# LiangZhaoPKUImperial/LinearSFM

Hardware: AMD Instinct MI355X
Metric: hierarchical linear map-joining solve wall-clock, NC3500-like stereo (all transforms + joins) (lower is better)
Workload: dtype f64

## Files before the change

include/lsfm.h:

```cpp
#ifndef LSFM_H
#define LSFM_H

#include <stddef.h>

#ifdef __cplusplus
extern "C" {
#endif

#define LSFM_OK 0
#define LSFM_ERR_ARG (-1)
#define LSFM_ERR_NO_DEVICE (-2)
#define LSFM_ERR_HIP (-3)
#define LSFM_ERR_OOM (-4)
#define LSFM_ERR_INTERNAL (-5)
#define LSFM_ERR_IO (-6)
#define LSFM_ERR_NOT_SPD (-7)
#define LSFM_NOT_CONVERGED 1

typedef struct lsfm_context lsfm_context;

typedef struct lsfm_map {
	int Ref, FRef, m, n, nU, nW;
	int ScaP, Fix, Sign, FScaP, FFix;
	int* stno;
	double* stVal;
	double* U;
	int *Ui, *Uj;
	double* W;
	int *photo, *feature;
	double* V;
	int* FBlock;
	int* pose_origin;
} lsfm_map;

typedef struct lsfm_stats {
	double t_total_ms;
	double t_transform_ms, t_join_ms, t_schur_ms, t_pcg_ms, t_backsub_ms;
	long pcg_iterations;
	long spmv_launches;
	double spmv_ms;
	double spmv_bytes;
	long spmv_nnzb_upper_last, spmv_rows_last;
	double max_rel_residual;
	int levels, joins, transforms;
	int not_converged;
	long schur_launches, trf_launches;
	double schur_ms, schur_bytes, trf_ms, trf_bytes;
	double schur_flops;
	double upload_ms;
	int attempts;
	unsigned long long s_digest, factor_digest;
	int dist_solves;
	double dist_work_total, dist_work_shared;
	int refactor_mismatch;
	int s_rebuild_mismatch;
	int small_levels;
	double t_small_ms;
} lsfm_stats;

int lsfm_context_create(int device, size_t arena_bytes, lsfm_context** out);
void lsfm_context_destroy(lsfm_context* ctx);
int lsfm_set_pcg(lsfm_context* ctx, double rel_tol, int max_steps);
int lsfm_set_precision(lsfm_context* ctx, int mode);
int lsfm_set_small_solve(lsfm_context* ctx, int max_poses);
int lsfm_set_spmv_variant(lsfm_context* ctx, int variant);
int lsfm_set_covcols_panel(lsfm_context* ctx, int variant);
const char* lsfm_last_error(lsfm_context* ctx);
void* lsfm_stream(lsfm_context* ctx);

void lsfm_map_release(lsfm_map* g);

int lsfm_transform_stereo(lsfm_context* ctx, const lsfm_map* in, int Ref, lsfm_map* out);
int lsfm_transform_mono(lsfm_context* ctx, const lsfm_map* in, int Ref, int ScaP, int Fix, lsfm_map* out);

int lsfm_join_stereo(lsfm_context* ctx, const lsfm_map* End, const lsfm_map* Cur, lsfm_map* joint,
                     double* eP_out, double* eF_out);
int lsfm_join_mono(lsfm_context* ctx, const lsfm_map* End, const lsfm_map* Cur, lsfm_map* joint,
                   double* eP_out, double* eF_out);

int lsfm_solve_stereo(lsfm_context* ctx, double* stVal, const double* eb, const double* ea, const double* U,
                      const double* W, const double* V, const int* Ui, const int* Uj, const int* photo,
                      const int* feature, int m, int n, int nU, int nW, const double* x0);
int lsfm_solve_mono(lsfm_context* ctx, double* stVal, const double* eb, const double* ea, const double* U,
                    const double* W, const double* V, const int* Ui, const int* Uj, const int* photo,
                    const int* feature, int m, int n, int nU, int nW, int Ref, int ScaP, int Fix, int Sign,
                    int FixBlk, const double* x0);

int lsfm_gn_polish(lsfm_context* ctx, const lsfm_map* maps, int N, int type, lsfm_map* x, int iters, double* obj, double* gnorm, int* halvings);

int lsfm_map_chi2(lsfm_context* ctx, const lsfm_map* maps, int N, int type, const lsfm_map* x, double* chi2, int* dof);
int lsfm_gn_polish_robust(lsfm_context* ctx, const lsfm_map* maps, int N, int type, lsfm_map* x, int iters, int kind, double c,
                          double* obj, double* gnorm, int* halvings, double* chi2, double* weight);

int lsfm_map_feature_chi2(lsfm_context* ctx, const lsfm_map* maps, int N, int type, const lsfm_map* x, double* fchi2, double* pose_chi2);
int lsfm_gn_polish_robust_features(lsfm_context* ctx, const lsfm_map* maps, int N, int type, lsfm_map* x, int iters, int kind, double c,
                                   double* obj, double* gnorm, int* halvings, double* fchi2, double* fweight);

int lsfm_gn_linearise(lsfm_context* ctx, const lsfm_map* maps, int N, int type, const lsfm_map* x, const double* weight,
                      lsfm_map* out, double* obj, double* b);
int lsfm_gn_linearise_timed(lsfm_context* ctx, const lsfm_map* maps, int N, int type, const lsfm_map* x, const double* weight,
                            lsfm_map* out, double* obj, double* b, double* times, int* counts);

int lsfm_map_covariance(lsfm_context* ctx, const lsfm_map* map, int mono, double* pose_cov, double* feat_cov, double* pair_cov, int cap_blocks, int* nnzb);
int lsfm_map_covariance_timed(lsfm_context* ctx, const lsfm_map* map, int mono, double* pose_cov, double* feat_cov, double* pair_cov, int cap_blocks, int* nnzb,
                              double* times);

int lsfm_map_covariance_columns(lsfm_context* ctx, const lsfm_map* map, int mono, const int* poses, int k, double* pose_cols, double* feat_cols,
                                double* joint, int* steps, double* last_corr);
int lsfm_map_covariance_columns_timed(lsfm_context* ctx, const lsfm_map* map, int mono, const int* poses, int k, double* pose_cols, double* feat_cols,
                                      double* joint, int* steps, double* last_corr, double* times);

int lsfm_map_covariance_feature_columns(lsfm_context* ctx, const lsfm_map* map, int mono, const int* feats, int k, double* pose_cols, double* feat_cols,
                                        double* joint, int* steps, double* last_corr);
int lsfm_map_feature_pair_gate(lsfm_context* ctx, const lsfm_map* map, int mono, const int* pairs, int K, double* d2, double* cov_diff, int* steps,
                               double* last_corr);
int lsfm_map_covariance_feature_columns_timed(lsfm_context* ctx, const lsfm_map* map, int mono, const int* feats, int k, double* pose_cols,
                                              double* feat_cols, double* joint, int* steps, double* last_corr, double* times);
int lsfm_map_feature_pair_gate_timed(lsfm_context* ctx, const lsfm_map* map, int mono, const int* pairs, int K, double* d2, double* cov_diff, int* steps,
                                     double* last_corr, double* times);

int lsfm_map_merge_features(lsfm_context* ctx, const lsfm_map* map, int mono, const int* pairs, int K, lsfm_map* out, double* d2, int* dof, int* rep,
                            int* steps, double* last_corr);
int lsfm_map_merge_features_timed(lsfm_context* ctx, const lsfm_map* map, int mono, const int* pairs, int K, lsfm_map* out, double* d2, int* dof,
                                  int* rep, int* steps, double* last_corr, double* times);
int lsfm_merge_structure(const lsfm_map* map, const int* pairs, int K, int* rep, int* photo, int* feature, int* FBlock, int* sptr, int* sidx, int cap_w,
                         int* info, char* why, int why_cap);

int lsfm_map_feature_pair_candidates(lsfm_context* ctx, const lsfm_map* map, const double* feat_cov, double radius, double tau, int* pairs, double* dist2,
                                     double* q, long long cap, long long* count);
int lsfm_map_feature_pair_candidates_timed(lsfm_context* ctx, const lsfm_map* map, const double* feat_cov, double radius, double tau, int* pairs,
                                           double* dist2, double* q, long long cap, long long* count, double* times, long long* info);

#define LSFM_JOINT_GATE_MAX 2048
int lsfm_map_feature_pair_joint_gate(lsfm_context* ctx, const lsfm_map* map, int mono, const int* pairs, int K, const int* order, double tau, int* status,
                                     double* delta, double* d2, double* joint_C, int* accepted, int* implied, double* D2, int* steps, double* last_corr);
int lsfm_map_feature_pair_joint_gate_timed(lsfm_context* ctx, const lsfm_map* map, int mono, const int* pairs, int K, const int* order, double tau,
                                           int* status, double* delta, double* d2, double* joint_C, int* accepted, int* implied, double* D2, int* steps,
                                           double* last_corr, double* times);
int lsfm_selftest_pair_select(lsfm_context* ctx, int K, const double* C, const double* d, const int* ends, const int* order, double tau, int* status,
                              double* delta, double* D2, int* accepted, int* implied);

int lsfm_map_marginalise(lsfm_context* ctx, const lsfm_map* map, const unsigned char* drop, lsfm_map* out);
int lsfm_map_marginalise_timed(lsfm_context* ctx, const lsfm_map* map, const unsigned char* drop, lsfm_map* out, double* times);

int lsfm_map_marginalise_poses(lsfm_context* ctx, const lsfm_map* map, int mono, const unsigned char* keep_pose, const unsigned char* drop_feat,
                               lsfm_map* out);
int lsfm_map_marginalise_poses_timed(lsfm_context* ctx, const lsfm_map* map, int mono, const unsigned char* keep_pose, const unsigned char* drop_feat,
                                     lsfm_map* out, double* times, int* info);
int lsfm_marg_pose_structure(const lsfm_map* map, int mono, const unsigned char* keep_pose, const unsigned char* drop_feat, unsigned char* drop,
                             int* comp, int* nptr, int* nidx, int cap_n, int* bd, int* Ui, int* Uj, int cap_u, int* info, char* why, int why_cap);

int lsfm_gn_structure(const lsfm_map* maps, int N, int type, const lsfm_map* x, int want_slots, int want_coalesce, int* info, int* map_hubs,
                      int* wdst, int* fptrJ, int* photoJ, int cap_wj, int* UiJ, int* UjJ, int cap_uj, int* photo, int* feature, int* FBlock,
                      int cap_w, int* Ui, int* Uj, int cap_u, int* slot_map, int* slot_a, int* slot_b, int* slot_count, int cap_s, char* why,
                      int why_cap);

int lsfm_inverse_v(lsfm_context* ctx, double* V, int m, int n);
int lsfm_solve_features(lsfm_context* ctx, const double* W, const double* IV, const double* ea, const double* eb, const double* dpa, double* dpb,
                        int m, int n, const int* mapCor, const int* photo);

int lsfm_schur_pattern(lsfm_context* ctx, const int* Ui, const int* Uj, const int* photo, const int* feature, int m, int n, int nU, int nW,
                       int* rowptr, int* colidx, int cap, int* nnzb);

int lsfm_symbolic_analyse(int m, const int* rowptr, const int* colidx, const int* origin, int reps, int* perm, int* colptr, int* rowidx,
                          int cap, int* info, double* avg_ms);

typedef struct lsfm_tree lsfm_tree;
int lsfm_tree_upload(lsfm_context* ctx, const lsfm_map* maps, int N, int mono, lsfm_tree** out);
int lsfm_tree_run(lsfm_context* ctx, lsfm_tree* tree, lsfm_stats* stats);
int lsfm_tree_set_final_reanchor(lsfm_tree* tree, int on);
int lsfm_tree_set_plans(lsfm_tree* tree, int on);
int lsfm_tree_download(lsfm_context* ctx, lsfm_tree* tree, lsfm_map* out);
int lsfm_tree_set_stop_level(lsfm_tree* tree, int levels);
int lsfm_tree_node_count(lsfm_context* ctx, lsfm_tree* tree);
int lsfm_tree_download_node(lsfm_context* ctx, lsfm_tree* tree, int k, lsfm_map* out);
int lsfm_tree_download_state(lsfm_context* ctx, lsfm_tree* tree, int* m, int* n, int* stno, double* stVal, size_t cap);
void lsfm_tree_free(lsfm_context* ctx, lsfm_tree* tree);
size_t lsfm_tree_export_size(lsfm_context* ctx, lsfm_tree* tree);
int lsfm_tree_export_dev(lsfm_context* ctx, lsfm_tree* tree, void* dst, size_t cap);
#define LSFM_PACK_HEADER_BYTES 256
size_t lsfm_packed_size(const void* host_header256);
int lsfm_tree_upload_dev(lsfm_context* ctx, const void* const* packed, int N, int mono, lsfm_tree** out);
int lsfm_tree_export_reduced_size(lsfm_context* ctx, lsfm_tree* tree, const int* keep_ids, int nkeep, size_t* bytes);
int lsfm_tree_export_reduced_dev(lsfm_context* ctx, lsfm_tree* tree, const int* keep_ids, int nkeep, void* dst, size_t cap);
int lsfm_tree_export_reduced_dev_timed(lsfm_context* ctx, lsfm_tree* tree, const int* keep_ids, int nkeep, void* dst, size_t cap, double* times);
int lsfm_tree_reload_dev(lsfm_context* ctx, lsfm_tree* tree, const void* const* packed, int N);

#define LSFM_DTYPE_F64 0
#define LSFM_DTYPE_I64 1
typedef int (*lsfm_allreduce_fn)(void* user, size_t offset_bytes, size_t count, int dtype, void* hip_stream);
int lsfm_tree_set_comm(lsfm_tree* tree, int rank, int world, lsfm_allreduce_fn fn, void* user, void* dev_buf, size_t dev_bytes);
int lsfm_tree_set_comm_blocks(lsfm_tree* tree, int block_maps);
int lsfm_tree_export_slice_sizes(lsfm_context* ctx, lsfm_tree* tree, int nslices, size_t* sizes);
int lsfm_tree_export_slice_dev(lsfm_context* ctx, lsfm_tree* tree, int nslices, int slice, void* dst, size_t cap);

int lsfm_divide_conquer(lsfm_context* ctx, const lsfm_map* maps, int N, int mono, lsfm_map* out, lsfm_stats* stats);

int lsfm_read_localmap(const char* path, int mono, lsfm_map* out);
int lsfm_read_localmaps(const char* dir, int first, int count, int mono, int threads, lsfm_map* out, int* failed);
int lsfm_write_localmap(const char* path, int mono, const lsfm_map* map);
int lsfm_write_mapset(const char* path, const lsfm_map* maps, int N, int mono);
int lsfm_mapset_info(const char* path, int* N, int* mono);
int lsfm_mapset_stamp(const char* path, unsigned long long* stamp, const unsigned long long* set_to);
int lsfm_read_mapset(const char* path, int mono, int first, int count, int threads, lsfm_map* out);
int lsfm_save_covariances(const char* pose_path, const char* feat_path, const int* stno, int m, int n, const double* pose_cov, const double* feat_cov);
int lsfm_read_covariances(const char* path, int k, int* ids, double* cov, int cap, int* count);
int lsfm_save_cov_columns(const char* path, const int* stno, int m, const int* poses, int k, const double* pose_cols);
int lsfm_read_cov_columns(const char* path, int* ids_q, int* ids_p, double* blocks, int cap, int* count);
int lsfm_save_pair_gate(const char* path, const int* ids, int K, const double* d2, const double* cov_diff);
int lsfm_read_pair_gate(const char* path, int* ids_f, int* ids_g, double* d2, double* cov_diff, int cap, int* count);
int lsfm_save_merge_report(const char* path, int K, int removed, int dof, double d2, const int* ids);
int lsfm_read_merge_report(const char* path, int* K, int* removed, int* dof, double* d2, int* ids, int cap);
int lsfm_save_joint_gate(const char* path, const int* ids, int K, const int* status, const double* d2, const double* delta, int accepted, int implied,
                         double D2);
int lsfm_read_joint_gate(const char* path, int* ids, int* status, double* d2, double* delta, int cap, int* head, double* D2);
int lsfm_save_pair_list(const char* path, const int* ids, long long K);
int lsfm_read_pair_list(const char* path, int* ids, long long cap, long long* count);
int lsfm_save_state(const char* path, const double* st, const int* stno, int n);
int lsfm_save_state_bin(const char* path, const double* st, const int* stno, int n);
int lsfm_save_poses(const char* pose_path, const char* feat_path, const int* stno, const double* st, int n);

int lsfm_spmv_bench(lsfm_context* ctx, int m, const int* rowptr, const int* colidx, const double* val,
                    const double* x, double* y, int reps, double* avg_ms, double* algorithmic_bytes);

int lsfm_wstream_bench(lsfm_context* ctx, long long nblocks, int mode, int reps, double* avg_ms);

int lsfm_selftest_prims(lsfm_context* ctx, int cases, unsigned seed);

int lsfm_selftest_vinv(lsfm_context* ctx, const double* V, const double* eb, int n, int skip, double* IV, double* LY);

#define LSFM_SELFTEST_CHOL_INFO 16
int lsfm_selftest_chol(lsfm_context* ctx, int m, const int* rowptr, const int* colidx, const double* val, const int* origin, const unsigned char* fixed,
                       const int* pose_seg, int nseg, const double* r, int nrhs, int mode, double* z, double* dot, int* perm, int* colptr, int* rowidx,
                       double* L, double* Dinv, double* dscale, int cap_blocks, int* info);

int lsfm_selftest_transform(lsfm_context* ctx, const lsfm_map* maps, int N, int mono, const int* tref, const int* tscap, const int* tfix,
                            int alias_passthrough, lsfm_map* out);

int lsfm_selftest_small(lsfm_context* ctx, int G, const int* pose_off, const int* feat_off, const int* u_off, const unsigned char* active,
                        const double* U, const int* Ui, const int* Uj, const double* W, const int* photo, const int* feature, int nW, const double* V,
                        const double* ea, const double* eb, const double* x0, const unsigned char* fixed, int strips, double* x_pose, double* x_feat,
                        int* status, double* max_rel);

#ifdef __cplusplus
}
#endif
#endif
```

linearsfm_amd/api.py:

```python
from __future__ import annotations

import ctypes as C
import os

import numpy as np

_HERE = os.path.dirname(os.path.abspath(__file__))
LIB_PATH = os.path.join(_HERE, "liblsfm_hip.so")
_LIB = None

LSFM_OK = 0
LSFM_NOT_CONVERGED = 1


class LsfmMap(C.Structure):
    _fields_ = [("Ref", C.c_int), ("FRef", C.c_int), ("m", C.c_int), ("n", C.c_int), ("nU", C.c_int), ("nW", C.c_int),
                ("ScaP", C.c_int), ("Fix", C.c_int), ("Sign", C.c_int), ("FScaP", C.c_int), ("FFix", C.c_int),
                ("stno", C.POINTER(C.c_int)), ("stVal", C.POINTER(C.c_double)),
                ("U", C.POINTER(C.c_double)), ("Ui", C.POINTER(C.c_int)), ("Uj", C.POINTER(C.c_int)),
                ("W", C.POINTER(C.c_double)), ("photo", C.POINTER(C.c_int)), ("feature", C.POINTER(C.c_int)),
                ("V", C.POINTER(C.c_double)), ("FBlock", C.POINTER(C.c_int)), ("pose_origin", C.POINTER(C.c_int))]


class LsfmStats(C.Structure):
    _fields_ = [("t_total_ms", C.c_double), ("t_transform_ms", C.c_double), ("t_join_ms", C.c_double),
                ("t_schur_ms", C.c_double), ("t_pcg_ms", C.c_double), ("t_backsub_ms", C.c_double),
                ("pcg_iterations", C.c_long), ("spmv_launches", C.c_long), ("spmv_ms", C.c_double),
                ("spmv_bytes", C.c_double), ("spmv_nnzb_upper_last", C.c_long), ("spmv_rows_last", C.c_long),
                ("max_rel_residual", C.c_double), ("levels", C.c_int), ("joins", C.c_int), ("transforms", C.c_int),
                ("not_converged", C.c_int), ("schur_launches", C.c_long), ("trf_launches", C.c_long),
                ("schur_ms", C.c_double), ("schur_bytes", C.c_double), ("trf_ms", C.c_double), ("trf_bytes", C.c_double),
                ("schur_flops", C.c_double), ("upload_ms", C.c_double), ("attempts", C.c_int),
                ("s_digest", C.c_ulonglong), ("factor_digest", C.c_ulonglong), ("dist_solves", C.c_int), ("dist_work_total", C.c_double), ("dist_work_shared", C.c_double), ("refactor_mismatch", C.c_int), ("s_rebuild_mismatch", C.c_int), ("small_levels", C.c_int), ("t_small_ms", C.c_double)]

    def as_dict(self):
        return {k: getattr(self, k) for k, _ in self._fields_}


class LsfmError(RuntimeError):
    pass


ALLREDUCE_FN = C.CFUNCTYPE(C.c_int, C.c_void_p, C.c_size_t, C.c_size_t, C.c_int, C.c_void_p)
LSFM_DTYPE_F64, LSFM_DTYPE_I64 = 0, 1
JOINT_GATE_MAX = 2048
JOINT_GATE_TAU = 11.344866730144373


def lib():
    global _LIB
    if _LIB is None:
        if not os.path.exists(LIB_PATH):
            raise LsfmError(f"{LIB_PATH} is missing: build it with `python -c 'import __graft_entry__ as g; g.build()'` "
                            "(hipcc --offload-arch=gfx950).  There is no CPU fallback.")
        L = C.CDLL(LIB_PATH)
        P = C.POINTER
        dp, ip, vp = P(C.c_double), P(C.c_int), C.c_void_p
        L.lsfm_context_create.argtypes = [C.c_int, C.c_size_t, P(vp)]
        L.lsfm_context_destroy.argtypes = [vp]
        L.lsfm_context_destroy.restype = None
        L.lsfm_set_pcg.argtypes = [vp, C.c_double, C.c_int]
        L.lsfm_set_precision.argtypes = [vp, C.c_int]
        L.lsfm_set_small_solve.argtypes = [vp, C.c_int]
        L.lsfm_set_spmv_variant.argtypes = [vp, C.c_int]
        L.lsfm_set_covcols_panel.argtypes = [vp, C.c_int]
        L.lsfm_last_error.argtypes = [vp]
        L.lsfm_last_error.restype = C.c_char_p
        L.lsfm_stream.argtypes = [vp]
        L.lsfm_stream.restype = vp
        L.lsfm_map_release.argtypes = [P(LsfmMap)]
        L.lsfm_map_release.restype = None
        L.lsfm_transform_stereo.argtypes = [vp, P(LsfmMap), C.c_int, P(LsfmMap)]
        L.lsfm_transform_mono.argtypes = [vp, P(LsfmMap), C.c_int, C.c_int, C.c_int, P(LsfmMap)]
        L.lsfm_join_stereo.argtypes = [vp, P(LsfmMap), P(LsfmMap), P(LsfmMap), dp, dp]
        L.lsfm_join_mono.argtypes = [vp, P(LsfmMap), P(LsfmMap), P(LsfmMap), dp, dp]
        L.lsfm_solve_stereo.argtypes = [vp, dp, dp, dp, dp, dp, dp, ip, ip, ip, ip, C.c_int, C.c_int, C.c_int, C.c_int, dp]
        L.lsfm_solve_mono.argtypes = [vp, dp, dp, dp, dp, dp, dp, ip, ip, ip, ip, C.c_int, C.c_int, C.c_int, C.c_int,
                                      C.c_int, C.c_int, C.c_int, C.c_int, C.c_int, dp]
        L.lsfm_tree_upload.argtypes = [vp, P(LsfmMap), C.c_int, C.c_int, P(vp)]
        L.lsfm_tree_run.argtypes = [vp, vp, P(LsfmStats)]
        L.lsfm_tree_set_final_reanchor.argtypes = [vp, C.c_int]
        L.lsfm_tree_set_plans.argtypes = [vp, C.c_int]
        L.lsfm_tree_export_size.argtypes = [vp, vp]
        L.lsfm_tree_export_size.restype = C.c_size_t
        L.lsfm_tree_export_dev.argtypes = [vp, vp, vp, C.c_size_t]
        L.lsfm_packed_size.argtypes = [vp]
        L.lsfm_packed_size.restype = C.c_size_t
        L.lsfm_tree_upload_dev.argtypes = [vp, P(vp), C.c_int, C.c_int, P(vp)]
        L.lsfm_tree_reload_dev.argtypes = [vp, vp, P(vp), C.c_int]
        L.lsfm_tree_set_comm.argtypes = [vp, C.c_int, C.c_int, ALLREDUCE_FN, vp, vp, C.c_size_t]
        L.lsfm_tree_set_comm_blocks.argtypes = [vp, C.c_int]
        L.lsfm_tree_export_slice_sizes.argtypes = [vp, vp, C.c_int, P(C.c_size_t)]
        L.lsfm_tree_export_slice_dev.argtypes = [vp, vp, C.c_int, C.c_int, vp, C.c_size_t]
        L.lsfm_tree_download.argtypes = [vp, vp, P(LsfmMap)]
        L.lsfm_tree_set_stop_level.argtypes = [vp, C.c_int]
        L.lsfm_tree_node_count.argtypes = [vp, vp]
        L.lsfm_tree_download_node.argtypes = [vp, vp, C.c_int, P(LsfmMap)]
        L.lsfm_tree_download_state.argtypes = [vp, vp, ip, ip, ip, dp, C.c_size_t]
        L.lsfm_tree_free.argtypes = [vp, vp]
        L.lsfm_tree_free.restype = None
        L.lsfm_divide_conquer.argtypes = [vp, P(LsfmMap), C.c_int, C.c_int, P(LsfmMap), P(LsfmStats)]
        L.lsfm_read_localmap.argtypes = [C.c_char_p, C.c_int, P(LsfmMap)]
        L.lsfm_write_localmap.argtypes = [C.c_char_p, C.c_int, P(LsfmMap)]
        L.lsfm_read_localmaps.argtypes = [C.c_char_p, C.c_int, C.c_int, C.c_int, C.c_int, P(LsfmMap), P(C.c_int)]
        L.lsfm_write_mapset.argtypes = [C.c_char_p, P(LsfmMap), C.c_int, C.c_int]
        L.lsfm_mapset_info.argtypes = [C.c_char_p, P(C.c_int), P(C.c_int)]
        L.lsfm_read_mapset.argtypes = [C.c_char_p, C.c_int, C.c_int, C.c_int, C.c_int, P(LsfmMap)]
        L.lsfm_save_state_bin.argtypes = [C.c_char_p, P(C.c_double), P(C.c_int), C.c_int]
        L.lsfm_save_state.argtypes = [C.c_char_p, dp, ip, C.c_int]
        L.lsfm_save_poses.argtypes = [C.c_char_p, C.c_char_p, ip, dp, C.c_int]
        L.lsfm_schur_pattern.argtypes = [vp, ip, ip, ip, ip, C.c_int, C.c_int, C.c_int, C.c_int, ip, ip, C.c_int, ip]
        L.lsfm_symbolic_analyse.argtypes = [C.c_int, ip, ip, ip, C.c_int, ip, ip, ip, C.c_int, ip, dp]
        L.lsfm_inverse_v.argtypes = [vp, dp, C.c_int, C.c_int]
        L.lsfm_selftest_vinv.argtypes = [vp, dp, dp, C.c_int, C.c_int, dp, dp]
        L.lsfm_gn_polish.argtypes = [vp, P(LsfmMap), C.c_int, C.c_int, P(LsfmMap), C.c_int, dp, dp, ip]
        L.lsfm_gn_polish_robust.argtypes = [vp, P(LsfmMap), C.c_int, C.c_int, P(LsfmMap), C.c_int, C.c_int, C.c_double, dp, dp, ip, dp, dp]
        L.lsfm_map_chi2.argtypes = [vp, P(LsfmMap), C.c_int, C.c_int, P(LsfmMap), dp, ip]
        L.lsfm_map_feature_chi2.argtypes = [vp, P(LsfmMap), C.c_int, C.c_int, P(LsfmMap), dp, dp]
        L.lsfm_gn_polish_robust_features.argtypes = [vp, P(LsfmMap), C.c_int, C.c_int, P(LsfmMap), C.c_int, C.c_int, C.c_double, dp, dp, ip, dp, dp]
        L.lsfm_gn_linearise.argtypes = [vp, P(LsfmMap), C.c_int, C.c_int, P(LsfmMap), dp, P(LsfmMap), dp, dp]
        L.lsfm_gn_linearise_timed.argtypes = [vp, P(LsfmMap), C.c_int, C.c_int, P(LsfmMap), dp, P(LsfmMap), dp, dp, dp, ip]
        L.lsfm_solve_features.argtypes = [vp, dp, dp, dp, dp, dp, dp, C.c_int, C.c_int, ip, ip]
        L.lsfm_map_covariance.argtypes = [vp, P(LsfmMap), C.c_int, dp, dp, dp, C.c_int, ip]
        L.lsfm_map_covariance_timed.argtypes = [vp, P(LsfmMap), C.c_int, dp, dp, dp, C.c_int, ip, dp]
        L.lsfm_save_covariances.argtypes = [C.c_char_p, C.c_char_p, ip, C.c_int, C.c_int, dp, dp]
        L.lsfm_read_covariances.argtypes = [C.c_char_p, C.c_int, ip, dp, C.c_int, ip]
        L.lsfm_map_covariance_columns.argtypes = [vp, P(LsfmMap), C.c_int, ip, C.c_int, dp, dp, dp, ip, dp]
        L.lsfm_map_covariance_columns_timed.argtypes = [vp, P(LsfmMap), C.c_int, ip, C.c_int, dp, dp, dp, ip, dp, dp]
        L.lsfm_map_covariance_feature_columns.argtypes = [vp, P(LsfmMap), C.c_int, ip, C.c_int, dp, dp, dp, ip, dp]
        L.lsfm_map_covariance_feature_columns_timed.argtypes = [vp, P(LsfmMap), C.c_int, ip, C.c_int, dp, dp, dp, ip, dp, dp]
        L.lsfm_map_feature_pair_gate.argtypes = [vp, P(LsfmMap), C.c_int, ip, C.c_int, dp, dp, ip, dp]
        L.lsfm_map_feature_pair_gate_timed.argtypes = [vp, P(LsfmMap), C.c_int, ip, C.c_int, dp, dp, ip, dp, dp]
        L.lsfm_map_merge_features.argtypes = [vp, P(LsfmMap), C.c_int, ip, C.c_int, P(LsfmMap), dp, ip, ip, ip, dp]
        L.lsfm_map_merge_features_timed.argtypes = [vp, P(LsfmMap), C.c_int, ip, C.c_int, P(LsfmMap), dp, ip, ip, ip, dp, dp]
        L.lsfm_map_feature_pair_joint_gate.argtypes = [vp, P(LsfmMap), C.c_int, ip, C.c_int, ip, C.c_double, ip, dp, dp, dp, ip, ip, dp, ip, dp]
        L.lsfm_map_feature_pair_joint_gate_timed.argtypes = [vp, P(LsfmMap), C.c_int, ip, C.c_int, ip, C.c_double, ip, dp, dp, dp, ip, ip, dp, ip, dp, dp]
        L.lsfm_selftest_pair_select.argtypes = [vp, C.c_int, dp, dp, ip, ip, C.c_double, ip, dp, dp, ip, ip]
        L.lsfm_save_joint_gate.argtypes = [C.c_char_p, ip, C.c_int, ip, dp, dp, C.c_int, C.c_int, C.c_double]
        L.lsfm_read_joint_gate.argtypes = [C.c_char_p, ip, ip, dp, dp, C.c_int, ip, dp]
        L.lsfm_merge_structure.argtypes = [P(LsfmMap), ip, C.c_int, ip, ip, ip, ip, ip, ip, C.c_int, ip, C.c_char_p, C.c_int]
        llp = P(C.c_longlong)
        L.lsfm_map_feature_pair_candidates.argtypes = [vp, P(LsfmMap), dp, C.c_double, C.c_double, ip, dp, dp, C.c_longlong, llp]
        L.lsfm_map_feature_pair_candidates_timed.argtypes = [vp, P(LsfmMap), dp, C.c_double, C.c_double, ip, dp, dp, C.c_longlong, llp, dp, llp]
        L.lsfm_save_pair_list.argtypes = [C.c_char_p, ip, C.c_longlong]
        L.lsfm_read_pair_list.argtypes = [C.c_char_p, ip, C.c_longlong, llp]
        L.lsfm_save_merge_report.argtypes = [C.c_char_p, C.c_int, C.c_int, C.c_int, C.c_double, ip]
        L.lsfm_read_merge_report.argtypes = [C.c_char_p, ip, ip, ip, dp, ip, C.c_int]
        L.lsfm_save_cov_columns.argtypes = [C.c_char_p, ip, C.c_int, ip, C.c_int, dp]
        L.lsfm_read_cov_columns.argtypes = [C.c_char_p, ip, ip, dp, C.c_int, ip]
        L.lsfm_save_pair_gate.argtypes = [C.c_char_p, ip, C.c_int, dp, dp]
        L.lsfm_read_pair_gate.argtypes = [C.c_char_p, ip, ip, dp, dp, C.c_int, ip]
        L.lsfm_map_marginalise.argtypes = [vp, P(LsfmMap), P(C.c_ubyte), P(LsfmMap)]
        L.lsfm_map_marginalise_timed.argtypes = [vp, P(LsfmMap), P(C.c_ubyte), P(LsfmMap), dp]
        ub = P(C.c_ubyte)
        L.lsfm_map_marginalise_poses.argtypes = [vp, P(LsfmMap), C.c_int, ub, ub, P(LsfmMap)]
        L.lsfm_map_marginalise_poses_timed.argtypes = [vp, P(LsfmMap), C.c_int, ub, ub, P(LsfmMap), dp, ip]
        L.lsfm_marg_pose_structure.argtypes = [P(LsfmMap), C.c_int, ub, ub, ub, ip, ip, ip, C.c_int, ip, ip, ip, C.c_int, ip, C.c_char_p, C.c_int]
        L.lsfm_gn_structure.argtypes = [P(LsfmMap), C.c_int, C.c_int, P(LsfmMap), C.c_int, C.c_int, ip, ip, ip, ip, ip, C.c_int, ip, ip, C.c_int, ip, ip, ip,
                                        C.c_int, ip, ip, C.c_int, ip, ip, ip, ip, C.c_int, C.c_char_p, C.c_int]
        L.lsfm_tree_export_reduced_size.argtypes = [vp, vp, ip, C.c_int, P(C.c_size_t)]
        L.lsfm_tree_export_reduced_dev.argtypes = [vp, vp, ip, C.c_int, vp, C.c_size_t]
        L.lsfm_tree_export_reduced_dev_timed.argtypes = [vp, vp, ip, C.c_int, vp, C.c_size_t, dp]
        L.lsfm_spmv_bench.argtypes = [vp, C.c_int, ip, ip, dp, dp, dp, C.c_int, dp, dp]
        L.lsfm_wstream_bench.argtypes = [vp, C.c_longlong, C.c_int, C.c_int, dp]
        L.lsfm_selftest_prims.argtypes = [vp, C.c_int, C.c_uint]
        L.lsfm_selftest_chol.argtypes = [vp, C.c_int, ip, ip, dp, ip, P(C.c_ubyte), ip, C.c_int, dp, C.c_int, C.c_int, dp, dp, ip, ip, ip, dp, dp, dp,
                                         C.c_int, ip]
        L.lsfm_selftest_transform.argtypes = [vp, P(LsfmMap), C.c_int, C.c_int, ip, ip, ip, C.c_int, P(LsfmMap)]
        L.lsfm_selftest_small.argtypes = [vp, C.c_int, ip, ip, ip, ub, dp, ip, ip, dp, ip, ip, C.c_int, dp, dp, dp, dp, ub, C.c_int, dp, dp, ip, dp]
        _LIB = L
    return _LIB


EXPORTS = ["lsfm_context_create", "lsfm_context_destroy", "lsfm_set_pcg", "lsfm_set_precision", "lsfm_set_small_solve", "lsfm_set_spmv_variant", "lsfm_set_covcols_panel", "lsfm_last_error", "lsfm_stream",
           "lsfm_map_release", "lsfm_transform_stereo", "lsfm_transform_mono", "lsfm_join_stereo", "lsfm_join_mono",
           "lsfm_solve_stereo", "lsfm_solve_mono", "lsfm_tree_upload", "lsfm_tree_run", "lsfm_tree_set_final_reanchor",
           "lsfm_tree_download", "lsfm_tree_set_stop_level", "lsfm_tree_node_count", "lsfm_tree_download_node", "lsfm_tree_download_state", "lsfm_tree_set_plans", "lsfm_tree_export_size", "lsfm_tree_export_dev", "lsfm_packed_size",
           "lsfm_tree_upload_dev", "lsfm_tree_reload_dev", "lsfm_tree_set_comm", "lsfm_tree_set_comm_blocks", "lsfm_tree_export_slice_sizes", "lsfm_tree_export_slice_dev",
           "lsfm_tree_free", "lsfm_divide_conquer", "lsfm_read_localmap", "lsfm_read_localmaps", "lsfm_write_localmap", "lsfm_write_mapset", "lsfm_mapset_info", "lsfm_mapset_stamp", "lsfm_read_mapset", "lsfm_save_state_bin", "lsfm_save_state", "lsfm_save_poses", "lsfm_gn_polish",
           "lsfm_gn_polish_robust", "lsfm_map_chi2", "lsfm_map_feature_chi2", "lsfm_gn_polish_robust_features", "lsfm_gn_linearise", "lsfm_gn_linearise_timed",
           "lsfm_spmv_bench", "lsfm_wstream_bench", "lsfm_selftest_prims", "lsfm_selftest_chol", "lsfm_selftest_transform", "lsfm_selftest_small", "lsfm_schur_pattern", "lsfm_symbolic_analyse", "lsfm_inverse_v", "lsfm_selftest_vinv", "lsfm_solve_features",
           "lsfm_map_covariance", "lsfm_map_covariance_timed",
           "lsfm_save_covariances", "lsfm_read_covariances",
           "lsfm_map_covariance_columns", "lsfm_map_covariance_columns_timed", "lsfm_save_cov_columns", "lsfm_read_cov_columns",
           "lsfm_map_covariance_feature_columns", "lsfm_map_covariance_feature_columns_timed", "lsfm_map_feature_pair_gate", "lsfm_map_feature_pair_gate_timed", "lsfm_save_pair_gate", "lsfm_read_pair_gate",
           "lsfm_map_merge_features", "lsfm_map_merge_features_timed", "lsfm_merge_structure", "lsfm_save_merge_report", "lsfm_read_merge_report",
           "lsfm_map_feature_pair_candidates", "lsfm_map_feature_pair_candidates_timed", "lsfm_save_pair_list", "lsfm_read_pair_list",
           "lsfm_map_feature_pair_joint_gate", "lsfm_map_feature_pair_joint_gate_timed", "lsfm_selftest_pair_select", "lsfm_save_joint_gate", "lsfm_read_joint_gate",
           "lsfm_map_marginalise", "lsfm_map_marginalise_timed", "lsfm_tree_export_reduced_size", "lsfm_tree_export_reduced_dev",
           "lsfm_tree_export_reduced_dev_timed", "lsfm_map_marginalise_poses", "lsfm_map_marginalise_poses_timed", "lsfm_marg_pose_structure", "lsfm_gn_structure"]


def _c(a, dtype):
    return np.ascontiguousarray(a, dtype=dtype).reshape(-1)


def _ptr(a, ctype):
    return a.ctypes.data_as(C.POINTER(ctype))


class HostMap:

    def __init__(self, d):
        g = d if isinstance(d, dict) else d.__dict__
        self.stno = _c(g["stno"], np.int32); self.stVal = _c(g["stVal"], np.float64)
        self.U = _c(g["U"], np.float64); self.Ui = _c(g["Ui"], np.int32); self.Uj = _c(g["Uj"], np.int32)
        self.W = _c(g["W"], np.float64); self.photo = _c(g["photo"], np.int32); self.feature = _c(g["feature"], np.int32)
        self.V = _c(g["V"], np.float64); self.FBlock = _c(g["FBlock"], np.int32)
        c = LsfmMap()
        c.Ref = int(g["Ref"]); c.FRef = int(g.get("FRef", g["Ref"])); c.m = int(g["m"]); c.n = int(g["n"])
        c.nU = len(self.Ui); c.nW = len(self.photo)
        c.ScaP = int(g.get("ScaP", 0)); c.Fix = int(g.get("Fix", 0)); c.Sign = int(g.get("Sign", 1))
        c.FScaP = int(g.get("FScaP", c.ScaP)); c.FFix = int(g.get("FFix", c.Fix))
        c.stno = _ptr(self.stno, C.c_int); c.stVal = _ptr(self.stVal, C.c_double)
        c.U = _ptr(self.U, C.c_double); c.Ui = _ptr(self.Ui, C.c_int); c.Uj = _ptr(self.Uj, C.c_int)
        c.W = _ptr(self.W, C.c_double); c.photo = _ptr(self.photo, C.c_int); c.feature = _ptr(self.feature, C.c_int)
        c.V = _ptr(self.V, C.c_double); c.FBlock = _ptr(self.FBlock, C.c_int)
        if g.get("pose_origin") is not None:
            self.pose_origin = _c(g["pose_origin"], np.int32)
            c.pose_origin = _ptr(self.pose_origin, C.c_int)
        self.c = c


def _arr(ptr, n, dtype):
    if n == 0:
        return np.zeros(0, dtype)
    return np.ctypeslib.as_array(ptr, shape=(n,)).astype(dtype, copy=True)


def map_to_dict(g: LsfmMap, release=True):
    r = 6 * g.m + 3 * g.n
    d = dict(Ref=g.Ref, FRef=g.FRef, m=g.m, n=g.n, nU=g.nU, nW=g.nW, ScaP=g.ScaP, Fix=g.Fix, Sign=g.Sign,
             FScaP=g.FScaP, FFix=g.FFix,
             stno=_arr(g.stno, r, np.int32), stVal=_arr(g.stVal, r, np.float64),
             U=_arr(g.U, 36 * g.nU, np.float64).reshape(-1, 36), Ui=_arr(g.Ui, g.nU, np.int32), Uj=_arr(g.Uj, g.nU, np.int32),
             W=_arr(g.W, 18 * g.nW, np.float64).reshape(-1, 18), photo=_arr(g.photo, g.nW, np.int32),
             feature=_arr(g.feature, g.nW, np.int32), V=_arr(g.V, 9 * g.n, np.float64).reshape(-1, 9),
             FBlock=_arr(g.FBlock, g.n, np.int32))
    if g.pose_origin:
        d["pose_origin"] = _arr(g.pose_origin, g.m, np.int32)
    if release:
        lib().lsfm_map_release(C.byref(g))
    return d


def _gn_args(maps, G):
    hms = [HostMap(d) for d in maps]
    arr = (LsfmMap * len(hms))(*[h.c for h in hms])
    x = LsfmMap()
    stno = _c(G["stno"], np.int32)
    st = np.array(np.asarray(G["stVal"], np.float64), copy=True)
    x.m, x.n, x.Ref, x.FRef = int(G["m"]), int(G["n"]), int(G["Ref"]), int(G.get("FRef", G["Ref"]))
    x.ScaP, x.Fix, x.Sign = int(G.get("ScaP", 0)), int(G.get("Fix", 0)), int(G.get("Sign", 1))
    x.FScaP, x.FFix = int(G.get("FScaP", x.ScaP)), int(G.get("FFix", x.Fix))
    x.stno, x.stVal = _ptr(stno, C.c_int), _ptr(st, C.c_double)
    org = None
    if G.get("pose_origin") is not None:
        org = _c(G["pose_origin"], np.int32)
        x.pose_origin = _ptr(org, C.c_int)
    return hms, arr, x, (stno, st, org)


class Context:

    def __init__(self, device=0, arena_bytes=0):
        self._h = C.c_void_p()
        rc = lib().lsfm_context_create(int(device), int(arena_bytes), C.byref(self._h))
        if rc != 0:
            self._h = None
            raise LsfmError(f"lsfm_context_create failed (rc={rc}): no usable HIP device -- there is no CPU fallback")

    def close(self):
        if self._h:
            lib().lsfm_context_destroy(self._h)
            self._h = None

    def __del__(self):
        try:
            self.close()
        except Exception:
            pass

    def _check(self, rc, what):
        if rc < 0:
            raise LsfmError(f"{what} failed (rc={rc}): {lib().lsfm_last_error(self._h).decode()}")
        return rc

    def set_pcg(self, rel_tol=1e-12, max_steps=0):
        self._check(lib().lsfm_set_pcg(self._h, float(rel_tol), int(max_steps)), "lsfm_set_pcg")

    def set_precision(self, mixed):
        self._check(lib().lsfm_set_precision(self._h, 1 if mixed else 0), "lsfm_set_precision")

    def set_small_solve(self, max_poses=5):
        self._check(lib().lsfm_set_small_solve(self._h, int(max_poses)), "lsfm_set_small_solve")

    def set_spmv_variant(self, variant):
        self._check(lib().lsfm_set_spmv_variant(self._h, int(variant)), "lsfm_set_spmv_variant")

    def set_covcols_panel(self, variant):
        self._check(lib().lsfm_set_covcols_panel(self._h, int(variant)), "lsfm_set_covcols_panel")

    def stream(self):
        return lib().lsfm_stream(self._h)

    def tree_reload_dev(self, tree, dev_ptrs):
        arr = (C.c_void_p * len(dev_ptrs))(*[C.c_void_p(int(p)) for p in dev_ptrs])
        self._check(lib().lsfm_tree_reload_dev(self._h, tree, arr, len(dev_ptrs)), "lsfm_tree_reload_dev")

    def transform(self, d, mono, Ref, ScaP=0, Fix=0):
        hm = HostMap(d)
        out = LsfmMap()
        if mono:
            rc = lib().lsfm_transform_mono(self._h, C.byref(hm.c), int(Ref), int(ScaP), int(Fix), C.byref(out))
        else:
            rc = lib().lsfm_transform_stereo(self._h, C.byref(hm.c), int(Ref), C.byref(out))
        self._check(rc, "lsfm_transform")
        return map_to_dict(out)

    def join(self, dEnd, dCur, mono):
        he, hc = HostMap(dEnd), HostMap(dCur)
        out = LsfmMap()
        m = he.c.m + hc.c.m - (2 if mono else 0)
        eP = np.zeros(6 * m)
        eF = np.zeros(3 * (he.c.n + hc.c.n))
        fn = lib().lsfm_join_mono if mono else lib().lsfm_join_stereo
        rc = self._check(fn(self._h, C.byref(he.c), C.byref(hc.c), C.byref(out), _ptr(eP, C.c_double), _ptr(eF, C.c_double)),
                         "lsfm_join")
        j = map_to_dict(out)
        return j, eP, eF[:3 * j["n"]], rc

    def solve(self, j, eP, eF, mono, sa=None, x0=None):
        m, n = int(j["m"]), int(j["n"])
        st = np.zeros(6 * m + 3 * n)
# ... 367 lines not shown
        if (feat_cov is None) != (tau is None):
            raise LsfmError("feature_pair_candidates: feat_cov and tau go together")
        rc, count, _, _, _, _, _ = self.feature_pair_candidates_raw(d, radius, feat_cov, tau)
        self._check(rc, "lsfm_map_feature_pair_candidates")
        rc, count, pr, dd, qq, _, _ = self.feature_pair_candidates_raw(d, radius, feat_cov, tau, cap=count)
        self._check(rc, "lsfm_map_feature_pair_candidates")
        return dict(pairs=pr[:count], dist2=dd[:count], q=qq[:count] if qq is not None else None)

    def feature_pair_joint_gate_raw(self, d, mono, pairs, tau=None, order=None, want_C=False, times=False):
        h = HostMap(d)
        pr = _c(pairs, np.int32)
        K = len(pr) // 2
        k1 = max(K, 1)
        od = _c(order, np.int32) if order is not None else None
        if od is not None and len(od) != K:
            raise LsfmError(f"feature_pair_joint_gate: an order of {len(od)} entries for {K} pairs")
        st, dl, dd, corr = np.zeros(k1, np.int32), np.zeros(k1), np.zeros(k1), np.zeros(k1)
        Cm = np.zeros((3 * K, 3 * K)) if (want_C and 1 <= K <= JOINT_GATE_MAX) else None
        acc, imp, steps, D2 = C.c_int(0), C.c_int(0), C.c_int(0), C.c_double(0.0)
        t = np.zeros(6) if times else None
        rc = lib().lsfm_map_feature_pair_joint_gate_timed(self._h, C.byref(h.c), int(mono), _ptr(pr, C.c_int) if K else None, K,
                                                          _ptr(od, C.c_int) if od is not None and K else None, float(JOINT_GATE_TAU if tau is None else tau),
                                                          _ptr(st, C.c_int), _ptr(dl, C.c_double), _ptr(dd, C.c_double),
                                                          _ptr(Cm, C.c_double) if Cm is not None else None, C.byref(acc), C.byref(imp), C.byref(D2),
                                                          C.byref(steps), _ptr(corr, C.c_double), _ptr(t, C.c_double) if times else None)
        return rc, dict(status=st[:K], delta=dl[:K], d2=dd[:K], C=Cm, accepted=acc.value, implied=imp.value, D2=D2.value, steps=steps.value,
                        last_corr=corr[:K]), t

    def feature_pair_joint_gate(self, d, mono, pairs, tau=None, order=None, want_C=False):
        rc, out, _ = self.feature_pair_joint_gate_raw(d, mono, pairs, tau, order, want_C)
        self._check(rc, "lsfm_map_feature_pair_joint_gate")
        if rc > 0 and out["steps"] == 0:
            raise LsfmError(f"lsfm_map_feature_pair_joint_gate: {rc} pivot(s) floored -- the information matrix is too close to singular")
        out["dof"] = 3 * out["accepted"]
        out["converged"] = rc == 0
        return out

    def selftest_pair_select(self, Cm, d, ends, tau, order=None, raw=False):
        en = _c(ends, np.int32)
        K = len(en) // 2
        cm, dv = _c(Cm, np.float64), _c(d, np.float64)
        if len(cm) != 9 * K * K or len(dv) != 3 * K:
            raise LsfmError(f"selftest_pair_select: {len(cm)} matrix and {len(dv)} vector entries for {K} pairs")
        od = _c(order, np.int32) if order is not None else None
        if od is not None and len(od) != K:
            raise LsfmError(f"selftest_pair_select: an order of {len(od)} entries for {K} pairs")
        st, dl = np.zeros(max(K, 1), np.int32), np.zeros(max(K, 1))
        acc, imp, D2 = C.c_int(0), C.c_int(0), C.c_double(0.0)
        rc = lib().lsfm_selftest_pair_select(self._h, K, _ptr(cm, C.c_double), _ptr(dv, C.c_double), _ptr(en, C.c_int),
                                             _ptr(od, C.c_int) if od is not None else None, float(tau), _ptr(st, C.c_int), _ptr(dl, C.c_double),
                                             C.byref(D2), C.byref(acc), C.byref(imp))
        out = dict(status=st[:K], delta=dl[:K], D2=D2.value, accepted=acc.value, implied=imp.value)
        if raw:
            return rc, out
        self._check(rc, "lsfm_selftest_pair_select")
        return out

    def marginalise(self, d, drop, times=False):
        h = HostMap(d)
        fl = np.ascontiguousarray(np.asarray(drop).astype(bool), dtype=np.uint8).reshape(-1)
        if len(fl) != h.c.n:
            raise LsfmError(f"marginalise: {len(fl)} flags for {h.c.n} features")
        out = LsfmMap()
        t = np.zeros(3)
        self._check(lib().lsfm_map_marginalise_timed(self._h, C.byref(h.c), _ptr(fl, C.c_ubyte), C.byref(out), _ptr(t, C.c_double) if times else None),
                    "lsfm_map_marginalise")
        g = map_to_dict(out)
        if times:
            return g, dict(zip(("structure_ms", "values_ms", "emit_ms"), t.tolist()))
        return g

    def marginalise_poses(self, d, mono, keep_pose, drop_feat=None, times=False, info=False):
        h = HostMap(d)
        kp = np.ascontiguousarray(np.asarray(keep_pose).astype(bool), dtype=np.uint8).reshape(-1)
        if len(kp) != h.c.m:
            raise LsfmError(f"marginalise_poses: {len(kp)} flags for {h.c.m} poses")
        fl = None
        if drop_feat is not None:
            fl = np.ascontiguousarray(np.asarray(drop_feat).astype(bool), dtype=np.uint8).reshape(-1)
            if len(fl) != h.c.n:
                raise LsfmError(f"marginalise_poses: {len(fl)} flags for {h.c.n} features")
        out = LsfmMap()
        t = np.zeros(5)
        inf = np.zeros(8, np.int32)
        rc = self._check(lib().lsfm_map_marginalise_poses_timed(self._h, C.byref(h.c), int(mono), _ptr(kp, C.c_ubyte), _ptr(fl, C.c_ubyte) if fl is not None else None,
                                                                C.byref(out), _ptr(t, C.c_double), _ptr(inf, C.c_int)), "lsfm_map_marginalise_poses")
        if rc != 0:
            raise LsfmError(f"lsfm_map_marginalise_poses: {rc} pivot(s) floored -- the dropped poses' own system is too close to singular")
        res = [map_to_dict(out)]
        if times:
            res.append(dict(zip(("stage_a_ms", "structure_ms", "factor_ms", "sweeps_ms", "syrk_emit_ms"), t.tolist())))
        if info:
            res.append(dict(zip(MARG_POSES_INFO, (int(v) for v in inf))))
        return res[0] if len(res) == 1 else tuple(res)

    def spmv_bench(self, rowptr, colidx, val, x, reps=20):
        rowptr = _c(rowptr, np.int32); colidx = _c(colidx, np.int32); val = _c(val, np.float64); x = _c(x, np.float64)
        m = len(rowptr) - 1
        y = np.zeros(6 * m)
        ms, by = C.c_double(), C.c_double()
        self._check(lib().lsfm_spmv_bench(self._h, m, _ptr(rowptr, C.c_int), _ptr(colidx, C.c_int), _ptr(val, C.c_double),
                                          _ptr(x, C.c_double), _ptr(y, C.c_double), int(reps), C.byref(ms), C.byref(by)),
                    "lsfm_spmv_bench")
        return y, ms.value, by.value


def _wstream(self, nblocks, mode, reps=10):
    ms = C.c_double()
    self._check(lib().lsfm_wstream_bench(self._h, int(nblocks), int(mode), int(reps), C.byref(ms)), "lsfm_wstream_bench")
    return ms.value


Context.wstream_bench = _wstream


def _selftest_prims(self, cases=64, seed=1):
    self._check(lib().lsfm_selftest_prims(self._h, int(cases), int(seed)), "lsfm_selftest_prims")


Context.selftest_prims = _selftest_prims

SELFTEST_CHOL_INFO = ("blocks", "leaf_tasks", "leaf_columns", "task0_outer", "groups", "group_levels", "fused_levels", "split_levels", "max_rows_below",
                      "d_err", "floored")


def _selftest_chol(self, rowptr, colidx, val, r, origin=None, fixed=None, pose_seg=None, nseg=1, mode=0):
    rowptr = _c(rowptr, np.int32); colidx = _c(colidx, np.int32); val = _c(val, np.float64)
    m = len(rowptr) - 1
    if m < 1 or len(colidx) != rowptr[-1] or len(val) != 36 * len(colidx):
        raise LsfmError("selftest_chol: rowptr / colidx / val do not fit together")
    r = np.ascontiguousarray(r, dtype=np.float64).reshape(-1, 6 * m)
    nrhs = r.shape[0]
    org = _c(origin, np.int32) if origin is not None else None
    fx = np.ascontiguousarray(np.asarray(fixed).astype(bool), dtype=np.uint8).reshape(-1) if fixed is not None else None
    seg = _c(pose_seg, np.int32) if pose_seg is not None else np.zeros(m, np.int32)
    if (org is not None and len(org) != m) or (fx is not None and len(fx) != 6 * m) or len(seg) != m:
        raise LsfmError("selftest_chol: origin / fixed / pose_seg do not fit m")
    cap = int(symbolic_analyse(rowptr, colidx, org)["info"][0])
    z = np.zeros((nrhs, 6 * m)); dot = np.zeros((nrhs, int(nseg)))
    perm = np.zeros(m, np.int32); colptr = np.zeros(m + 1, np.int32); rowidx = np.zeros(cap, np.int32)
    Lb = np.zeros((cap, 6, 6)); Dinv = np.zeros((m, 6, 6)); dscale = np.zeros(6 * m)
    info = np.zeros(16, np.int32)
    rc = lib().lsfm_selftest_chol(self._h, m, _ptr(rowptr, C.c_int), _ptr(colidx, C.c_int), _ptr(val, C.c_double),
                                  _ptr(org, C.c_int) if org is not None else None, _ptr(fx, C.c_ubyte) if fx is not None else None,
                                  _ptr(seg, C.c_int), int(nseg), _ptr(r, C.c_double), nrhs, int(mode), _ptr(z, C.c_double), _ptr(dot, C.c_double),
                                  _ptr(perm, C.c_int), _ptr(colptr, C.c_int), _ptr(rowidx, C.c_int), _ptr(Lb, C.c_double), _ptr(Dinv, C.c_double),
                                  _ptr(dscale, C.c_double), cap, _ptr(info, C.c_int))
    self._check(rc, "lsfm_selftest_chol")
    return dict(z=z, dot=dot, perm=perm, colptr=colptr, rowidx=rowidx, L=Lb, Dinv=Dinv, dscale=dscale,
                info=dict(zip(SELFTEST_CHOL_INFO, (int(v) for v in info))))


Context.selftest_chol = _selftest_chol


def _selftest_transform(self, dicts, mono, targets, alias=False):
    hms = [HostMap(d) for d in dicts]
    N = len(hms)
    if N < 1 or len(targets) != N:
        raise LsfmError("selftest_transform: one target per map")
    t = np.zeros((3, N), np.int32)
    for b, tg in enumerate(targets):
        t[:, b] = (-1, 0, 0) if tg is None else (tuple(tg) + (0, 0))[:3] if isinstance(tg, (tuple, list)) else (int(tg), 0, 0)
    arr = (LsfmMap * N)(*[h.c for h in hms])
    out = (LsfmMap * N)()
    rc = lib().lsfm_selftest_transform(self._h, arr, N, int(bool(mono)), _ptr(t[0], C.c_int), _ptr(t[1], C.c_int), _ptr(t[2], C.c_int),
                                       int(bool(alias)), out)
    self._check(rc, "lsfm_selftest_transform")
    return [map_to_dict(out[b]) for b in range(N)]


Context.selftest_transform = _selftest_transform


def _selftest_small(self, B, strips=0, active=None, fixed=None, x0=None, prefill=None):
    po, fo, uo = (_c(B[k], np.int32) for k in ("pose_off", "feat_off", "u_off"))
    G = len(po) - 1
    if G < 1 or len(fo) != G + 1 or len(uo) != G + 1:
        raise LsfmError("selftest_small: pose_off / feat_off / u_off must have one entry per system and one more")
    M, NF, NU = int(po[-1]), int(fo[-1]), int(uo[-1])
    U = _c(B["U"], np.float64); Ui = _c(B["Ui"], np.int32); Uj = _c(B["Uj"], np.int32)
    W = _c(B["W"], np.float64); ph = _c(B["photo"], np.int32); fe = _c(B["feature"], np.int32); V = _c(B["V"], np.float64)
    ea = _c(B["ea"], np.float64); eb = _c(B["eb"], np.float64)
    nW = len(ph)
    if (len(U), len(Ui), len(Uj)) != (36 * NU, NU, NU) or (len(W), len(fe)) != (18 * nW, nW) or (len(V), len(ea), len(eb)) != (9 * NF, 6 * M, 3 * NF):
        raise LsfmError("selftest_small: the arrays do not fit the offsets")
    flags = lambda a, n, what: None if a is None else _fit(np.ascontiguousarray(np.asarray(a).astype(bool), dtype=np.uint8).reshape(-1), n, what)
    act, fx = flags(active, G, "active"), flags(fixed, 6 * M, "fixed")
    x0 = None if x0 is None else _fit(_c(x0, np.float64), 6 * M, "x0")
    if prefill is None:
        xp, xf = np.full(6 * M, np.nan), np.full(3 * NF, np.nan)
    else:
        xp, xf = _fit(np.array(_c(prefill[0], np.float64)), 6 * M, "prefill"), _fit(np.array(_c(prefill[1], np.float64)), 3 * NF, "prefill")
    st = np.zeros(2, np.int32)
    mr = C.c_double()
    d, i, opt = C.c_double, C.c_int, lambda a, t: None if a is None else _ptr(a, t)
    rc = lib().lsfm_selftest_small(self._h, G, _ptr(po, i), _ptr(fo, i), _ptr(uo, i), opt(act, C.c_ubyte), _ptr(U, d), _ptr(Ui, i), _ptr(Uj, i),
                                   _ptr(W, d), _ptr(ph, i), _ptr(fe, i), nW, _ptr(V, d), _ptr(ea, d), _ptr(eb, d), opt(x0, d), opt(fx, C.c_ubyte),
                                   int(strips), _ptr(xp, d), _ptr(xf, d), _ptr(st, i), C.byref(mr))
    self._check(rc, "lsfm_selftest_small")
    return xp, xf, st, mr.value


def _fit(a, n, what):
    if len(a) != n:
        raise LsfmError(f"selftest_small: {what} has {len(a)} entries, not {n}")
    return a


Context.selftest_small = _selftest_small


def symbolic_analyse(rowptr, colidx, origin=None, reps=1):
    rowptr = _c(rowptr, np.int32); colidx = _c(colidx, np.int32)
    m = len(rowptr) - 1
    org = _c(origin, np.int32) if origin is not None else None
    info = np.zeros(8, np.int32)
    perm = np.zeros(m, np.int32); colptr = np.zeros(m + 1, np.int32)
    ms = C.c_double()
    lib().lsfm_symbolic_analyse(m, _ptr(rowptr, C.c_int), _ptr(colidx, C.c_int), _ptr(org, C.c_int) if org is not None else None, 1,
                                _ptr(perm, C.c_int), _ptr(colptr, C.c_int), None, 0, _ptr(info, C.c_int), None)
    rowidx = np.zeros(max(int(info[0]), 1), np.int32)
    rc = lib().lsfm_symbolic_analyse(m, _ptr(rowptr, C.c_int), _ptr(colidx, C.c_int), _ptr(org, C.c_int) if org is not None else None, int(reps),
                                     _ptr(perm, C.c_int), _ptr(colptr, C.c_int), _ptr(rowidx, C.c_int), len(rowidx), _ptr(info, C.c_int), C.byref(ms))
    if rc:
        raise LsfmError(f"lsfm_symbolic_analyse failed (rc={rc}): malformed pattern")
    return dict(perm=perm, colptr=colptr, rowidx=rowidx[:int(info[0])], info=info, ms=ms.value)


MARG_POSES_INFO = ("dropped", "boundary", "components", "blocks", "chunks", "leaf_tasks", "groups", "group_levels")


def marg_pose_structure(d, mono, keep_pose, drop_feat=None):
    h = HostMap(d)
    m, n = h.c.m, h.c.n
    kp = None if keep_pose is None else np.ascontiguousarray(np.asarray(keep_pose).astype(bool), dtype=np.uint8).reshape(-1)
    fl = None if drop_feat is None else np.ascontiguousarray(np.asarray(drop_feat).astype(bool), dtype=np.uint8).reshape(-1)
    if (kp is not None and len(kp) != m) or (fl is not None and len(fl) != n):
        raise LsfmError("marg_pose_structure: the flags do not fit the map")
    info = np.zeros(8, np.int32)
    why = C.create_string_buffer(512)
    ub = C.c_ubyte
    args = (C.byref(h.c), int(mono), _ptr(kp, ub) if kp is not None else None, _ptr(fl, ub) if fl is not None else None)
    rc = lib().lsfm_marg_pose_structure(*args, None, None, None, None, 0, None, None, None, 0, _ptr(info, C.c_int), why, len(why))
    if rc:
        raise LsfmError(f"lsfm_marg_pose_structure failed (rc={rc}): {why.value.decode()}")
    drop = np.zeros(max(n, 1), np.uint8); comp = np.zeros(m, np.int32); nptr = np.zeros(m + 1, np.int32); bd = np.zeros(m, np.int32)
    nidx = np.zeros(max(int(info[4]), 1), np.int32); Ui = np.zeros(max(int(info[3]), 1), np.int32); Uj = np.zeros_like(Ui)
    rc = lib().lsfm_marg_pose_structure(*args, _ptr(drop, ub), _ptr(comp, C.c_int), _ptr(nptr, C.c_int), _ptr(nidx, C.c_int), len(nidx), _ptr(bd, C.c_int),
                                        _ptr(Ui, C.c_int), _ptr(Uj, C.c_int), len(Ui), _ptr(info, C.c_int), why, len(why))
    if rc:
        raise LsfmError(f"lsfm_marg_pose_structure failed (rc={rc}): {why.value.decode()}")
    nc = int(info[2])
    return dict(drop=drop[:n].astype(bool), comp=comp, nptr=nptr[:nc + 1].copy(), nidx=nidx[:int(info[4])].copy(), bd=bd[:int(info[1])].copy(),
                Ui=Ui[:int(info[3])].copy(), Uj=Uj[:int(info[3])].copy(), info=info)


MERGE_STRUCTURE_INFO = ("n", "nW", "classes", "removed", "summed_blocks")


def merge_structure(d, pairs):
    h = HostMap(d)
    pr = _c(pairs, np.int32)
    K = len(pr) // 2
    info = np.zeros(8, np.int32)
    why = C.create_string_buffer(512)
    p = lambda a: _ptr(a, C.c_int)
    head = (C.byref(h.c), p(pr) if K else None, K)
    rc = lib().lsfm_merge_structure(*head, None, None, None, None, None, None, 0, p(info), why, len(why))
    if rc:
        raise LsfmError(f"lsfm_merge_structure failed (rc={rc}): {why.value.decode()}")
    v = dict(zip(MERGE_STRUCTURE_INFO, (int(i) for i in info)))
    n, nW = h.c.n, h.c.nW
    cap = max(nW, 1)
    rep, photo, feature, FBlock = np.zeros(max(n, 1), np.int32), np.zeros(cap, np.int32), np.zeros(cap, np.int32), np.zeros(max(n, 1), np.int32)
    sptr, sidx = np.zeros(cap + 1, np.int32), np.zeros(cap, np.int32)
    rc = lib().lsfm_merge_structure(*head, p(rep), p(photo), p(feature), p(FBlock), p(sptr), p(sidx), cap, p(info), why, len(why))
    if rc:
        raise LsfmError(f"lsfm_merge_structure failed (rc={rc}): {why.value.decode()}")
    return dict(rep=rep[:n], photo=photo[:v["nW"]], feature=feature[:v["nW"]], FBlock=FBlock[:v["n"]], sptr=sptr[:v["nW"] + 1], sidx=sidx[:nW], info=v)


GN_STRUCTURE_INFO = ("M", "NFG", "P", "FI", "NUJ", "NWJ", "nU", "nW", "slots", "contributors")


def gn_structure(maps, mono, G, slots=False, coalesce=False):
    hms, arr, x, keep = _gn_args(maps, G)
    N = len(hms)
    info = np.zeros(10, np.int32)
    why = C.create_string_buffer(512)
    head = (arr, N, 1 if mono else 0, C.byref(x), int(bool(slots)), int(bool(coalesce)), _ptr(info, C.c_int))
    rc = lib().lsfm_gn_structure(*head, None, None, None, None, 0, None, None, 0, None, None, None, 0, None, None, 0, None, None, None, None, 0, why, len(why))
    if rc:
        raise LsfmError(f"lsfm_gn_structure failed (rc={rc}): {why.value.decode()}")
    v = dict(zip(GN_STRUCTURE_INFO, (int(i) for i in info)))
    z = lambda n: np.zeros(max(n, 1), np.int32)
    hubs, wdst, fptrJ, photoJ, UiJ, UjJ = z(3 * N), z(v["FI"]), z(v["NFG"] + 1), z(v["NWJ"]), z(v["NUJ"]), z(v["NUJ"])
    photo, feature, FBlock, Ui, Uj = z(v["nW"]), z(v["nW"]), z(v["NFG"]), z(v["nU"]), z(v["nU"])
    sm, sa, sb, sc = z(v["slots"]), z(v["slots"]), z(v["slots"]), z(v["slots"])
    p = lambda a: _ptr(a, C.c_int)
    rc = lib().lsfm_gn_structure(*head, p(hubs), p(wdst), p(fptrJ), p(photoJ), len(photoJ), p(UiJ), p(UjJ), len(UiJ), p(photo), p(feature), p(FBlock),
                                 len(photo), p(Ui), p(Uj), len(Ui), p(sm), p(sa), p(sb), p(sc), len(sm), why, len(why))
    if rc:
        raise LsfmError(f"lsfm_gn_structure failed (rc={rc}): {why.value.decode()}")
    return dict(info=v, map_hubs=hubs.reshape(N, 3), wdst=wdst[:v["FI"]], fptrJ=fptrJ, photoJ=photoJ[:v["NWJ"]], UiJ=UiJ[:v["NUJ"]], UjJ=UjJ[:v["NUJ"]],
                photo=photo[:v["nW"]], feature=feature[:v["nW"]], FBlock=FBlock[:v["NFG"] if coalesce else 0], Ui=Ui[:v["nU"]], Uj=Uj[:v["nU"]],
                slot_map=sm[:v["slots"]], slot_a=sa[:v["slots"]], slot_b=sb[:v["slots"]], slot_count=sc[:v["slots"]])


LSFM_NODE_MAGIC = 1279870541


def read_localmap(path, mono):
    g = LsfmMap()
    rc = lib().lsfm_read_localmap(str(path).encode(), int(mono), C.byref(g))
    if rc:
        raise LsfmError(f"lsfm_read_localmap({path}) failed (rc={rc})")
    return map_to_dict(g)


def write_localmap(path, d, mono):
    hm = HostMap(d)
    rc = lib().lsfm_write_localmap(str(path).encode(), int(mono), C.byref(hm.c))
    if rc:
        raise LsfmError(f"lsfm_write_localmap({path}) failed (rc={rc})")


def write_mapset(path, maps, mono):
    hms = [HostMap(d) for d in maps]
    arr = (LsfmMap * len(hms))(*[h.c for h in hms])
    rc = lib().lsfm_write_mapset(str(path).encode(), arr, len(hms), int(mono))
    if rc:
        raise LsfmError(f"lsfm_write_mapset({path}) failed (rc={rc})")


def mapset_info(path):
    n, mono = C.c_int(0), C.c_int(0)
    if lib().lsfm_mapset_info(str(path).encode(), C.byref(n), C.byref(mono)):
        return None
    return n.value, bool(mono.value)


def read_mapset(path, mono, first=0, count=None, threads=0):
    info = mapset_info(path)
    if info is None:
        raise LsfmError(f"{path}: not a map-set cache")
    if count is None:
        count = info[0] - first
    arr = (LsfmMap * max(count, 1))()
    rc = lib().lsfm_read_mapset(str(path).encode(), int(mono), int(first), int(count), int(threads), arr)
    if rc:
        raise LsfmError(f"lsfm_read_mapset({path}) failed (rc={rc})")
    return [map_to_dict(arr[k]) for k in range(count)]


def read_localmaps(directory, count, mono, first=1, threads=0):
    arr = (LsfmMap * count)()
    bad = C.c_int(0)
    rc = lib().lsfm_read_localmaps(str(directory).encode(), int(first), int(count), int(mono), int(threads), arr, C.byref(bad))
    if rc:
        raise LsfmError(f"lsfm_read_localmaps({directory}) failed at localmap_{bad.value}.txt (rc={rc})")
    return [map_to_dict(arr[k]) for k in range(count)]


def save_covariances(pose_path, feat_path, d, pose_cov, feat_cov):
    stno = _c(d["stno"], np.int32)
    pc = _c(pose_cov, np.float64)
    fc = _c(feat_cov if feat_cov is not None else np.zeros(0), np.float64)
    rc = lib().lsfm_save_covariances(pose_path.encode() if pose_path else None, feat_path.encode() if feat_path else None, _ptr(stno, C.c_int),
                                     int(d["m"]), int(d["n"]), _ptr(pc, C.c_double), _ptr(fc, C.c_double))
    if rc != 0:
        raise LsfmError(f"lsfm_save_covariances failed (rc={rc})")


def read_covariances(path, k, cap=None):
    if cap is None:
        with open(path) as f:
            cap = sum(1 for line in f if line.strip())
    ids = np.zeros(max(cap, 1), np.int32)
    cov = np.zeros((max(cap, 1), k, k))
    cnt = C.c_int(0)
    rc = lib().lsfm_read_covariances(path.encode(), int(k), _ptr(ids, C.c_int), _ptr(cov, C.c_double), int(cap), C.byref(cnt))
# ... 127 lines not shown
```

linearsfm_amd/csrc/lsfm_capi.hip:

```cpp
#include <climits>
#include <cmath>
#include <cstring>

#include "lsfm_internal.hpp"
#include "lsfm_marg.hpp"
#include "lsfm_solve.hpp"
#include "lsfm_system.hpp"
#include "lsfm_tree.hpp"

using namespace lsfm;

namespace {

template <class F> int guarded(lsfm_context* ctx, F&& f)
{
	if (!ctx) return LSFM_ERR_ARG;
	struct Reset {
		lsfm_context* c;
		~Reset() { c->timed.clear(); c->ev_next = 0; c->plan = nullptr; }
	} reset{ ctx };
	try
	{
		if (hipSetDevice(ctx->device) != hipSuccess) return LSFM_ERR_NO_DEVICE;
		return f();
// ... 553 lines not shown
int lsfm_map_covariance_feature_columns_timed(lsfm_context* ctx, const lsfm_map* map, int mono, const int* feats, int k, double* pose_cols, double* feat_cols,
                                              double* joint, int* steps, double* last_corr, double* times)
{
	if (!map_ok(map, mono, 0) || !feats || k < 1 || (!pose_cols && !feat_cols && !joint)) return LSFM_ERR_ARG;
	return guarded(ctx, [&]() { return map_covariance_feature_columns(ctx, map, mono == 1, feats, k, pose_cols, feat_cols, joint, steps, last_corr, times); });
}

int lsfm_map_covariance_feature_columns(lsfm_context* ctx, const lsfm_map* map, int mono, const int* feats, int k, double* pose_cols, double* feat_cols,
                                        double* joint, int* steps, double* last_corr)
{
	return lsfm_map_covariance_feature_columns_timed(ctx, map, mono, feats, k, pose_cols, feat_cols, joint, steps, last_corr, nullptr);
}

int lsfm_map_feature_pair_gate_timed(lsfm_context* ctx, const lsfm_map* map, int mono, const int* pairs, int K, double* d2, double* cov_diff, int* steps,
                                     double* last_corr, double* times)
{
	if (!map_ok(map, mono, MAP_STVAL) || !pairs || K < 1 || (!d2 && !cov_diff)) return LSFM_ERR_ARG;
	return guarded(ctx, [&]() { return map_feature_pair_gate(ctx, map, mono == 1, pairs, K, d2, cov_diff, steps, last_corr, times); });
}

int lsfm_map_feature_pair_gate(lsfm_context* ctx, const lsfm_map* map, int mono, const int* pairs, int K, double* d2, double* cov_diff, int* steps,
                               double* last_corr)
{
	return lsfm_map_feature_pair_gate_timed(ctx, map, mono, pairs, K, d2, cov_diff, steps, last_corr, nullptr);
}

int lsfm_map_feature_pair_joint_gate_timed(lsfm_context* ctx, const lsfm_map* map, int mono, const int* pairs, int K, const int* order, double tau,
                                           int* status, double* delta, double* d2, double* joint_C, int* accepted, int* implied, double* D2, int* steps,
                                           double* last_corr, double* times)
{
	if (steps) *steps = 0;
	if (!map_ok(map, mono, MAP_STVAL) || !pairs || K < 1 || !status || !delta || !accepted || !implied || !D2) return LSFM_ERR_ARG;
	return guarded(ctx, [&]() {
		return map_feature_pair_joint_gate(ctx, map, mono == 1, pairs, K, order, tau, status, delta, d2, joint_C, accepted, implied, D2, steps, last_corr, times);
	});
}

int lsfm_map_feature_pair_joint_gate(lsfm_context* ctx, const lsfm_map* map, int mono, const int* pairs, int K, const int* order, double tau, int* status,
                                     double* delta, double* d2, double* joint_C, int* accepted, int* implied, double* D2, int* steps, double* last_corr)
{
	return lsfm_map_feature_pair_joint_gate_timed(ctx, map, mono, pairs, K, order, tau, status, delta, d2, joint_C, accepted, implied, D2, steps, last_corr, nullptr);
}

int lsfm_selftest_pair_select(lsfm_context* ctx, int K, const double* Cm, const double* d, const int* ends, const int* order, double tau, int* status,
                              double* delta, double* D2, int* accepted, int* implied)
{
	if (K < 1 || !Cm || !d || !ends || !status || !delta || !D2 || !accepted || !implied) return LSFM_ERR_ARG;
	return guarded(ctx, [&]() { return pair_select_selftest(ctx, K, Cm, d, ends, order, tau, status, delta, D2, accepted, implied); });
}

int lsfm_map_merge_features_timed(lsfm_context* ctx, const lsfm_map* map, int mono, const int* pairs, int K, lsfm_map* out, double* d2, int* dof, int* rep,
                                  int* steps, double* last_corr, double* times)
{
	if (steps) *steps = 0;
	if (!map_ok(map, mono, MAP_STNO | MAP_STVAL) || !pairs || K < 1 || !out) return LSFM_ERR_ARG;
	return guarded(ctx, [&]() { return map_merge_features(ctx, map, mono == 1, pairs, K, out, d2, dof, rep, steps, last_corr, times); });
}

int lsfm_map_merge_features(lsfm_context* ctx, const lsfm_map* map, int mono, const int* pairs, int K, lsfm_map* out, double* d2, int* dof, int* rep,
                            int* steps, double* last_corr)
{
	return lsfm_map_merge_features_timed(ctx, map, mono, pairs, K, out, d2, dof, rep, steps, last_corr, nullptr);
}

int lsfm_map_feature_pair_candidates_timed(lsfm_context* ctx, const lsfm_map* map, const double* feat_cov, double radius, double tau, int* pairs,
                                           double* dist2, double* q, long long cap, long long* count, double* times, long long* info)
{
	if (!map || map->m < 0 || map->n < 0 || (map->n && !map->stVal) || !count) return LSFM_ERR_ARG;
	long long cnt = 0;
	const int rc = guarded(ctx, [&]() { return map_feature_pair_candidates(ctx, map, feat_cov, radius, tau, pairs, dist2, q, cap, &cnt, times, info); });
	*count = cnt;
	return rc;
}

int lsfm_map_feature_pair_candidates(lsfm_context* ctx, const lsfm_map* map, const double* feat_cov, double radius, double tau, int* pairs, double* dist2,
                                     double* q, long long cap, long long* count)
{
	return lsfm_map_feature_pair_candidates_timed(ctx, map, feat_cov, radius, tau, pairs, dist2, q, cap, count, nullptr, nullptr);
}

int lsfm_inverse_v(lsfm_context* ctx, double* V, int m, int n)
{
	(void)m;
	if (n < 0 || (n && !V)) return LSFM_ERR_ARG;
	return guarded(ctx, [&]() { return inverse_v(ctx, V, n); });
}

int lsfm_selftest_vinv(lsfm_context* ctx, const double* V, const double* eb, int n, int skip, double* IV, double* LY)
{
	if (n < 0 || skip < 0 || skip > 1 || (n && (!V || !eb || !IV || !LY))) return LSFM_ERR_ARG;
	return guarded(ctx, [&]() { return vinv_selftest(ctx, V, eb, n, skip, IV, LY); });
}

int lsfm_solve_features(lsfm_context* ctx, const double* W, const double* IV, const double* ea, const double* eb, const double* dpa, double* dpb,
                        int m, int n, const int* mapCor, const int* photo)
{
	(void)ea;
	if (m <= 0 || n < 0 || !dpa || (n && (!W || !IV || !eb || !dpb || !mapCor || !photo))) return LSFM_ERR_ARG;
	return guarded(ctx, [&]() { return solve_features(ctx, W, IV, eb, dpa, dpb, m, n, mapCor, photo); });
}

int lsfm_schur_pattern(lsfm_context* ctx, const int* Ui, const int* Uj, const int* photo, const int* feature, int m, int n, int nU, int nW, int* rowptr,
                       int* colidx, int cap, int* nnzb)
{
	if (m <= 0 || n < 0 || nU < 0 || nW < 0 || !rowptr || !colidx || !nnzb || (nU && (!Ui || !Uj)) || (nW && (!photo || !feature))) return LSFM_ERR_ARG;
	return guarded(ctx, [&]() {
		HostSystem h;
		h.m = m; h.n = n; h.nU = nU; h.nW = nW;
		h.Ui = Ui; h.Uj = Uj; h.photo = photo; h.feature = feature;
		SolveIO io;
		system_upload(ctx, h, 0, system_fptr(h, true), nullptr, io);
		int cnt = 0;
		const int* d_rowptr = nullptr;
		const int* d_colidx = nullptr;
		schur_pattern_only(ctx, io, &cnt, &d_rowptr, &d_colidx);
		*nnzb = cnt;
		if (cnt > cap) LSFM_FAIL(LSFM_ERR_ARG, "colidx too small for the pattern (" + std::to_string(cnt) + " blocks)");
		d2h(ctx, rowptr, d_rowptr, (size_t)(m + 1) * sizeof(int));
		d2h(ctx, colidx, d_colidx, (size_t)cnt * sizeof(int));
		return LSFM_OK;
	});
}

int lsfm_spmv_bench(lsfm_context* ctx, int m, const int* rowptr, const int* colidx, const double* val, const double* x, double* y,
                    int reps, double* avg_ms, double* algorithmic_bytes)
{
	if (!rowptr || !colidx || !val || !x || !y || m <= 0) return LSFM_ERR_ARG;
	return guarded(ctx, [&]() {
		ctx->ensure_arenas(((size_t)rowptr[m] * 480 + (size_t)m * 1000) * 2 + ((size_t)64 << 20));
		ctx->scratch.reset();
		return spmv_external(ctx, m, rowptr, colidx, val, x, y, reps, avg_ms, algorithmic_bytes);
	});
}

int lsfm_selftest_chol(lsfm_context* ctx, int m, const int* rowptr, const int* colidx, const double* val, const int* origin, const unsigned char* fixed,
                       const int* pose_seg, int nseg, const double* r, int nrhs, int mode, double* z, double* dot, int* perm, int* colptr, int* rowidx,
                       double* L, double* Dinv, double* dscale, int cap_blocks, int* info)
{
	if (m <= 0 || !rowptr || !colidx || !val || !pose_seg || nseg <= 0 || !r || nrhs <= 0 || mode < 0 || mode > 3 || !z || !dot || !info || cap_blocks < 0 ||
	    rowptr[0] != 0)
		return LSFM_ERR_ARG;
	for (int p = 0; p < m; p++)
	{
		if (rowptr[p + 1] <= rowptr[p] || colidx[rowptr[p]] != p || pose_seg[p] < 0 || pose_seg[p] >= nseg) return LSFM_ERR_ARG;
		for (int k = rowptr[p] + 1; k < rowptr[p + 1]; k++)
			if (colidx[k] <= colidx[k - 1] || colidx[k] >= m) return LSFM_ERR_ARG;
	}
	for (int i = 0; i < LSFM_SELFTEST_CHOL_INFO; i++) info[i] = 0;
	return guarded(ctx, [&]() {
		return chol_selftest(ctx, m, rowptr, colidx, val, origin, fixed, pose_seg, nseg, r, nrhs, mode, z, dot, perm, colptr, rowidx, L, Dinv, dscale, cap_blocks, info);
	});
}

int lsfm_selftest_transform(lsfm_context* ctx, const lsfm_map* maps, int N, int mono, const int* tref, const int* tscap, const int* tfix,
                            int alias_passthrough, lsfm_map* out)
{
	if (!maps || N <= 0 || !tref || !out || (mono && (!tscap || !tfix))) return LSFM_ERR_ARG;
	for (int b = 0; b < N; b++) memset(&out[b], 0, sizeof out[b]);
	int rc = guarded(ctx, [&]() {
		ctx->ensure_arenas(estimate_arena(maps, N, 1));
		ctx->arena[0].reset(); ctx->arena[1].reset(); ctx->scratch.reset();
		DevBatch X, Y;
		batch_upload(ctx, ctx->arena[0], maps, N, mono != 0, X);
		std::vector<int> r(tref, tref + N), s(N, 0), f(N, 0);
		if (mono) { s.assign(tscap, tscap + N); f.assign(tfix, tfix + N); }
		transform_batch(ctx, ctx->arena[1], X, r, s, f, mono != 0, Y, alias_passthrough != 0);
		std::vector<int> delta(N, INT_MIN);
		if (Y.W_alias) d2h(ctx, delta.data(), Y.d_alias, (size_t)N * sizeof(int));
		for (int b = 0; b < N; b++)
		{
			batch_download_map(ctx, Y, b, mono != 0, &out[b]);
			if (delta[b] == INT_MIN || !out[b].nW) continue;
			d2h(ctx, out[b].W, Y.W_alias + ((ptrdiff_t)Y.w_off[b] + delta[b]) * 18, (size_t)out[b].nW * 18 * sizeof(double));
		}
		return LSFM_OK;
	});
	if (rc < 0) for (int b = 0; b < N; b++) lsfm_map_release(&out[b]);
	return rc;
}

int lsfm_selftest_small(lsfm_context* ctx, int G, const int* pose_off, const int* feat_off, const int* u_off, const unsigned char* active,
                        const double* U, const int* Ui, const int* Uj, const double* W, const int* photo, const int* feature, int nW, const double* V,
                        const double* ea, const double* eb, const double* x0, const unsigned char* fixed, int strips, double* x_pose, double* x_feat,
                        int* status, double* max_rel)
{
	if (G <= 0 || !pose_off || !feat_off || !u_off || !ea || !x_pose || !status || !max_rel || strips < 0 || nW < 0) return LSFM_ERR_ARG;
	const int M = pose_off[G], NF = feat_off[G], NU = u_off[G];
	if (M <= 0 || NF < 0 || NU < 0 || (NU && (!U || !Ui || !Uj)) || (nW && (!W || !photo || !feature)) || (NF && (!V || !eb || !x_feat))) return LSFM_ERR_ARG;
	status[0] = status[1] = 0; *max_rel = 0.0;
	return guarded(ctx, [&]() {
		HostSystem h;
		h.m = M; h.n = NF; h.nU = NU; h.nW = nW;
		h.Ui = Ui; h.Uj = Uj; h.photo = photo; h.feature = feature;
		h.U = U; h.W = W; h.V = V; h.ea = ea; h.eb = eb; h.x0 = x0;
		return small_selftest(ctx, G, pose_off, feat_off, u_off, active, h, fixed, strips, x_pose, x_feat, status, max_rel);
	});
}

int lsfm_wstream_bench(lsfm_context* ctx, long long nblocks, int mode, int reps, double* avg_ms)
{
	if (nblocks <= 0 || mode < 0 || mode > 2 || reps <= 0 || !avg_ms) return LSFM_ERR_ARG;
	return guarded(ctx, [&]() {
		ctx->ensure_arenas((size_t)nblocks * 144 * 2 + ((size_t)64 << 20));
		ctx->scratch.reset();
		return wstream_bench(ctx, nblocks, mode, reps, avg_ms);
	});
}
int lsfm_selftest_prims(lsfm_context* ctx, int cases, unsigned seed)
{
	if (cases <= 0) return LSFM_ERR_ARG;
	return guarded(ctx, [&]() { return prims_selftest(ctx, cases, seed); });
}

}
```

linearsfm_amd/csrc/lsfm_chol.hip:

```cpp
#include <algorithm>
#include <climits>
#include <cmath>
#include <cstdlib>
#include <numeric>

#include "lsfm_device.hpp"
#include "lsfm_symbolic.hpp"
#include "lsfm_chol.hpp"

namespace lsfm {

#define FX_ONE 0x1p61
#define FX_INV 0x1p-61
__device__ __forceinline__ long long fx_from(double v) { return __double2ll_rn(fmin(fmax(v, -2.0), 2.0) * FX_ONE); }
__device__ __forceinline__ double fx_to(long long a) { return (double)a * FX_INV; }
__device__ __forceinline__ void fx_atomic_sub(double* slot, double t)
{
	__hip_atomic_fetch_add(reinterpret_cast<unsigned long long*>(slot), (unsigned long long)fx_from(-t), __ATOMIC_RELAXED, __HIP_MEMORY_SCOPE_AGENT);
}
__device__ __forceinline__ int scale_exp(double d)
{
	if (!(d > 0) || !(d < 1e300)) return 0;
	return (__builtin_amdgcn_frexp_exp(d) + 1) >> 1;
}
// ... 883 lines not shown
			{
				const int ti = q / NTL, tj = q - ti * NTL;
				const double* pa = &XA[(16 * ti + (lane & 15)) * xs + (lane >> 4)];
				const double* pb = &XB[(16 * tj + (lane & 15)) * xs + (lane >> 4)];
				for (int ks = 0; ks < n6r; ks += 4) acc[i] = __builtin_amdgcn_mfma_f64_16x16x4f64(pa[ks], pb[ks], acc[i], 0, 0, 0);
			}
		}
		__syncthreads();
		double* sT = Ms;
#pragma unroll
		for (int i = 0; i < TPW; i++)
		{
			const int q = wave + (SN_THREADS / 64) * i;
			if (q < NTL * NTL)
			{
				const int ti = q / NTL, tj = q - ti * NTL;
#pragma unroll
				for (int e = 0; e < 4; e++) sT[(16 * ti + (lane >> 4) + 4 * e) * TS + 16 * tj + (lane & 15)] = acc[i][e];
			}
		}
		__syncthreads();
		for (int idx = tid; idx < HB * HB * 36; idx += nt)
		{
			const int pp = idx / 36, q = idx - pp * 36, ps = spos[pp];
			if (ps >= 0) fx_atomic_sub(L + (size_t)ps * 36 + q, sT[(6 * (pp / HB) + q / 6) * TS + 6 * (pp % HB) + q % 6]);
		}
		__syncthreads();
	}
}
static size_t sn_syrk_lds(int smax)
{
	const size_t xs = ((6 * (size_t)smax + 3) & ~(size_t)3) + 1;
	return std::max((size_t)(6 * SN_RB) * xs, (size_t)(6 * SN_RB / 2) * (6 * SN_RB / 2 + 1)) * sizeof(double);
}
static size_t sn_panel_lds(int smax)
{
	const size_t LD = 6 * (size_t)smax, xs = ((LD + 3) & ~(size_t)3) + 1;
	return std::max((LD + 6 * SN_RB + 1) * xs, (size_t)(6 * SN_RB / 2) * (6 * SN_RB / 2 + 1)) * sizeof(double);
}
__global__ void k_sn_merge(const int* __restrict__ grp_c0, const int* __restrict__ grp_s, const int* __restrict__ colptr, const double* __restrict__ Lg,
                           double* __restrict__ L)
{
	const int g = blockIdx.x, c0 = grp_c0[g], s = grp_s[g];
	const size_t b0 = (size_t)colptr[c0] * 36, b1 = (size_t)colptr[c0 + s] * 36;
	for (size_t q = b0 + threadIdx.x; q < b1; q += blockDim.x) L[q] = Lg[q];
}


template <class FT> struct SnPair;
template <> struct SnPair<double> { typedef double2 T; };
template <> struct SnPair<float> { typedef float2 T; };
template <class FT>
__device__ __forceinline__ void sn_load_diag(int s, int c0, const int* __restrict__ colptr, const FT* __restrict__ L, double* Ls, int* sSrc,
                                             int* sDst, int* sCol)
{
	const int tid = threadIdx.x, nt = blockDim.x, nb = s * (s + 1) / 2;
	for (int t = tid; t < s; t += nt) sCol[t] = colptr[c0 + t];
	__syncthreads();
	for (int e = tid; e < nb; e += nt)
	{
		int t = 0;
		while (sn_idx(s, s - 1, t) < e) t++;
		const int u = t + (e - sn_idx(s, t, t));
		sSrc[e] = (sCol[t] + (u - t)) * 36;
		sDst[e] = 6 * u * SN_XS + 6 * t;
	}
	__syncthreads();
	const int nd2 = nb * 18;
	for (int base = 0; base < nd2; base += nt * SN_LD)
	{
		typename SnPair<FT>::T v[SN_LD];
#pragma unroll
		for (int i = 0; i < SN_LD; i++)
		{
			const int q = base + i * nt + tid;
			if (q < nd2) { const int e = q / 18; v[i] = *reinterpret_cast<const typename SnPair<FT>::T*>(L + (size_t)sSrc[e] + 2 * (q - e * 18)); }
		}
#pragma unroll
		for (int i = 0; i < SN_LD; i++)
		{
			const int q = base + i * nt + tid;
			if (q < nd2) { const int e = q / 18, w = 2 * (q - e * 18); double* d = &Ls[sDst[e] + (w / 6) * SN_XS + w % 6]; d[0] = (double)v[i].x; d[1] = (double)v[i].y; }
		}
	}
	__syncthreads();
}

template <class FT>
__global__ void __launch_bounds__(SN_THREADS) k_sn_fwd(const int* __restrict__ grp_c0, const int* __restrict__ grp_s, const int* __restrict__ grp_nr,
                                                        const int* __restrict__ colptr, const int* __restrict__ rowidx, const FT* __restrict__ L,
                                                        const FT* __restrict__ Dinv, double* __restrict__ v, double* __restrict__ w, OwnFilter of)
{
	__shared__ double Ls[6 * CHOL_GS * SN_XS];
	__shared__ double sDi[CHOL_GS * 36];
	__shared__ double sA[6], sY[6 * CHOL_GS];
	__shared__ int sSrc[CHOL_GS * (CHOL_GS + 1) / 2], sDst[CHOL_GS * (CHOL_GS + 1) / 2], sCol[CHOL_GS];
	const int g = blockIdx.x, c0 = grp_c0[g], s = grp_s[g], nr = grp_nr[g];
	if (of.skip(c0)) return;
	const int tid = threadIdx.x, n6 = 6 * s;
	for (int q = tid; q < s * 36; q += SN_THREADS) sDi[q] = (double)Dinv[(size_t)c0 * 36 + q];
	double acc = tid < n6 ? v[(size_t)c0 * 6 + tid] : 0.0;
	sn_load_diag(s, c0, colptr, L, Ls, sSrc, sDst, sCol);
	for (int t = 0; t < s; t++)
	{
		const int k0 = 6 * t;
		if (tid >= k0 && tid < k0 + 6) sA[tid - k0] = acc;
		__syncthreads();
		if (tid >= k0 && tid < k0 + 6)
		{
			const int c = tid - k0;
			double y = 0.0;
			for (int k = 0; k <= c; k++) y = fma(sDi[t * 36 + c * 6 + k], sA[k], y);
			sY[tid] = y;
		}
		__syncthreads();
		if (tid >= k0 + 6 && tid < n6)
		{
			const double* lr = &Ls[tid * SN_XS + k0];
#pragma unroll
			for (int k = 0; k < 6; k++) acc = fma(-lr[k], sY[k0 + k], acc);
		}
	}
	if (tid < n6) w[(size_t)c0 * 6 + tid] = sY[tid];
	const int rows0 = colptr[c0 + s - 1] + 1;
	const int sub = tid & 3;
	for (int i = tid >> 2; i < nr; i += SN_THREADS / 4)
	{
		double o[6] = { 0, 0, 0, 0, 0, 0 };
		for (int t = sub; t < s; t += 4)
		{
			const FT* blk = L + ((size_t)sCol[t] + (s - t) + i) * 36;
			double b[36];
			ld<36>(b, blk);
#pragma unroll
			for (int r = 0; r < 6; r++)
#pragma unroll
				for (int k = 0; k < 6; k++) o[r] = fma(b[r * 6 + k], sY[6 * t + k], o[r]);
		}
#pragma unroll
		for (int r = 0; r < 6; r++)
		{
			o[r] += __shfl_xor(o[r], 1, LSFM_WAVE);
			o[r] += __shfl_xor(o[r], 2, LSFM_WAVE);
		}
		if (sub == 0)
		{
			double* dst = v + (size_t)rowidx[rows0 + i] * 6;
#pragma unroll
			for (int r = 0; r < 6; r++) atomic_add_f64(dst + r, -o[r]);
		}
	}
}

template <class FT>
__global__ void __launch_bounds__(SN_THREADS) k_sn_bwd(const int* __restrict__ grp_c0, const int* __restrict__ grp_s, const int* __restrict__ grp_nr,
                                                        const int* __restrict__ colptr, const int* __restrict__ rowidx, const FT* __restrict__ L,
                                                        const FT* __restrict__ Dinv, double* __restrict__ v, const double* __restrict__ w, OwnFilter of)
{
	__shared__ double Ls[6 * CHOL_GS * SN_XS];
	__shared__ double sDi[CHOL_GS * 36];
	__shared__ double sA[6], sZ[6 * CHOL_GS], sX[6 * CHOL_GS];
	__shared__ int sSrc[CHOL_GS * (CHOL_GS + 1) / 2], sDst[CHOL_GS * (CHOL_GS + 1) / 2], sCol[CHOL_GS];
	const int g = blockIdx.x, c0 = grp_c0[g], s = grp_s[g], nr = grp_nr[g];
	if (of.skip(c0)) return;
	const int tid = threadIdx.x, n6 = 6 * s;
	for (int q = tid; q < s * 36; q += SN_THREADS) sDi[q] = (double)Dinv[(size_t)c0 * 36 + q];
	if (tid < n6) sZ[tid] = w[(size_t)c0 * 6 + tid];
	sn_load_diag(s, c0, colptr, L, Ls, sSrc, sDst, sCol);
	const int rows0 = colptr[c0 + s - 1] + 1;
	const int sub = tid & 3;
	for (int i = tid >> 2; i < nr; i += SN_THREADS / 4)
	{
		const double* xr = v + (size_t)rowidx[rows0 + i] * 6;
		double x6[6];
		ld<6>(x6, xr);
		for (int t = sub; t < s; t += 4)
		{
			const FT* blk = L + ((size_t)sCol[t] + (s - t) + i) * 36;
			double b[36];
			ld<36>(b, blk);
#pragma unroll
			for (int c = 0; c < 6; c++)
			{
				double o = 0.0;
#pragma unroll
				for (int r = 0; r < 6; r++) o = fma(b[r * 6 + c], x6[r], o);
				lds_add_f64(&sZ[6 * t + c], -o);
			}
		}
	}
	__syncthreads();
	double acc = tid < n6 ? sZ[tid] : 0.0;
	for (int t = s - 1; t >= 0; t--)
	{
		const int k0 = 6 * t;
		if (tid >= k0 && tid < k0 + 6) sA[tid - k0] = acc;
		__syncthreads();
		if (tid >= k0 && tid < k0 + 6)
		{
			const int c = tid - k0;
			double x = 0.0;
			for (int k = c; k < 6; k++) x = fma(sDi[t * 36 + k * 6 + c], sA[k], x);
			sX[tid] = x;
		}
		__syncthreads();
		if (tid < k0)
		{
#pragma unroll
			for (int k = 0; k < 6; k++) acc = fma(-Ls[(k0 + k) * SN_XS + tid], sX[k0 + k], acc);
		}
	}
	if (tid < n6) v[(size_t)c0 * 6 + tid] = sX[tid];
}

__global__ void k_to_float(size_t n, const double* __restrict__ a, float* __restrict__ b)
{
	size_t i = (size_t)blockIdx.x * blockDim.x + threadIdx.x;
	if (i < n) b[i] = (float)a[i];
}

__global__ void k_perm_in(int M, const int* __restrict__ perm, const double* __restrict__ r, const unsigned char* __restrict__ fixed,
                          const double* __restrict__ dscale, double* __restrict__ v, int zero_from)
{
	size_t i = (size_t)blockIdx.x * blockDim.x + threadIdx.x;
	if (i >= (size_t)M * 6) return;
	const size_t src = (size_t)perm[i / 6] * 6 + i % 6;
	v[i] = ((fixed && fixed[src]) || (long)(i / 6) >= (long)zero_from) ? 0.0 : r[src] * dscale[i];
}
__global__ void k_perm_out_dot(int M, const int* __restrict__ pinv, const double* __restrict__ v, const double* __restrict__ r,
                               const unsigned char* __restrict__ fixed, const double* __restrict__ dscale, const int* __restrict__ pose_seg,
                               double* __restrict__ z, double* dot, int dot_stride, const int* __restrict__ col_owner, int rank)
{
	int row = blockIdx.x * blockDim.x + threadIdx.x;
	const bool ok = row < M;
	double acc = 0;
	int sg = 0;
	if (ok)
	{
		sg = pose_seg[row];
		const double* src = v + (size_t)pinv[row] * 6;
		const double* sc = dscale + (size_t)pinv[row] * 6;
		for (int i = 0; i < 6; i++)
		{
			double zz = src[i] * sc[i];
			if (fixed && fixed[(size_t)row * 6 + i]) zz = 0.0;
			if (col_owner) { const int ow = col_owner[pinv[row]]; if (!(ow == rank || (ow < 0 && rank == 0))) zz = 0.0; }
			z[(size_t)row * 6 + i] = zz;
			acc = fma(zz, r[(size_t)row * 6 + i], acc);
		}
	}
	if (dot) wave_scatter_add<1>(dot + (size_t)sg * dot_stride, &acc, ok);
}
__global__ void k_rz_dot(int M, const double* __restrict__ z, const double* __restrict__ r, const int* __restrict__ pose_seg, double* dot, int dot_stride)
{
	int row = blockIdx.x * blockDim.x + threadIdx.x;
	const bool ok = row < M;
	double acc = 0;
	int sg = 0;
	if (ok)
	{
		sg = pose_seg[row];
		for (int i = 0; i < 6; i++) acc = fma(z[(size_t)row * 6 + i], r[(size_t)row * 6 + i], acc);
	}
	wave_scatter_add<1>(dot + (size_t)sg * dot_stride, &acc, ok);
}

void chol_fetch(lsfm_context* ctx, const SchurSystem& sy, const int* d_origin, CholHostIn& in)
{
	const int M = sy.M, nnzb = sy.nnzb;
	in.keys.resize(nnzb);
	in.origin.resize(M);
	if (d_origin) LSFM_CHECK_HIP(hipMemcpyAsync(in.origin.data(), d_origin, (size_t)M * sizeof(int), hipMemcpyDeviceToHost, ctx->stream));
	else std::iota(in.origin.begin(), in.origin.end(), 0);
	d2h(ctx, in.keys.data(), sy.upper_keys, (size_t)nnzb * sizeof(unsigned long long));
}

void chol_alloc_values(lsfm_context* ctx, CholDev& ch)
{
	Arena& sc = ctx->scratch;
	ch.L = sc.alloc<double>((size_t)ch.nnzL * 36); ch.Dinv = sc.alloc<double>((size_t)ch.M * 36);
	ch.wv = sc.alloc<double>((size_t)ch.M * 6);
	ch.diag0 = sc.alloc<double>((size_t)ch.M * 6);
	ch.dscale = sc.alloc<double>((size_t)ch.M * 6);
	ch.Lg = ch.ngroups ? sc.alloc<double>((size_t)ch.nnzL * 36) : nullptr;
	dev_zero(ctx, ch.L, (size_t)ch.nnzL * 36 * sizeof(double));
	static const bool digest = getenv("LSFM_FACTOR_DIGEST") != nullptr;
	if (digest && ch.Lg) dev_zero(ctx, ch.Lg, (size_t)ch.nnzL * 36 * sizeof(double));
	ch.d_err = sc.alloc<int>(1);
	dev_zero(ctx, ch.d_err, sizeof(int));
}

static size_t chol_task_lds(const CholDev& ch) { return (size_t)ch.task0_maxsize * CHOL_TASK_LDS_PER_COL + 8; }
void chol_upload_index(lsfm_context* ctx, const CholSymbolic& sym, CholDev& ch)
{
	Arena& sc = ctx->scratch;
	ch.M = sym.M; ch.nnzL = sym.nnzL; ch.nlevels = sym.nlevels; ch.tail_begin = sym.tail_begin;
	ch.level_ptr = sym.level_ptr;
	if (!sym.tlevel_ptr.empty())
	{
		ch.ntask0 = sym.tlevel_ptr[1]; ch.ncol0 = sym.tlevel_col0[1];
		ch.task0_maxsize = sym.tlevel_maxsize[0]; ch.task0_lds = sym.tlevel_small_lds[0]; ch.task0_outer = sym.tlevel_outer[0];
		if (sym.tlevel_nsmall[0] != ch.ntask0 || chol_task_lds(ch) > CHOL_SOLVE_LDS)
			LSFM_FAIL(LSFM_ERR_INTERNAL, "a leaf task of the factorisation does not fit LDS (" + std::to_string(sym.tlevel_nsmall[0]) + " of " + std::to_string(ch.ntask0) +
			                                 " fit, " + std::to_string(ch.task0_maxsize) + " columns at most)");
	}
	ch.ngroups = sym.ngroups; ch.glevel_ptr = sym.glevel_ptr; ch.glevel_maxnr = sym.glevel_maxnr; ch.glevel_maxs = sym.glevel_maxs;
	ch.work_total = sym.work_total; ch.work_shared = sym.work_shared;
	ch.first_shared = sym.first_shared; ch.shared_blk0 = sym.colptr[sym.first_shared]; ch.glevel_owned = sym.glevel_owned; ch.glevel_shared = sym.glevel_shared;
	const struct { int** dst; const std::vector<int>* v; } parts[] = {
		{ &ch.grp_c0, &sym.grp_c0 }, { &ch.grp_s, &sym.grp_s }, { &ch.grp_nr, &sym.grp_nr }, { &ch.col_nin, &sym.col_nin }, { &ch.col_task, &sym.col_task },
		{ &ch.col_lpos, &sym.col_lpos }, { &ch.task_cols, &sym.task_cols }, { &ch.task_ptr, &sym.task_ptr }, { &ch.colptr, &sym.colptr },
		{ &ch.rowidx, &sym.rowidx }, { &ch.perm, &sym.perm }, { &ch.pinv, &sym.pinv }, { &ch.order, &sym.order }, { &ch.col_owner, &sym.col_owner } };
	size_t total = 0;
	for (const auto& pt : parts) total += pt.v->size();
	static thread_local std::vector<int> blob;
	blob.resize(total);
	int* d_blob = sc.alloc<int>(total);
	size_t off = 0;
	for (const auto& pt : parts)
	{
		if (!pt.v->empty()) memcpy(blob.data() + off, pt.v->data(), pt.v->size() * sizeof(int));
		*pt.dst = pt.v->empty() ? nullptr : d_blob + off;
		off += pt.v->size();
	}
	h2d(ctx, d_blob, blob.data(), total * sizeof(int));
	ch.blob = d_blob; ch.blob_ints = total;
}
void chol_upload_symbolic(lsfm_context* ctx, const CholSymbolic& sym, CholDev& ch)
{
	chol_upload_index(ctx, sym, ch);
	chol_alloc_values(ctx, ch);
	if (getenv("LSFM_DEBUG") && sym.ngroups > 50)
	{
		int hist[CHOL_GS + 1] = { 0 };
		for (int g = 0; g < sym.ngroups; g++) hist[sym.grp_s[g]]++;
		fprintf(stderr, "[lsfm] groups %d, group levels %d, sizes:", sym.ngroups, (int)sym.glevel_ptr.size() - 1);
		for (int q = 1; q <= CHOL_GS; q++) fprintf(stderr, " %d", hist[q]);
		fprintf(stderr, " | groups per level:");
		for (size_t l = 0; l + 1 < sym.glevel_ptr.size(); l++) fprintf(stderr, " %d", sym.glevel_ptr[l + 1] - sym.glevel_ptr[l]);
		fprintf(stderr, "\n");
	}
}
void chol_analyse(lsfm_context* ctx, const SchurSystem& sy, const CholHostIn& in, CholDev& ch)
{
	static thread_local CholSymbolic sym;
	chol_symbolic(in.keys.data(), sy.nnzb, in.origin.data(), sy.M, sym, ctx->comm ? ctx->comm->block_maps : 0);
	chol_upload_symbolic(ctx, sym, ch);
}

bool chol_distributed(const lsfm_context* ctx, const CholDev& ch)
{
	return ctx->comm && ctx->comm->world > 1 && ch.col_owner && ch.first_shared < ch.M;
}
static void comm_sum(lsfm_context* ctx, void* p, size_t count, int dtype)
{
	if (!count) return;
	Comm& cm = *ctx->comm;
	const size_t mk = cm.off;
	void* b = cm.alloc_bytes(count * 8);
	LSFM_CHECK_HIP(hipMemcpyAsync(b, p, count * 8, hipMemcpyDeviceToDevice, ctx->stream));
	cm.allreduce(ctx->stream, b, count, dtype);
	LSFM_CHECK_HIP(hipMemcpyAsync(p, b, count * 8, hipMemcpyDeviceToDevice, ctx->stream));
	cm.off = mk;
}
void comm_sum_host(lsfm_context* ctx, long long* h, int n)
{
	hipStream_t s = ctx->stream;
	Comm& cm = *ctx->comm;
	const size_t mk = cm.off;
	long long* d = cm.alloc<long long>(n);
	LSFM_CHECK_HIP(hipMemcpyAsync(d, h, n * sizeof(long long), hipMemcpyHostToDevice, s));
	LSFM_CHECK_HIP(hipStreamSynchronize(s));
	cm.allreduce(s, d, n, LSFM_DTYPE_I64);
	LSFM_CHECK_HIP(hipMemcpyAsync(h, d, n * sizeof(long long), hipMemcpyDeviceToHost, s));
	LSFM_CHECK_HIP(hipStreamSynchronize(s));
	cm.off = mk;
}

void chol_scatter(lsfm_context* ctx, const SchurSystem& sy, const unsigned char* fixed, CholDev& ch)
{
	const bool dist = chol_distributed(ctx, ch);
	if (sy.nnzb)
		hipLaunchKernelGGL(k_chol_scatter, dim3((sy.nnzb + 127) / 128), dim3(128), 0, ctx->stream, sy.nnzb, sy.upper_keys, sy.S, sy.rowptr, ch.pinv, ch.colptr, ch.rowidx,
		                   fixed, ch.col_task, ch.ntask0, ch.L, ch.diag0, ch.dscale, dist ? ch.col_owner : (const int*)nullptr, dist ? ctx->comm->rank : 0);
}
void chol_factor(lsfm_context* ctx, const SchurSystem& sy, const unsigned char* fixed, CholDev& ch, double* fwd_v)
{
	hipStream_t s = ctx->stream;
	const bool dist = chol_distributed(ctx, ch);
	const OwnFilter mine{ dist ? ch.col_owner : nullptr, dist ? ctx->comm->rank : 0 }, shared{ dist ? ch.col_owner : nullptr, -1 };
	ch.sn_fused_levels = ch.sn_split_levels = 0;
	if (ch.ntask0)
	{
		hipLaunchKernelGGL(k_chol_factor_level, dim3(ch.ntask0), dim3(128), (size_t)ch.task0_lds, s, ch.task_ptr, ch.task_cols, ch.col_nin, ch.colptr, ch.rowidx,
		                   ch.L, ch.Dinv, ch.d_err, mine);
		if (ch.task0_outer > 0)
		{
			const dim3 grid(ch.ncol0, std::min((ch.task0_outer + CHOL_OUT_THREADS - 1) / CHOL_OUT_THREADS, 64));
			hipLaunchKernelGGL(k_chol_update_outer, grid, dim3(CHOL_OUT_THREADS), 0, s, ch.task_cols, ch.col_nin, ch.colptr, ch.rowidx, ch.L, mine);
		}
		if (fwd_v)
			hipLaunchKernelGGL(k_chol_fwd_tasks<double>, dim3(ch.ntask0), dim3(128), chol_task_lds(ch), s, ch.task_ptr, ch.task_cols, ch.col_task, ch.col_lpos, 0, ch.colptr,
			                   ch.rowidx, (const double*)ch.L, (const double*)ch.Dinv, fwd_v, mine);
	}
	static const int fuse_max = getenv("LSFM_SN_FUSE_MAX") ? atoi(getenv("LSFM_SN_FUSE_MAX")) : 96;
	static const double piv_floor = getenv("LSFM_PIVOT_FLOOR") ? atof(getenv("LSFM_PIVOT_FLOOR")) : 1e-13;
	static const bool lds_set = []() {
		(void)hipFuncSetAttribute(reinterpret_cast<const void*>(&k_sn_panel<true>), hipFuncAttributeMaxDynamicSharedMemorySize, (int)sn_panel_lds(CHOL_GS));
		(void)hipFuncSetAttribute(reinterpret_cast<const void*>(&k_sn_panel<false>), hipFuncAttributeMaxDynamicSharedMemorySize, (int)sn_panel_lds(CHOL_GS));
		(void)hipFuncSetAttribute(reinterpret_cast<const void*>(&k_sn_syrk), hipFuncAttributeMaxDynamicSharedMemorySize, (int)sn_syrk_lds(CHOL_GS));
		return true;
	}();
	(void)lds_set;
	for (int phase = 0; phase < (dist ? 2 : 1); phase++)
	{
		const OwnFilter of = phase == 0 ? mine : shared;
		if (phase == 1)
		{
			comm_sum(ctx, ch.L + (size_t)ch.shared_blk0 * 36, ((size_t)ch.nnzL - ch.shared_blk0) * 36, LSFM_DTYPE_I64);
			if (fwd_v) comm_sum(ctx, fwd_v + (size_t)ch.first_shared * 6, ((size_t)ch.M - ch.first_shared) * 6, LSFM_DTYPE_F64);
		}
		for (size_t l = 0; l + 1 < ch.glevel_ptr.size(); l++)
		{
			const int g0 = ch.glevel_ptr[l], ng = ch.glevel_ptr[l + 1] - g0, mnr = ch.glevel_maxnr[l];
			if (!ng) continue;
			if (dist && !(phase == 0 ? ch.glevel_owned[l] : ch.glevel_shared[l])) continue;
			const int smax = l < ch.glevel_maxs.size() ? ch.glevel_maxs[l] : CHOL_GS;
			if (mnr <= fuse_max)
			{
				const int nch = (mnr + SN_RB / 2 - 1) / (SN_RB / 2);
				hipLaunchKernelGGL(k_sn_panel<true>, dim3(ng, std::max(1, nch * (nch + 1) / 2)), dim3(SN_PT), sn_panel_lds(smax), s, ch.grp_c0 + g0, ch.grp_s + g0, ch.grp_nr + g0,
				                   ch.colptr, ch.L, ch.Lg, ch.Dinv, ch.d_err, ch.rowidx, fwd_v, ch.wv, smax, ch.diag0, piv_floor, ctx->d_run ? &ctx->d_run->floored : nullptr, of);
				ch.sn_fused_levels++;
				continue;
			}
			hipLaunchKernelGGL(k_sn_panel<false>, dim3(ng, std::max(1, (mnr + SN_RB - 1) / SN_RB)), dim3(SN_PT), sn_panel_lds(smax), s, ch.grp_c0 + g0, ch.grp_s + g0, ch.grp_nr + g0,
			                   ch.colptr, ch.L, ch.Lg, ch.Dinv, ch.d_err, ch.rowidx, fwd_v, ch.wv, smax, ch.diag0, piv_floor, ctx->d_run ? &ctx->d_run->floored : nullptr, of);
			const long nch = (mnr + SN_RB / 2 - 1) / (SN_RB / 2), npair = nch * (nch + 1) / 2;
			hipLaunchKernelGGL(k_sn_syrk, dim3(ng, (unsigned)std::max<long>(1, std::min<long>(npair, 8192))), dim3(SN_THREADS), sn_syrk_lds(smax), s,
			                   ch.grp_c0 + g0, ch.grp_s + g0, ch.grp_nr + g0, ch.colptr, ch.rowidx, ch.L, ch.Lg, smax, of);
			ch.sn_split_levels++;
		}
	}
}

void chol_merge_groups(lsfm_context* ctx, const CholDev& ch)
{
	if (ch.ngroups)
		hipLaunchKernelGGL(k_sn_merge, dim3(ch.ngroups), dim3(256), 0, ctx->stream, ch.grp_c0, ch.grp_s, ch.colptr, ch.Lg, ch.L);
}
void chol_round_to_float(lsfm_context* ctx, CholDev& ch)
{
	hipStream_t s = ctx->stream;
	Arena& sc = ctx->scratch;
	const size_t nl = (size_t)ch.nnzL * 36, nd = (size_t)ch.M * 36;
	ch.Lf = sc.alloc<float>(nl); ch.Dinvf = sc.alloc<float>(nd);
	hipLaunchKernelGGL(k_to_float, dim3((unsigned)((nl + 255) / 256)), dim3(256), 0, s, nl, ch.L, ch.Lf);
	if (ch.Lg)
	{
		ch.Lgf = sc.alloc<float>(nl);
		hipLaunchKernelGGL(k_to_float, dim3((unsigned)((nl + 255) / 256)), dim3(256), 0, s, nl, ch.Lg, ch.Lgf);
	}
	hipLaunchKernelGGL(k_to_float, dim3((unsigned)((nd + 255) / 256)), dim3(256), 0, s, nd, ch.Dinv, ch.Dinvf);
}

void chol_perm_in(lsfm_context* ctx, const CholDev& ch, const double* r, const unsigned char* fixed, double* v)
{
	const size_t ns = (size_t)ch.M * 6;
	const int zero_from = (chol_distributed(ctx, ch) && ctx->comm->rank != 0) ? ch.first_shared : INT_MAX;
	hipLaunchKernelGGL(k_perm_in, dim3((unsigned)((ns + 255) / 256)), dim3(256), 0, ctx->stream, ch.M, ch.perm, r, fixed, ch.dscale, v, zero_from);
}

void chol_apply(lsfm_context* ctx, const CholDev& ch, const double* r, double* v, double* z, const unsigned char* fixed, const int* pose_seg,
                double* dot, int dot_stride, bool fwd_done)
{
	hipStream_t s = ctx->stream;
	if (!fwd_done) chol_perm_in(ctx, ch, r, fixed, v);
	const int ngl = (int)ch.glevel_ptr.size() - 1;
	const bool dist = chol_distributed(ctx, ch);
	const OwnFilter mine{ dist ? ch.col_owner : nullptr, dist ? ctx->comm->rank : 0 }, shared{ dist ? ch.col_owner : nullptr, -1 };
	auto sweep = [&](auto tag, const auto* Lx, const auto* Gx, const auto* Dx) {
		typedef decltype(tag) FT;
		if (!fwd_done)
		{
			if (ch.ntask0) hipLaunchKernelGGL(k_chol_fwd_tasks<FT>, dim3(ch.ntask0), dim3(128), chol_task_lds(ch), s, ch.task_ptr, ch.task_cols, ch.col_task, ch.col_lpos, 0, ch.colptr, ch.rowidx, Lx, Dx, v, mine);
			for (int phase = 0; phase < (dist ? 2 : 1); phase++)
			{
				if (phase == 1) comm_sum(ctx, v + (size_t)ch.first_shared * 6, ((size_t)ch.M - ch.first_shared) * 6, LSFM_DTYPE_F64);
				for (int l = 0; l < ngl; l++)
				{
					const int g0 = ch.glevel_ptr[l], ng = ch.glevel_ptr[l + 1] - g0;
					if (!ng || (dist && !(phase == 0 ? ch.glevel_owned[l] : ch.glevel_shared[l]))) continue;
					hipLaunchKernelGGL(k_sn_fwd<FT>, dim3(ng), dim3(SN_THREADS), 0, s, ch.grp_c0 + g0, ch.grp_s + g0, ch.grp_nr + g0, ch.colptr, ch.rowidx, Gx, Dx, v, ch.wv, phase == 0 ? mine : shared);
				}
			}
		}
		for (int phase = (dist ? 1 : 0); phase >= 0; phase--)
			for (int l = ngl - 1; l >= 0; l--)
			{
				const int g0 = ch.glevel_ptr[l], ng = ch.glevel_ptr[l + 1] - g0;
				if (!ng || (dist && !(phase == 0 ? ch.glevel_owned[l] : ch.glevel_shared[l]))) continue;
				hipLaunchKernelGGL(k_sn_bwd<FT>, dim3(ng), dim3(SN_THREADS), 0, s, ch.grp_c0 + g0, ch.grp_s + g0, ch.grp_nr + g0, ch.colptr, ch.rowidx, Gx, Dx, v, ch.wv, (dist && phase == 1) ? shared : mine);
			}
		if (ch.ntask0) hipLaunchKernelGGL(k_chol_bwd_tasks<FT>, dim3(ch.ntask0), dim3(128), chol_task_lds(ch), s, ch.task_ptr, ch.task_cols, ch.col_task, ch.col_lpos, 0, ch.colptr, ch.rowidx, Lx, Dx, v, mine);
	};
	if (ch.Lf) sweep(float(), (const float*)ch.Lf, (const float*)ch.Lgf, (const float*)ch.Dinvf);
	else sweep(double(), (const double*)ch.L, (const double*)ch.Lg, (const double*)ch.Dinv);
	if (dist)
	{
		hipLaunchKernelGGL(k_perm_out_dot, dim3((ch.M + 127) / 128), dim3(128), 0, s, ch.M, ch.pinv, v, r, fixed, ch.dscale, pose_seg, z, (double*)nullptr, dot_stride,
		                   ch.col_owner, ctx->comm->rank);
		ctx->comm->allreduce(s, z, (size_t)ch.M * 6, LSFM_DTYPE_F64);
		hipLaunchKernelGGL(k_rz_dot, dim3((ch.M + 127) / 128), dim3(128), 0, s, ch.M, z, r, pose_seg, dot, dot_stride);
	}
	else
		hipLaunchKernelGGL(k_perm_out_dot, dim3((ch.M + 127) / 128), dim3(128), 0, s, ch.M, ch.pinv, v, r, fixed, ch.dscale, pose_seg, z, dot, dot_stride, (const int*)nullptr, 0);
}

int chol_selftest(lsfm_context* ctx, int m, const int* rowptr, const int* colidx, const double* val, const int* origin, const unsigned char* fixed,
                  const int* pose_seg, int nseg, const double* r, int nrhs, int mode, double* z, double* dot, int* perm, int* colptr, int* rowidx,
                  double* L, double* Dinv, double* dscale, int cap_blocks, int* info)
{
	const int nnzb = rowptr[m];
	const size_t ns = (size_t)m * 6;
	CholHostIn hin;
	hin.keys.resize(nnzb);
	hin.origin.resize(m);
	for (int p = 0; p < m; p++)
	{
		hin.origin[p] = origin ? origin[p] : p;
		for (int k = rowptr[p]; k < rowptr[p + 1]; k++) hin.keys[k] = ((unsigned long long)(unsigned)p << 32) | (unsigned)colidx[k];
	}
	{
		CholSymbolic sym;
		chol_symbolic(hin.keys.data(), nnzb, hin.origin.data(), m, sym);
		info[0] = sym.nnzL;
		if (cap_blocks < sym.nnzL) LSFM_FAIL(LSFM_ERR_ARG, "rowidx / L too small for the factor (" + std::to_string(sym.nnzL) + " blocks)");
		ctx->ensure_arenas((size_t)sym.nnzL * 36 * 32 + (size_t)nnzb * 320 + ns * 8 * (16 + 2 * (size_t)nrhs) + ((size_t)64 << 20));
	}
	ctx->scratch.reset();
	Arena& sc = ctx->scratch;
	SchurSystem sy;
	sy.M = m; sy.nnzb = nnzb;
	unsigned long long* dk = sc.alloc<unsigned long long>(nnzb + 1);
	sy.S = sc.alloc<double>((size_t)nnzb * 36);
	sy.rowptr = sc.alloc<int>(m + 1);
	h2d(ctx, dk, hin.keys.data(), (size_t)nnzb * sizeof(unsigned long long));
	h2d(ctx, sy.S, val, (size_t)nnzb * 36 * sizeof(double));
	h2d(ctx, sy.rowptr, rowptr, (size_t)(m + 1) * sizeof(int));
	sy.upper_keys = dk;
	unsigned char* dfx = nullptr;
	if (fixed) { dfx = sc.alloc<unsigned char>(ns); h2d(ctx, dfx, fixed, ns); }
	int* dseg = sc.alloc<int>(m);
	h2d(ctx, dseg, pose_seg, (size_t)m * sizeof(int));
	double* dr = sc.alloc<double>(ns * nrhs);
	double* dz = sc.alloc<double>(ns * nrhs);
	double* ddot = sc.alloc<double>((size_t)nseg * nrhs);
	double* dv = sc.alloc<double>(ns);
	h2d(ctx, dr, r, ns * nrhs * sizeof(double));
	dev_zero(ctx, ddot, (size_t)nseg * nrhs * sizeof(double));
	CholDev ch;
	chol_analyse(ctx, sy, hin, ch);
	RunStatsDev* d_run = sc.alloc<RunStatsDev>(1);
	dev_zero(ctx, d_run, sizeof(RunStatsDev));
	const bool fused = (mode & 1) != 0;
	{
		struct Swap { lsfm_context* c; RunStatsDev* keep; ~Swap() { c->d_run = keep; } } swap{ ctx, ctx->d_run };
		ctx->d_run = d_run;
		chol_scatter(ctx, sy, dfx, ch);
		if (fused) chol_perm_in(ctx, ch, dr, dfx, dv);
		chol_factor(ctx, sy, dfx, ch, fused ? dv : nullptr);
	}
	if (mode & 2) chol_round_to_float(ctx, ch);
	for (int k = 0; k < nrhs; k++) chol_apply(ctx, ch, dr + ns * k, dv, dz + ns * k, dfx, dseg, ddot + (size_t)nseg * k, 1, fused && k == 0);
	chol_merge_groups(ctx, ch);
	LSFM_CHECK_HIP(hipGetLastError());
	RunStatsDev rs;
	d2h(ctx, &rs, d_run, sizeof rs);
	const int chol_err = d2h_int(ctx, ch.d_err);
	const int ngl = (int)ch.glevel_ptr.size() - 1;
	info[1] = ch.ntask0; info[2] = ch.ncol0; info[3] = ch.task0_outer; info[4] = ch.ngroups; info[5] = std::max(ngl, 0);
	info[6] = ch.sn_fused_levels; info[7] = ch.sn_split_levels;
	info[8] = ch.glevel_maxnr.empty() ? 0 : *std::max_element(ch.glevel_maxnr.begin(), ch.glevel_maxnr.end());
	info[9] = chol_err; info[10] = rs.floored;
	d2h(ctx, z, dz, ns * nrhs * sizeof(double));
	d2h(ctx, dot, ddot, (size_t)nseg * nrhs * sizeof(double));
	if (perm) d2h(ctx, perm, ch.perm, (size_t)m * sizeof(int));
	if (colptr) d2h(ctx, colptr, ch.colptr, (size_t)(m + 1) * sizeof(int));
	if (rowidx) d2h(ctx, rowidx, ch.rowidx, (size_t)ch.nnzL * sizeof(int));
	if (L) d2h(ctx, L, ch.L, (size_t)ch.nnzL * 36 * sizeof(double));
	if (Dinv) d2h(ctx, Dinv, ch.Dinv, (size_t)m * 36 * sizeof(double));
	if (dscale) d2h(ctx, dscale, ch.dscale, ns * sizeof(double));
	if (chol_err) LSFM_FAIL(LSFM_ERR_NOT_SPD, "the matrix is not positive definite (block column " + std::to_string(chol_err - 1) + " of the factor)");
	return LSFM_OK;
}

}
```

linearsfm_amd/csrc/lsfm_chol.hpp:

```cpp
#pragma once
#include <vector>

#include "lsfm_internal.hpp"
#include "lsfm_solve.hpp"

namespace lsfm {

struct CholDev {
	int M = 0, nnzL = 0, nlevels = 0, tail_begin = 0;
	int* colptr = nullptr;
	int* rowidx = nullptr;
	int* perm = nullptr;
	int* pinv = nullptr;
	int* order = nullptr;
	std::vector<int> level_ptr;
	int* task_cols = nullptr;
	int* task_ptr = nullptr;
	int* col_task = nullptr;
	int* col_lpos = nullptr;
	int* col_nin = nullptr;
	int ntask0 = 0, ncol0 = 0;
	int task0_maxsize = 0;
	int task0_lds = 0;
	int task0_outer = 0;
	int ngroups = 0;
	int *grp_c0 = nullptr, *grp_s = nullptr, *grp_nr = nullptr;
	std::vector<int> glevel_ptr;
	std::vector<int> glevel_maxnr;
	std::vector<int> glevel_maxs;
	int sn_fused_levels = 0, sn_split_levels = 0;
	int* col_owner = nullptr;
	int first_shared = 0, shared_blk0 = 0;
	double work_total = 0, work_shared = 0;
	std::vector<char> glevel_owned, glevel_shared;
	int* blob = nullptr;
	size_t blob_ints = 0;
	float *Lf = nullptr, *Dinvf = nullptr;
	double* wv = nullptr;
	double* Lg = nullptr;
	float* Lgf = nullptr;
	double* L = nullptr;
	double* Dinv = nullptr;
	double* diag0 = nullptr;
	double* dscale = nullptr;
	int* d_err = nullptr;
};

struct OwnFilter {
	const int* col_owner = nullptr;
	int want = 0;
	__device__ __forceinline__ bool skip(int col) const { return col_owner && col_owner[col] != want; }
};
__device__ __forceinline__ int find_row(const int* __restrict__ rowidx, int lo, int hi, int target)
{
	while (lo < hi) { int mid = (lo + hi) >> 1; if (rowidx[mid] < target) lo = mid + 1; else hi = mid; }
	return lo;
}


struct CholSymbolic;
struct CholHostIn {
	std::vector<unsigned long long> keys;
	std::vector<int> origin;
};

void chol_fetch(lsfm_context* ctx, const SchurSystem& sy, const int* d_origin, CholHostIn& in);
void chol_analyse(lsfm_context* ctx, const SchurSystem& sy, const CholHostIn& in, CholDev& ch);
void chol_upload_index(lsfm_context* ctx, const CholSymbolic& sym, CholDev& ch);
void chol_upload_symbolic(lsfm_context* ctx, const CholSymbolic& sym, CholDev& ch);
void chol_alloc_values(lsfm_context* ctx, CholDev& ch);
void chol_scatter(lsfm_context* ctx, const SchurSystem& sy, const unsigned char* fixed, CholDev& ch);
void chol_factor(lsfm_context* ctx, const SchurSystem& sy, const unsigned char* fixed, CholDev& ch, double* fwd_v = nullptr);
void chol_merge_groups(lsfm_context* ctx, const CholDev& ch);
void chol_round_to_float(lsfm_context* ctx, CholDev& ch);
void chol_perm_in(lsfm_context* ctx, const CholDev& ch, const double* r, const unsigned char* fixed, double* v);
void chol_apply(lsfm_context* ctx, const CholDev& ch, const double* r, double* v, double* z, const unsigned char* fixed, const int* pose_seg, double* dot, int dot_stride, bool fwd_done = false);
bool chol_distributed(const lsfm_context* ctx, const CholDev& ch);
void comm_sum_host(lsfm_context* ctx, long long* h, int n);

}
```

linearsfm_amd/csrc/lsfm_internal.hpp:

```cpp
#pragma once
#include <hip/hip_runtime.h>

#include <cstdint>
#include <cstdio>
#include <condition_variable>
#include <cstring>
#include <exception>
#include <functional>
#include <memory>
#include <mutex>
#include <thread>
#include <string>
#include <vector>

#include "../../include/lsfm.h"
#include "lsfm_map.hpp"

namespace lsfm {

struct Error { int code; std::string msg; };
struct DevBatch;
struct IndexHold;
struct SolvePlan;
struct PreLevel;
// ... 87 lines not shown
	int s_rebuild_mismatch;
	unsigned long long k2;
};

struct Comm {
	int rank = 0, world = 1;
	lsfm_allreduce_fn fn = nullptr;
	void* user = nullptr;
	char* buf = nullptr;
	size_t cap = 0, off = 256;
	int block_maps = 0;
	enum { HDR_BYTES = 256, KIND_DATA = 0, KIND_FINAL = 1 };
	bool broken = false;
	void restart() { off = HDR_BYTES; }
	void* alloc_bytes(size_t bytes)
	{
		const size_t a = (off + 255) & ~size_t(255);
		if (a + bytes > cap)
			throw Error{ LSFM_ERR_ARG, "the buffer handed to lsfm_tree_set_comm is too small (" + std::to_string(a + bytes) + " bytes needed, " + std::to_string(cap) + " given)" };
		off = a + bytes;
		return buf + a;
	}
	template <class T> T* alloc(size_t n) { return static_cast<T*>(alloc_bytes(n * sizeof(T))); }
	void allreduce(hipStream_t s, void* p, size_t count, int dtype, int kind = KIND_DATA);
	void call(hipStream_t s, size_t offset, size_t count, int dtype)
	{
		const int rc = fn(user, offset, count, dtype, (void*)s);
		if (rc) { broken = true; throw Error{ LSFM_ERR_INTERNAL, "the caller's all-reduce failed with code " + std::to_string(rc) }; }
	}
	bool follow(hipStream_t s);
};

struct HostWorker {
	std::thread th;
	std::mutex m;
	std::condition_variable cv;
	std::function<void()> job;
	std::exception_ptr err;
	bool busy = false, quit = false;
	~HostWorker()
	{
		{ std::lock_guard<std::mutex> l(m); quit = true; }
		cv.notify_all();
		if (th.joinable()) th.join();
	}
	void run(std::function<void()> f)
	{
		std::unique_lock<std::mutex> l(m);
		cv.wait(l, [&] { return !busy; });
		job = std::move(f); busy = true; err = nullptr;
		if (!th.joinable())
			th = std::thread([this] {
				std::unique_lock<std::mutex> lk(m);
				for (;;)
				{
					cv.wait(lk, [&] { return quit || (busy && job); });
					if (quit) return;
					std::function<void()> j = std::move(job);
					job = nullptr;
					lk.unlock();
					std::exception_ptr e;
					try { j(); } catch (...) { e = std::current_exception(); }
					lk.lock();
					err = e; busy = false;
					cv.notify_all();
				}
			});
		cv.notify_all();
	}
	void wait()
	{
		std::unique_lock<std::mutex> l(m);
		cv.wait(l, [&] { return !busy; });
		if (err) { std::exception_ptr e = err; err = nullptr; std::rethrow_exception(e); }
	}
};

}

namespace lsfm {
struct Roctx {
	int (*push)(const char*) = nullptr;
	int (*pop)() = nullptr;
	void (*mark)(const char*) = nullptr;
	Roctx();
};
Roctx& roctx();
struct Range {
	bool on;
	explicit Range(const char* name) : on(roctx().push != nullptr) { if (on) roctx().push(name); }
	~Range() { if (on) roctx().pop(); }
	Range(const Range&) = delete;
	Range& operator=(const Range&) = delete;
};
}

namespace lsfm {
enum Ord {
	evA,
	evB,
	evC_pairs,
	evC_runs,
	evY,
	evP,
	evU,
	evG,
	evT,
	evK9_fork,
	evK9_done,
	evR_fork,
	evR_done,
	ORD_COUNT
};
}

struct lsfm_context {
	int device = 0;
	hipStream_t stream = nullptr;
	lsfm::Arena arena[3];
	lsfm::Arena scratch;
	int cur = 0;
	size_t arena_bytes = 0, arena_req = 0;
	lsfm::PcgOptions pcg;
	int covcols_panel = 0;
	int small_max = 5;
	std::string last_error;
	int* h_pinned = nullptr;
	char* h_stage = nullptr;
	char* d_stage = nullptr;
	size_t stage_size = 0, stage_off = 0;
	hipEvent_t ev_half[2] = { nullptr, nullptr };
	unsigned long long generation = 0;
	hipStream_t stream2 = nullptr;
	hipEvent_t ord[lsfm::ORD_COUNT] = {};
	void quiesce_side_streams();
	std::shared_ptr<lsfm::EarlyPattern> early;
	hipStream_t stream3 = nullptr;
	lsfm::Arena sarena[2];
	std::shared_ptr<lsfm::PreLevel> pre;
	lsfm::LevelPlan pre_plan;
	int pre_plan_level = -1;
	std::unique_ptr<lsfm::HostWorker> worker;
	void drop_prepared() { pre.reset(); pre_plan = lsfm::LevelPlan(); pre_plan_level = -1; }
	double dbg_gap_ms = 0.0;
	std::vector<std::pair<const char*, double>> timeline;
	bool timeline_on = false;
	void mark(const char* what);
	bool in_tree_run = false;
	lsfm_stats* stats = nullptr;
	lsfm::LevelPlan* plan = nullptr;
	bool warm() const { return plan && plan->valid; }
	lsfm::RunStatsDev* d_run = nullptr;
	lsfm::Comm* comm = nullptr;
	std::vector<hipEvent_t> ev_pool;
	size_t ev_next = 0;
	struct Timed { hipEvent_t a, b; double* sink; };
	std::vector<Timed> timed;
	hipEvent_t pool_event();
	void defer_time(hipEvent_t a, hipEvent_t b, double* sink) { timed.push_back(Timed{ a, b, sink }); }
	void flush_times();
	void ensure_arenas(size_t bytes_each, bool start_small = false);
	bool grow_arenas();
	bool arena_small = false;
	size_t arena_bound = 0;
};

namespace lsfm {

struct OnStream {
	lsfm_context* c; hipStream_t& s; Arena* a;
	OnStream(lsfm_context* ctx, hipStream_t& other, Arena* arena = nullptr) : c(ctx), s(other), a(arena) { std::swap(c->stream, s); if (a) std::swap(c->scratch, *a); }
	~OnStream() { if (a) std::swap(c->scratch, *a); std::swap(c->stream, s); }
	OnStream(const OnStream&) = delete;
	OnStream& operator=(const OnStream&) = delete;
};
inline void wait_for(lsfm_context* ctx, hipStream_t s, Ord e) { LSFM_CHECK_HIP(hipStreamWaitEvent(s, ctx->ord[e], 0)); }
struct Fork {
	lsfm_context* c; hipStream_t main; OnStream on;
	Fork(lsfm_context* ctx, hipStream_t& side, Arena* arena = nullptr) : c(ctx), main(ctx->stream), on(ctx, side, arena) {}
	Fork(lsfm_context* ctx, hipStream_t& side, Ord start, bool record = true, Arena* arena = nullptr) : Fork(ctx, side, arena)
	{
		if (record) LSFM_CHECK_HIP(hipEventRecord(c->ord[start], main));
		wait_for(c, c->stream, start);
	}
	void done(Ord e) { LSFM_CHECK_HIP(hipEventRecord(c->ord[e], c->stream)); }
	void join(Ord e) { done(e); wait_for(c, main, e); }
};

void dev_exclusive_scan(lsfm_context* ctx, const int* in, int* out, size_t n);
void dev_sort_pairs_u64(lsfm_context* ctx, unsigned long long* keys, int* vals, size_t n, int end_bit, int begin_bit = 0);
void dev_sort_keys_u64(lsfm_context* ctx, const unsigned long long* keys, unsigned long long* sorted, size_t n, int begin_bit, int end_bit);
int d2h_int(lsfm_context* ctx, const int* dptr);
void d2h_ints(lsfm_context* ctx, const int* dptr, int* h, size_t n);
void h2d(lsfm_context* ctx, void* d, const void* h, size_t bytes);
struct HostPiece { const void* p; size_t bytes; };
void h2d_gather(lsfm_context* ctx, void* d, const std::vector<HostPiece>& pieces);
struct CopyBatch {
	lsfm_context* ctx;
	struct Item { void* dst; const void* src; size_t bytes; bool host; };
	std::vector<Item> items;
	explicit CopyBatch(lsfm_context* c) : ctx(c) {}
	void h2d(void* d, const void* h, size_t bytes) { if (bytes) items.push_back(Item{ d, h, bytes, true }); }
	void d2d(void* d, const void* s, size_t bytes) { if (bytes) items.push_back(Item{ d, s, bytes, false }); }
	void flush();
};
void d2h(lsfm_context* ctx, void* h, const void* d, size_t bytes);
void dev_zero(lsfm_context* ctx, void* d, size_t bytes);
void fill_async(hipStream_t s, void* d, int byte, size_t bytes);

void batch_upload(lsfm_context* ctx, Arena& ar, const lsfm_map* maps, int N, bool mono, DevBatch& out);
void batch_download_map(lsfm_context* ctx, const DevBatch& b, int k, bool mono, lsfm_map* out);
inline void map_new(lsfm_map& g, const lsfm_map* like, int m, int n, int nU, int nW, bool pose_origin)
{
	if (map_alloc(g, like, m, n, nU, nW, pose_origin) != LSFM_OK) throw Error{ LSFM_ERR_OOM, "out of host memory for the merged map" };
}
struct CopyBatch;
void batch_set_offsets(lsfm_context* ctx, Arena& ar, DevBatch& b, CopyBatch* cb = nullptr);
void batch_fill_maps(lsfm_context* ctx, DevBatch& b);
struct PackHeader {
	int magic, version, mono, m, n, nU, nW, Ref, FRef, ScaP, Fix, Sign, FScaP, FFix, pad0, pad1;
	unsigned long long total;
	unsigned long long off[12];
	unsigned long long pad[11];
};
static_assert(sizeof(PackHeader) == 256, "the header is the first 256 bytes of a pack");
#define LSFM_PACK_MAGIC 0x4d46534c
size_t pack_layout(PackHeader& h);
void batch_pack_map(lsfm_context* ctx, const DevBatch& b, int k, bool mono, void* dst, size_t cap);
void batch_slice_counts(lsfm_context* ctx, const DevBatch& b, int nslices, std::vector<int>& nf, std::vector<int>& nw);
void batch_pack_slice(lsfm_context* ctx, const DevBatch& b, bool mono, int nslices, int slice, int nf, int nw, void* dst, size_t cap);
void batch_unpack_maps(lsfm_context* ctx, Arena& ar, const void* const* packed, const PackHeader* hdr, int N, bool mono, DevBatch& out);
unsigned long long batch_structure_digest(lsfm_context* ctx, const DevBatch& b);

inline bool map_in_frame(const DevBatch& X, int b, int tref, int tscap, bool mono) { return X.Ref[b] == tref && (!mono || X.ScaP[b] == tscap); }
int level_targets(const DevBatch& X, bool mono, std::vector<int>& tref, std::vector<int>& tscap, std::vector<int>& tfix);
struct TrRedirect {
	const int* wbase = nullptr;
	const int* newf = nullptr;
	double* W = nullptr;
	int *photo = nullptr, *feature = nullptr, *srcf = nullptr;
};
using TrHook = std::function<TrRedirect(DevBatch& mid, const int* hub)>;
void transform_batch(lsfm_context* ctx, Arena& ar, const DevBatch& in, const std::vector<int>& target_ref,
                     const std::vector<int>& target_scap, const std::vector<int>& target_fix, bool mono, DevBatch& out,
                     bool alias_passthrough = false, const TrHook* hook = nullptr);

struct JoinWork;
struct SolveIO {
	int M = 0, NF = 0, NU = 0, NW = 0, nseg = 0;
	const int* d_pose_seg = nullptr;
	const int* d_feat_seg = nullptr;
	const unsigned char* d_seg_active = nullptr;
	const double* U = nullptr; const int *Ui = nullptr, *Uj = nullptr;
	const double* W = nullptr; const int *photo = nullptr, *fptr = nullptr;
	const double* V = nullptr;
	const double* ea = nullptr;
	const double* eb = nullptr;
	const double* x0 = nullptr;
	const unsigned char* d_fixed = nullptr;
	const int* d_pose_origin = nullptr;
	double* x_pose = nullptr;
	double* x_feat = nullptr;
	std::vector<int> seg_rows;
	const int *d_pose_off = nullptr, *d_feat_off = nullptr, *d_u_off = nullptr;
	const struct RhsFused* rhs = nullptr;
	const struct PatternSeed* seed = nullptr;
	bool index_arrays_at_evA = false;
	int step_hint = 0;
	bool caller_syncs = false;
};
struct SolveOutcome {
	int not_converged = 0;
	int steps_used = 0;
	const unsigned long long* keys = nullptr;
	int nnzb = 0;
	hipEvent_t end = nullptr;
};
int small_level_strips(const lsfm_context* ctx, int most_rows);
inline int most_rows(const std::vector<int>& seg_rows) { int most = 0; for (int r : seg_rows) most = r > most ? r : most; return most; }
inline int small_level_strips(const lsfm_context* ctx, const std::vector<int>& seg_rows) { return small_level_strips(ctx, most_rows(seg_rows)); }
void small_level_offsets(lsfm_context* ctx, const DevBatch& out, SolveIO& io);
void small_solve_launch(lsfm_context* ctx, const SolveIO& io, int strips, int* status, double* max_rel);
struct HostSystem;
int small_selftest(lsfm_context* ctx, int G, const int* pose_off, const int* feat_off, const int* u_off, const unsigned char* active, const HostSystem& h,
                   const unsigned char* fixed, int strips, double* x_pose, double* x_feat, int* status, double* max_rel);
SolveOutcome solve_batch(lsfm_context* ctx, const SolveIO& io);
SolveOutcome join_batch_stereo(lsfm_context* ctx, Arena& ar, const DevBatch& in, DevBatch& out, double* eP_out, double* eF_out, int step_hint = 0);
SolveOutcome join_batch_mono(lsfm_context* ctx, Arena& ar, const DevBatch& in, DevBatch& out, double* eP_out, double* eF_out, int step_hint = 0);
int gn_polish(lsfm_context* ctx, const lsfm_map* maps, int N, bool mono, lsfm_map* x, int iters, int kind, double c, double* obj, double* gnorm,
              int* halvings, double* chi2, double* weight);
int map_feature_chi2(lsfm_context* ctx, const lsfm_map* maps, int N, bool mono, const lsfm_map* x, double* fchi2, double* pose_chi2);
int gn_polish_features(lsfm_context* ctx, const lsfm_map* maps, int N, bool mono, lsfm_map* x, int iters, int kind, double c, double* obj, double* gnorm,
                       int* halvings, double* fchi2, double* fweight);
int map_chi2(lsfm_context* ctx, const lsfm_map* maps, int N, bool mono, const lsfm_map* x, double* chi2, int* dof);
int gn_linearise(lsfm_context* ctx, const lsfm_map* maps, int N, bool mono, const lsfm_map* x, const double* weight, lsfm_map* out, double* obj,
                 double* b, double* times, int* counts);
int map_covariance(lsfm_context* ctx, const lsfm_map* map, bool mono, double* pose_cov, double* feat_cov, double* pair_cov, int cap_blocks, int* nnzb,
                   double* times);
int map_covariance_columns(lsfm_context* ctx, const lsfm_map* map, bool mono, const int* poses, int k, double* pose_cols, double* feat_cols, double* joint,
                           int* steps, double* last_corr, double* times);
int map_covariance_feature_columns(lsfm_context* ctx, const lsfm_map* map, bool mono, const int* feats, int k, double* pose_cols, double* feat_cols,
                                   double* joint, int* steps, double* last_corr, double* times);
int map_feature_pair_gate(lsfm_context* ctx, const lsfm_map* map, bool mono, const int* pairs, int K, double* d2, double* cov_diff, int* steps,
                          double* last_corr, double* times);
int map_feature_pair_joint_gate(lsfm_context* ctx, const lsfm_map* map, bool mono, const int* pairs, int K, const int* order, double tau, int* status,
                                double* delta, double* d2, double* joint_C, int* accepted, int* implied, double* D2, int* steps, double* last_corr, double* times);
// ... 26 lines not shown
```

linearsfm_amd/csrc/lsfm_level.hip:

```cpp
#include <algorithm>
#include <chrono>
#include <cmath>
#include <cstdlib>

#include "lsfm_device.hpp"
#include "lsfm_symbolic.hpp"
#include "lsfm_pcg.hpp"

namespace lsfm {

struct SolvePlan {
	SchurSystem sy;
	CholDev ch;
	int its = 1;
	bool mixed = false;
	double rel_tol = 0;
	bool small = false;
	char* mem = nullptr;
	~SolvePlan() { if (mem) (void)hipFree(mem); }
};
static std::shared_ptr<SolvePlan> solve_plan_store(lsfm_context* ctx, const SchurSystem& sy, const CholDev& ch, int its)
{
	auto sp = std::make_shared<SolvePlan>();
	const size_t M = sy.M, nnzb = sy.nnzb, cap = (size_t)sy.mask + 1;
	if (getenv("LSFM_DEBUG") && sy.k9.ns && sy.k9_tiles > 0)
	{
		std::vector<int> h(sy.k9_tiles);
		d2h(ctx, h.data(), sy.k9.ns, sizeof(int) * h.size());
		int b16 = 0, b32 = 0, b48 = 0, b64 = 0, b96 = 0, more = 0;
		for (int v : h) { const int n = v < 0 ? -v : v; (n <= 16 ? b16 : n <= 32 ? b32 : n <= 48 ? b48 : n <= 64 ? b64 : n <= 96 ? b96 : more)++; }
		fprintf(stderr, "[lsfm] Schur tiles by poses: <=16 %d, <=32 %d, <=48 %d, <=64 %d, <=96 %d, more (or > 64 distinct: hash full) %d\n", b16, b32, b48, b64, b96, more);
	}
	struct Item { const void* src; size_t bytes; void** dst; };
	SolvePlan& P = *sp;
	P.sy = sy; P.ch = ch; P.its = its; P.mixed = ch.Lf != nullptr; P.rel_tol = ctx->pcg.rel_tol;
	P.sy.S = nullptr; P.sy.E = nullptr; P.sy.IV = nullptr;
	P.ch.L = nullptr; P.ch.Dinv = nullptr; P.ch.diag0 = nullptr; P.ch.dscale = nullptr; P.ch.Lg = nullptr; P.ch.Lgf = nullptr; P.ch.d_err = nullptr; P.ch.wv = nullptr; P.ch.Lf = nullptr; P.ch.Dinvf = nullptr;
	std::vector<Item> items = {
		{ sy.rowptr, (M + 1) * 4, (void**)&P.sy.rowptr }, { sy.colidx, (nnzb + 1) * 4, (void**)&P.sy.colidx },
		{ sy.upper_keys, nnzb * 8, (void**)&P.sy.upper_keys }, { sy.longrows, (M + 1) * 4, (void**)&P.sy.longrows },
		{ sy.d_nlong, 4, (void**)&P.sy.d_nlong }, { sy.tab, cap * 8, (void**)&P.sy.tab }, { sy.hval, cap * 4, (void**)&P.sy.hval },
		{ ch.blob, ch.blob_ints * 4, (void**)&P.ch.blob },
		{ sy.gent, sy.gent ? nnzb * 16 : 0, (void**)&P.sy.gent }, { sy.goth, sy.goth ? nnzb * 8 : 0, (void**)&P.sy.goth },
		{ sy.k9.ns, sy.k9.ns ? (size_t)sy.k9_tiles * 4 : 0, (void**)&P.sy.k9.ns }, { sy.k9.pose, sy.k9.pose ? (size_t)sy.k9_tiles * 64 * 4 : 0, (void**)&P.sy.k9.pose },
		{ sy.k9.eslot, sy.k9.eslot ? (size_t)sy.k9_NW : 0, (void**)&P.sy.k9.eslot },
		{ sy.k9.wlist, sy.k9.wlist ? (size_t)sy.k9_tiles * 3 * 4 : 0, (void**)&P.sy.k9.wlist }, { sy.k9.wcnt, sy.k9.wcnt ? (size_t)32 : (size_t)0, (void**)&P.sy.k9.wcnt },
	};
	size_t total = 0;
	for (const Item& it : items) total += (it.bytes + 255) & ~(size_t)255;
	LSFM_CHECK_HIP(hipMalloc((void**)&P.mem, total + 256));
	size_t off = 0;
	for (const Item& it : items)
	{
		if (it.bytes) LSFM_CHECK_HIP(hipMemcpyAsync(P.mem + off, it.src, it.bytes, hipMemcpyDeviceToDevice, ctx->stream));
		*it.dst = it.src ? P.mem + off : nullptr;
		off += (it.bytes + 255) & ~(size_t)255;
	}
	const ptrdiff_t shift = (char*)P.ch.blob - (char*)ch.blob;
	auto rebase = [&](int*& p) { if (p) p = (int*)((char*)p + shift); };
	rebase(P.ch.colptr); rebase(P.ch.rowidx); rebase(P.ch.perm); rebase(P.ch.pinv); rebase(P.ch.order); rebase(P.ch.task_cols);
	rebase(P.ch.task_ptr); rebase(P.ch.col_task); rebase(P.ch.col_lpos); rebase(P.ch.col_nin); rebase(P.ch.grp_c0); rebase(P.ch.grp_s);
	rebase(P.ch.grp_nr); rebase(P.ch.col_owner);
	LSFM_CHECK_HIP(hipStreamSynchronize(ctx->stream));
	return sp;
}

struct PreLevel {
	SchurSystem sy;
	CholSymbolic sym;
	CholHostIn hin;
	int M = 0;
	HostWorker* worker = nullptr;
	bool whole = false;
	int level = -1, its = 0;
	void wait()
	{
		HostWorker* w = worker;
		worker = nullptr;
		if (w) w->wait();
	}
	~PreLevel() { try { wait(); } catch (...) {} }
};
void prefetch_next_level(lsfm_context* ctx, const DevBatch& Y, const std::vector<int>& target_ref, int next_level, int step_hint,
                         const unsigned long long* level_keys, int level_nnzb)
{
	ctx->drop_prepared();
	if (!Y.M || Y.B < 2) return;
	int most_next = 0;
	for (int b = 0; b < Y.B; b += 2) most_next = std::max(most_next, Y.pose_off[std::min(b + 2, Y.B)] - Y.pose_off[b]);
	const bool next_small = small_level_strips(ctx, most_next) > 0;
	const bool whole = step_hint > 0 && !getenv("LSFM_CHECK_EARLY_PATTERN");
	if (next_small && !whole) return;
	ctx->mark("pre_start");
	auto pl = std::make_shared<PreLevel>();
	pl->M = Y.M;
	Arena& sa = ctx->sarena[next_level & 1];
	sa.reset();
	std::vector<int> counts;
	LevelIndex kept;
	bool ok = false;
	{
		Fork side(ctx, ctx->stream3, evY, false, &sa);
		if (ctx->timeline_on) { (void)hipEventSynchronize(ctx->ord[evY]); ctx->mark("pre_evY"); }
		int* d_tref = ctx->scratch.alloc<int>(Y.B);
		h2d(ctx, d_tref, target_ref.data(), sizeof(int) * (size_t)Y.B);
		ok = schur_pattern_prefetch(ctx, Y, d_tref, level_keys, level_nnzb, pl->sy, whole ? &counts : nullptr, !next_small, whole ? &kept : nullptr);
		if (ok)
		{
			if (!next_small) chol_fetch(ctx, pl->sy, Y.pose_origin, pl->hin);
			side.done(evP);
		}
	}
	ctx->mark("pre_pat");
	if (!ok) return;
	if (!next_small)
	{
		if (!ctx->worker) ctx->worker.reset(new HostWorker());
		PreLevel* raw = pl.get();
		ctx->worker->run([raw]() { chol_symbolic(raw->hin.keys.data(), raw->sy.nnzb, raw->hin.origin.data(), raw->sy.M, raw->sym); });
		pl->worker = ctx->worker.get();
		ctx->mark("pre_sym");
		pl->whole = whole; pl->level = next_level; pl->its = step_hint;
		ctx->pre = pl;
	}
	if (!whole) return;
	const int B = Y.B;
	ctx->pre_plan.tr_cnt.assign(counts.begin(), counts.begin() + 2 * (B + 1));
	ctx->pre_plan.join_rb.assign(counts.begin() + 2 * (B + 1), counts.end());
	ctx->pre_plan.solve.reset();
	ctx->pre_plan.idx = kept;
	ctx->pre_plan.valid = true;
	ctx->pre_plan_level = next_level;
	ctx->mark("pre_plan");
}
static std::shared_ptr<SolvePlan> pre_plan_complete(lsfm_context* ctx, PreLevel& pl)
{
	pl.wait();
	auto sp = std::make_shared<SolvePlan>();
	sp->sy = pl.sy;
	sp->its = pl.its; sp->mixed = ctx->pcg.mixed; sp->rel_tol = ctx->pcg.rel_tol;
	{
		Fork side(ctx, ctx->stream3, &ctx->sarena[pl.level & 1]);
		chol_upload_index(ctx, pl.sym, sp->ch);
		side.join(evP);
	}
	return sp;
}

__global__ void k_dbg_absstats(size_t n, const double* __restrict__ a, double* __restrict__ out)
{
	double s = 0.0, m = 0.0;
	for (size_t i = (size_t)blockIdx.x * blockDim.x + threadIdx.x; i < n; i += (size_t)gridDim.x * blockDim.x)
	{
		const double v = fabs(a[i]);
		s += v; if (v > m || !(v == v)) m = v == v ? v : 1e300;
	}
	atomic_add_f64(out, s);
	atomicMax(reinterpret_cast<unsigned long long*>(out + 1), (unsigned long long)__double_as_longlong(m));
}
__global__ void k_dbg_dinv(int M, const double* __restrict__ Dinv, const double* __restrict__ diag0, const int* __restrict__ colptr, int first_group_col)
{
	int j = blockIdx.x * blockDim.x + threadIdx.x;
	if (j >= M) return;
	double m = 0.0;
	for (int q = 0; q < 36; q++) m = fmax(m, fabs(Dinv[(size_t)j * 36 + q]));
	if (m > 1e3 || !(m == m))
		printf("[lsfm conv] column %d (%s, %d blocks): max |Dinv| %.3e, Dinv diag %.3e %.3e %.3e %.3e %.3e %.3e, diag0 %.3e %.3e %.3e %.3e %.3e %.3e\n", j,
		       j >= first_group_col ? "group" : "leaf", colptr[j + 1] - colptr[j], m, Dinv[(size_t)j * 36], Dinv[(size_t)j * 36 + 7], Dinv[(size_t)j * 36 + 14],
		       Dinv[(size_t)j * 36 + 21], Dinv[(size_t)j * 36 + 28], Dinv[(size_t)j * 36 + 35], diag0[j * 6], diag0[j * 6 + 1], diag0[j * 6 + 2], diag0[j * 6 + 3],
		       diag0[j * 6 + 4], diag0[j * 6 + 5]);
}
__global__ void k_digest(size_t n, const unsigned long long* __restrict__ a, unsigned long long* out)
{
	unsigned long long h = 0;
	for (size_t i = (size_t)blockIdx.x * blockDim.x + threadIdx.x; i < n; i += (size_t)gridDim.x * blockDim.x)
	{
		unsigned long long b = a[i];
		if (b == 0x8000000000000000ull) b = 0;
		b ^= b >> 31; b *= 0x9E3779B97F4A7C15ull * (2 * (unsigned long long)i + 1); b ^= b >> 29;
		h += b;
	}
	atomicAdd(out, h);
}
__global__ void k_digest_compare(const unsigned long long* d, int* mismatch)
{
	if (d[0] != d[1]) atomicAdd(mismatch, 1);
}
__global__ void k_chol_err_to_run(const int* err, RunStatsDev* run)
{
	if (*err && !run->chol_err) run->chol_err = *err;
}

struct LevelStructure {
	SchurSystem sy;
	CholDev ch;
	SolvePlan* sp = nullptr;
	double tw0 = 0, tw1 = 0;
};
static double wall_ms() { return std::chrono::duration<double, std::milli>(std::chrono::steady_clock::now().time_since_epoch()).count(); }
static LevelStructure level_structure(lsfm_context* ctx, const SolveIO& io, SolvePlan* sp, PreLevel* pre, bool pending, hipEvent_t eb)
{
	hipStream_t s = ctx->stream;
	LevelStructure ls;
	SchurSystem& sy = ls.sy;
	CholDev& ch = ls.ch;
	auto assemble = [&]() {
		build_schur_values(ctx, io, sy);
		LSFM_REC_T(eb, s); if (roctx().mark) roctx().mark("lsfm factor + refine: begin");
	};
	if (sp || pending)
	{
		sy = pending ? pre->sy : sp->sy;
		schur_vinv(ctx, io, sy);
		assemble();
		if (pending)
// ... 259 lines not shown
```

linearsfm_amd/csrc/lsfm_symbolic.cpp:

```cpp
#include "lsfm_symbolic.hpp"

#include <algorithm>
#include <chrono>
#include <cstdio>
#include <cstring>
#include <cstdlib>
#include <condition_variable>
#include <functional>
#include <mutex>
#include <queue>
#include <thread>
#include <utility>

namespace lsfm {
static int sym_threads()
{
	static const int cap = getenv("LSFM_SYM_THREADS") ? std::max(1, atoi(getenv("LSFM_SYM_THREADS"))) : 8;
	return std::min<int>(cap, std::max(1u, std::thread::hardware_concurrency() / 2));
}
static const int gs_cap = []() { const char* e = getenv("LSFM_GS"); const int v = e ? atoi(e) : CHOL_GS; return v >= 1 && v <= CHOL_GS ? v : CHOL_GS; }();


namespace {

// ... 504 lines not shown
				for (int t = rcnt[k]; t < rcnt[k + 1]; t++)
					for (int i = radj[t]; mark[i] != k; i = parent[i]) { rowidx[colptr[i] + w.cfill[i]++] = k; mark[i] = k; }
			});
		});
	}
	const int nnzL = colptr[M];
	ch.work_total = ch.work_shared = 0;
	for (int j = 0; j < M; j++)
	{
		const double w = 0.5 * (double)ccount[j] * (ccount[j] + 1);
		ch.work_total += w;
		if (j >= ch.first_shared) ch.work_shared += w;
	}
	tick("column patterns");
	std::vector<int>& lev = w.lev;
	lev.assign(M, 0);
	int nlev = 0;
	for (int j = 0; j < M; j++)
	{
		if (parent[j] >= 0) lev[parent[j]] = std::max(lev[parent[j]], lev[j] + 1);
		nlev = std::max(nlev, lev[j] + 1);
	}
	std::vector<int>& lcount = w.lcount;
	lcount.assign(nlev + 1, 0);
	for (int j = 0; j < M; j++) lcount[lev[j] + 1]++;
	int tail_level = nlev;
	while (tail_level > 0 && lcount[tail_level] <= 2) tail_level--;
	for (int l = 0; l < nlev; l++) lcount[l + 1] += lcount[l];
	std::vector<int>& order = ch.order;
	order.resize(M);
	w.lfill.assign(nlev, 0);
	for (int j = 0; j < M; j++) order[lcount[lev[j]] + w.lfill[lev[j]]++] = j;
	ch.M = M; ch.nnzL = nnzL; ch.nlevels = tail_level;
	ch.level_ptr.assign(lcount.begin(), lcount.begin() + tail_level + 1);
	ch.tail_begin = lcount[tail_level];
	std::sort(order.begin() + ch.tail_begin, order.end());
	static const int task_x = std::min(std::max(getenv("LSFM_TASK_X") ? atoi(getenv("LSFM_TASK_X")) : 90, 1), CHOL_TASK_X_MAX);
	static_assert(CHOL_TASK_X_MAX * CHOL_TASK_LDS_PER_COL + 8 <= CHOL_SOLVE_LDS && (CHOL_TASK_X_MAX + 1) * CHOL_TASK_LDS_PER_COL + 8 > CHOL_SOLVE_LDS &&
	              CHOL_TASK_X_MAX * (288 + 4) + (5 * CHOL_TASK_X_MAX + 1) * 4 + 16 <= CHOL_FACTOR_LDS, "CHOL_TASK_X_MAX");
	ch.task_x = task_x;
	std::vector<int>&size = w.size, &ntc = w.ntc, &topchild = w.topchild, &task = w.task, &tlev = w.tlev;
	size.assign(ccount.begin(), ccount.end());
	ntc.assign(M, 0); topchild.assign(M, -1); task.assign(M, -1); tlev.clear();
	for (int j = 0; j < M; j++) if (parent[j] >= 0) size[parent[j]] += size[j];
	for (int j = ch.first_shared; j < M; j++) size[j] = std::max(size[j], task_x + 1);
	for (int j = 0; j < M; j++)
		if (size[j] > task_x && parent[j] >= 0) { ntc[parent[j]]++; topchild[parent[j]] = j; }
	int ntasks = 0;
	for (int j = 0; j < M; j++)
	{
		if (size[j] <= task_x) continue;
		if (ntc[j] == 1) { task[j] = task[topchild[j]]; continue; }
		task[j] = ntasks++;
		tlev.push_back(1);
	}
	for (int j = 0; j < M; j++)
	{
		if (size[j] <= task_x) continue;
		const int pj = parent[j];
		if (pj >= 0 && task[pj] != task[j]) tlev[task[pj]] = std::max(tlev[task[pj]], tlev[task[j]] + 1);
	}
	for (int j = M - 1; j >= 0; j--)
	{
		if (size[j] > task_x) continue;
		const int pj = parent[j];
		if (pj >= 0 && size[pj] <= task_x) task[j] = task[pj];
		else { task[j] = ntasks++; tlev.push_back(0); }
	}
	int ntl = 0;
	for (int t = 0; t < ntasks; t++) ntl = std::max(ntl, tlev[t] + 1);
	std::vector<int> tl_count(ntl + 1, 0), tpos(ntasks), tsize(ntasks, 0);
	for (int t = 0; t < ntasks; t++) tl_count[tlev[t] + 1]++;
	for (int l = 0; l < ntl; l++) tl_count[l + 1] += tl_count[l];
	std::vector<long> tblocks(ntasks, 0), tcolsn(ntasks, 0);
	for (int j = 0; j < M; j++) { tblocks[task[j]] += ccount[j]; tcolsn[task[j]]++; }
	auto task_lds = [&](int t) { return tblocks[t] * (288 + 4) + (5 * tcolsn[t] + 1) * 4 + 16; };
	const long small_cap = CHOL_FACTOR_LDS;
	ch.tlevel_nsmall.assign(ntl, 0);
	ch.tlevel_small_lds.assign(ntl, 0);
	{
		std::vector<int> f(ntl, 0);
		for (int pass = 0; pass < 2; pass++)
			for (int t = 0; t < ntasks; t++)
			{
				const bool small = task_lds(t) <= small_cap;
				if (small != (pass == 0)) continue;
				tpos[t] = tl_count[tlev[t]] + f[tlev[t]]++;
				if (small) { ch.tlevel_nsmall[tlev[t]]++; ch.tlevel_small_lds[tlev[t]] = std::max(ch.tlevel_small_lds[tlev[t]], (int)task_lds(t)); }
			}
	}
	for (int j = 0; j < M; j++) tsize[tpos[task[j]]]++;
	std::vector<int>&tptr = ch.task_ptr, &tcols = ch.task_cols;
	tptr.assign(ntasks + 1, 0); tcols.resize(M);
	std::vector<int> tf(ntasks, 0);
	for (int t = 0; t < ntasks; t++) tptr[t + 1] = tptr[t] + tsize[t];
	for (int j = 0; j < M; j++) { const int t = tpos[task[j]]; tcols[tptr[t] + tf[t]++] = j; }
	ch.tlevel_ptr = tl_count;
	ch.tlevel_maxsize.assign(ntl, 0);
	std::vector<int>&ctask = ch.col_task, &clpos = ch.col_lpos;
	ctask.resize(M); clpos.resize(M);
	for (int t = 0; t < ntasks; t++)
		for (int k = tptr[t]; k < tptr[t + 1]; k++) { ctask[tcols[k]] = t; clpos[tcols[k]] = k - tptr[t]; }
	for (int l = 0; l < ntl; l++)
		for (int t = tl_count[l]; t < tl_count[l + 1]; t++) ch.tlevel_maxsize[l] = std::max(ch.tlevel_maxsize[l], tsize[t]);
	ch.tlevel_col0.assign(ntl + 1, 0);
	for (int l = 0; l <= ntl; l++) ch.tlevel_col0[l] = tptr[tl_count[l]];
	std::vector<int>& nin = ch.col_nin;
	nin.assign(M, 0);
	ch.tlevel_outer.assign(ntl, 0);
	for (int j = 0; j < M; j++)
	{
		int m = 0;
		while (colptr[j] + 1 + m < colptr[j + 1] && task[rowidx[colptr[j] + 1 + m]] == task[j]) m++;
		nin[j] = m;
		const int no = ccount[j] - 1 - m, l = tlev[task[j]];
		ch.tlevel_outer[l] = std::max(ch.tlevel_outer[l], no * (no + 1) / 2);
	}
	tick("levels + tasks");
	{
		std::vector<int> grp(M, -1), gc0, gs, glev;
		for (int j = 0; j < M; j++)
		{
			if (size[j] <= task_x) continue;
			const bool join = j > 0 && size[j - 1] > task_x && parent[j - 1] == j && ccount[j - 1] == ccount[j] + 1 && gs[grp[j - 1]] < gs_cap &&
			                  j != ch.first_shared;
			if (join) { grp[j] = grp[j - 1]; gs[grp[j]]++; }
			else { grp[j] = (int)gc0.size(); gc0.push_back(j); gs.push_back(1); glev.push_back(0); }
		}
		const int ng = (int)gc0.size();
		int ngl = 0;
		for (int g = 0; g < ng; g++)
		{
			const int pj = parent[gc0[g] + gs[g] - 1];
			if (pj >= 0) glev[grp[pj]] = std::max(glev[grp[pj]], glev[g] + 1);
			ngl = std::max(ngl, glev[g] + 1);
		}
		std::vector<int> gl_count(ngl + 1, 0), gfill(ngl, 0);
		ch.grp_c0.resize(ng); ch.grp_s.resize(ng); ch.grp_nr.resize(ng);
		for (int g = 0; g < ng; g++) gl_count[glev[g] + 1]++;
		for (int l = 0; l < ngl; l++) gl_count[l + 1] += gl_count[l];
		ch.glevel_maxnr.assign(ngl, 0);
		ch.glevel_maxs.assign(ngl, 1);
		for (int g = 0; g < ng; g++)
		{
			const int at = gl_count[glev[g]] + gfill[glev[g]]++;
			ch.grp_c0[at] = gc0[g]; ch.grp_s[at] = gs[g]; ch.grp_nr[at] = ccount[gc0[g] + gs[g] - 1] - 1;
			ch.glevel_maxnr[glev[g]] = std::max(ch.glevel_maxnr[glev[g]], ch.grp_nr[at]);
			ch.glevel_maxs[glev[g]] = std::max(ch.glevel_maxs[glev[g]], gs[g]);
		}
		ch.ngroups = ng;
		ch.glevel_ptr = gl_count;
		ch.glevel_owned.assign(ngl, 0); ch.glevel_shared.assign(ngl, 0);
		for (int g = 0; g < ng; g++) (gc0[g] >= ch.first_shared ? ch.glevel_shared : ch.glevel_owned)[glev[g]] = 1;
	}
	tick("groups");
}

}

#include "../../include/lsfm.h"

extern "C" int lsfm_symbolic_analyse(int m, const int* rowptr, const int* colidx, const int* origin, int reps, int* perm, int* colptr, int* rowidx,
                                     int cap, int* info, double* avg_ms)
{
	if (m <= 0 || !rowptr || !colidx || rowptr[0] != 0) return LSFM_ERR_ARG;
	const int nnzb = rowptr[m];
	std::vector<unsigned long long> keys((size_t)nnzb);
	for (int p = 0; p < m; p++)
	{
		if (rowptr[p + 1] <= rowptr[p] || colidx[rowptr[p]] != p) return LSFM_ERR_ARG;
		for (int k = rowptr[p]; k < rowptr[p + 1]; k++)
		{
			if (colidx[k] < p || colidx[k] >= m || (k > rowptr[p] && colidx[k] <= colidx[k - 1])) return LSFM_ERR_ARG;
			keys[k] = ((unsigned long long)(unsigned)p << 32) | (unsigned)colidx[k];
		}
	}
	std::vector<int> org(m);
	for (int p = 0; p < m; p++) org[p] = origin ? origin[p] : p;
	lsfm::CholSymbolic sym;
	if (reps < 1) reps = 1;
	lsfm::chol_symbolic(keys.data(), nnzb, org.data(), m, sym);
	const auto t0 = std::chrono::steady_clock::now();
	for (int r = 0; r < reps; r++) lsfm::chol_symbolic(keys.data(), nnzb, org.data(), m, sym);
	if (avg_ms) *avg_ms = std::chrono::duration<double, std::milli>(std::chrono::steady_clock::now() - t0).count() / reps;
	if (info)
	{
		int height = 0, nsep = 0;
		{
			std::vector<int> lev(m, 0);
			for (int j = 0; j < m; j++)
			{
				if (sym.parent[j] >= 0) lev[sym.parent[j]] = std::max(lev[sym.parent[j]], lev[j] + 1);
				height = std::max(height, lev[j] + 1);
			}
			for (int j = 0; j < m; j++) nsep += sym.col_task[j] >= (sym.tlevel_ptr.size() > 1 ? sym.tlevel_ptr[1] : 0);
		}
		info[0] = sym.nnzL; info[1] = height; info[2] = sym.ngroups; info[3] = (int)sym.glevel_ptr.size() - 1;
		info[4] = sym.tlevel_ptr.size() > 1 ? sym.tlevel_ptr[1] : 0; info[5] = nsep; info[6] = 0; info[7] = 0;
	}
	if (perm) memcpy(perm, sym.perm.data(), (size_t)m * sizeof(int));
	if (colptr) memcpy(colptr, sym.colptr.data(), (size_t)(m + 1) * sizeof(int));
	if (rowidx)
	{
		if (cap < sym.nnzL) return LSFM_ERR_ARG;
		memcpy(rowidx, sym.rowidx.data(), (size_t)sym.nnzL * sizeof(int));
	}
	return LSFM_OK;
}
```

linearsfm_amd/csrc/lsfm_symbolic.hpp:

```cpp
#pragma once
#include <vector>

namespace lsfm {

#define CHOL_GS 8

#define CHOL_TASK_LDS_PER_COL (6 * 8 + 36 * 8 + 3 * 4)
#define CHOL_SOLVE_LDS (56 * 1024)
#define CHOL_FACTOR_LDS (60 * 1024)
#define CHOL_TASK_X_MAX 164

struct CholSymbolic {
	int M = 0, nnzL = 0, nlevels = 0, tail_begin = 0;
	std::vector<int> colptr, rowidx, perm, pinv, order, level_ptr;
	std::vector<int> task_cols, task_ptr, col_task, col_lpos, col_nin;
	std::vector<int> tlevel_ptr, tlevel_maxsize, tlevel_col0, tlevel_nsmall, tlevel_small_lds, tlevel_outer;
	int ngroups = 0;
	std::vector<int> grp_c0, grp_s, grp_nr, glevel_ptr, glevel_maxnr, glevel_maxs;
	std::vector<int> parent, ccount;
	int task_x = 0;
	std::vector<int> col_owner;
	int first_shared = 0;
	std::vector<char> glevel_owned, glevel_shared;
	double work_total = 0, work_shared = 0;
};

void chol_symbolic(const unsigned long long* keys, int nnzb, const int* origin, int M, CholSymbolic& out, int block_maps = 0);

}
```

Baseline: 29.62.

## Fuse top levels of supernodal backward solve into per-chain persistent tail kernel

Adds a symbolic pass that finds the top group levels of the elimination forest whose groups form small chains (bounded rows and columns per tree). A new kernel then runs each chain's backward triangular solve in one block, keeping solved values in LDS and double-buffering the next group's L, Dinv and RHS loads behind the current group's compute. This replaces many tiny per-level launches and global round trips at the top of the tree. The cost is more LDS per block, extra symbolic bookkeeping, and it is disabled in distributed runs.

```diff
diff --git a/include/lsfm.h b/include/lsfm.h
--- a/include/lsfm.h
+++ b/include/lsfm.h
@@ -165,6 +165,9 @@
 int lsfm_symbolic_analyse(int m, const int* rowptr, const int* colidx, const int* origin, int reps, int* perm, int* colptr, int* rowidx,
                           int cap, int* info, double* avg_ms);
 
+int lsfm_symbolic_tail(int nlevels, const int* glevel_ptr, const int* glevel_maxnr, const int* grp_parent, const int* grp_s, int* level,
+                       int* nchains, int* chain_ptr, int* chain_grp, int* nsingle, int* single);
+
 typedef struct lsfm_tree lsfm_tree;
 int lsfm_tree_upload(lsfm_context* ctx, const lsfm_map* maps, int N, int mono, lsfm_tree** out);
 int lsfm_tree_run(lsfm_context* ctx, lsfm_tree* tree, lsfm_stats* stats);
@@ -234,6 +237,9 @@
                        const int* pose_seg, int nseg, const double* r, int nrhs, int mode, double* z, double* dot, int* perm, int* colptr, int* rowidx,
                        double* L, double* Dinv, double* dscale, int cap_blocks, int* info);
 
+#define LSFM_SELFTEST_CHOL_TAIL_INFO 8
+int lsfm_selftest_chol_tail(lsfm_context* ctx, int* info);
+
 int lsfm_selftest_transform(lsfm_context* ctx, const lsfm_map* maps, int N, int mono, const int* tref, const int* tscap, const int* tfix,
                             int alias_passthrough, lsfm_map* out);
 
diff --git a/linearsfm_amd/api.py b/linearsfm_amd/api.py
--- a/linearsfm_amd/api.py
+++ b/linearsfm_amd/api.py
@@ -166,6 +166,8 @@
         L.lsfm_selftest_prims.argtypes = [vp, C.c_int, C.c_uint]
         L.lsfm_selftest_chol.argtypes = [vp, C.c_int, ip, ip, dp, ip, P(C.c_ubyte), ip, C.c_int, dp, C.c_int, C.c_int, dp, dp, ip, ip, ip, dp, dp, dp,
                                          C.c_int, ip]
+        L.lsfm_selftest_chol_tail.argtypes = [vp, ip]
+        L.lsfm_symbolic_tail.argtypes = [C.c_int, ip, ip, ip, ip, ip, ip, ip, ip, ip, ip]
         L.lsfm_selftest_transform.argtypes = [vp, P(LsfmMap), C.c_int, C.c_int, ip, ip, ip, C.c_int, P(LsfmMap)]
         L.lsfm_selftest_small.argtypes = [vp, C.c_int, ip, ip, ip, ub, dp, ip, ip, dp, ip, ip, C.c_int, dp, dp, dp, dp, ub, C.c_int, dp, dp, ip, dp]
         _LIB = L
@@ -179,7 +181,7 @@
            "lsfm_tree_upload_dev", "lsfm_tree_reload_dev", "lsfm_tree_set_comm", "lsfm_tree_set_comm_blocks", "lsfm_tree_export_slice_sizes", "lsfm_tree_export_slice_dev",
            "lsfm_tree_free", "lsfm_divide_conquer", "lsfm_read_localmap", "lsfm_read_localmaps", "lsfm_write_localmap", "lsfm_write_mapset", "lsfm_mapset_info", "lsfm_mapset_stamp", "lsfm_read_mapset", "lsfm_save_state_bin", "lsfm_save_state", "lsfm_save_poses", "lsfm_gn_polish",
            "lsfm_gn_polish_robust", "lsfm_map_chi2", "lsfm_map_feature_chi2", "lsfm_gn_polish_robust_features", "lsfm_gn_linearise", "lsfm_gn_linearise_timed",
-           "lsfm_spmv_bench", "lsfm_wstream_bench", "lsfm_selftest_prims", "lsfm_selftest_chol", "lsfm_selftest_transform", "lsfm_selftest_small", "lsfm_schur_pattern", "lsfm_symbolic_analyse", "lsfm_inverse_v", "lsfm_selftest_vinv", "lsfm_solve_features",
+           "lsfm_spmv_bench", "lsfm_wstream_bench", "lsfm_selftest_prims", "lsfm_selftest_chol", "lsfm_selftest_chol_tail", "lsfm_symbolic_tail", "lsfm_selftest_transform", "lsfm_selftest_small", "lsfm_schur_pattern", "lsfm_symbolic_analyse", "lsfm_inverse_v", "lsfm_selftest_vinv", "lsfm_solve_features",
            "lsfm_map_covariance", "lsfm_map_covariance_timed",
            "lsfm_save_covariances", "lsfm_read_covariances",
            "lsfm_map_covariance_columns", "lsfm_map_covariance_columns_timed", "lsfm_save_cov_columns", "lsfm_read_cov_columns",
@@ -853,6 +855,17 @@
 
 
 Context.selftest_chol = _selftest_chol
+
+SELFTEST_CHOL_TAIL_INFO = ("tail_level", "chains", "chain_groups", "longest_chain", "single_groups", "tail_launches")
+
+
+def _selftest_chol_tail(self):
+    info = np.zeros(8, np.int32)
+    self._check(lib().lsfm_selftest_chol_tail(self._h, _ptr(info, C.c_int)), "lsfm_selftest_chol_tail")
+    return dict(zip(SELFTEST_CHOL_TAIL_INFO, (int(v) for v in info)))
+
+
+Context.selftest_chol_tail = _selftest_chol_tail
 
 
 def _selftest_transform(self, dicts, mono, targets, alias=False):
@@ -929,6 +942,21 @@
     return dict(perm=perm, colptr=colptr, rowidx=rowidx[:int(info[0])], info=info, ms=ms.value)
 
 
+def symbolic_tail(glevel_ptr, glevel_maxnr, grp_parent, grp_s=None):
+    glevel_ptr = _c(glevel_ptr, np.int32); glevel_maxnr = _c(glevel_maxnr, np.int32); grp_parent = _c(grp_parent, np.int32)
+    ng = len(grp_parent)
+    grp_s = _c(grp_s, np.int32) if grp_s is not None else np.ones(ng, np.int32)
+    if len(glevel_ptr) != len(glevel_maxnr) + 1 or len(grp_s) != ng or (len(glevel_ptr) and glevel_ptr[-1] != ng):
+        raise LsfmError("symbolic_tail: the arrays do not fit together")
+    lev, nch, nsg = C.c_int(), C.c_int(), C.c_int()
+    cp = np.zeros(ng + 1, np.int32); cg = np.zeros(ng + 1, np.int32); sg = np.zeros(ng + 1, np.int32)
+    rc = lib().lsfm_symbolic_tail(len(glevel_maxnr), _ptr(glevel_ptr, C.c_int), _ptr(glevel_maxnr, C.c_int), _ptr(grp_parent, C.c_int),
+                                  _ptr(grp_s, C.c_int), C.byref(lev), C.byref(nch), _ptr(cp, C.c_int), _ptr(cg, C.c_int), C.byref(nsg), _ptr(sg, C.c_int))
+    if rc:
+        raise LsfmError(f"lsfm_symbolic_tail failed (rc={rc}): malformed forest")
+    return dict(level=lev.value, chains=[cg[cp[c]:cp[c + 1]].tolist() for c in range(nch.value)], single=sg[:nsg.value].tolist())
+
+
 MARG_POSES_INFO = ("dropped", "boundary", "components", "blocks", "chunks", "leaf_tasks", "groups", "group_levels")
 
 
diff --git a/linearsfm_amd/csrc/lsfm_capi.hip b/linearsfm_amd/csrc/lsfm_capi.hip
--- a/linearsfm_amd/csrc/lsfm_capi.hip
+++ b/linearsfm_amd/csrc/lsfm_capi.hip
@@ -729,6 +729,13 @@
 	});
 }
 
+int lsfm_selftest_chol_tail(lsfm_context* ctx, int* info)
+{
+	if (!ctx || !info) return LSFM_ERR_ARG;
+	for (int i = 0; i < LSFM_SELFTEST_CHOL_TAIL_INFO; i++) info[i] = ctx->chol_tail_info[i];
+	return LSFM_OK;
+}
+
 int lsfm_selftest_transform(lsfm_context* ctx, const lsfm_map* maps, int N, int mono, const int* tref, const int* tscap, const int* tfix,
                             int alias_passthrough, lsfm_map* out)
 {
diff --git a/linearsfm_amd/csrc/lsfm_chol.hip b/linearsfm_amd/csrc/lsfm_chol.hip
--- a/linearsfm_amd/csrc/lsfm_chol.hip
+++ b/linearsfm_amd/csrc/lsfm_chol.hip
@@ -1059,6 +1059,54 @@
 	}
 }
 
+template <class XF, class BF>
+__device__ __forceinline__ void sn_bwd_rows(int s, int nr, XF xrow, BF blk, double* sZ)
+{
+	const int tid = threadIdx.x, sub = tid & 3;
+	for (int i = tid >> 2; i < nr; i += SN_THREADS / 4)
+	{
+		double x6[6];
+		ld<6>(x6, xrow(i));
+		for (int t = sub; t < s; t += 4)
+		{
+			double b[36];
+			ld<36>(b, blk(i, t));
+#pragma unroll
+			for (int c = 0; c < 6; c++)
+			{
+				double o = 0.0;
+#pragma unroll
+				for (int r = 0; r < 6; r++) o = fma(b[r * 6 + c], x6[r], o);
+				lds_add_f64(&sZ[6 * t + c], -o);
+			}
+		}
+	}
+}
+__device__ __forceinline__ void sn_bwd_columns(int s, const double* Ls, const double* sDi, const double* sZ, double* sA, double* sX)
+{
+	const int tid = threadIdx.x, n6 = 6 * s;
+	double acc = tid < n6 ? sZ[tid] : 0.0;
+	for (int t = s - 1; t >= 0; t--)
+	{
+		const int k0 = 6 * t;
+		if (tid >= k0 && tid < k0 + 6) sA[tid - k0] = acc;
+		__syncthreads();
+		if (tid >= k0 && tid < k0 + 6)
+		{
+			const int c = tid - k0;
+			double x = 0.0;
+			for (int k = c; k < 6; k++) x = fma(sDi[t * 36 + k * 6 + c], sA[k], x);
+			sX[tid] = x;
+		}
+		__syncthreads();
+		if (tid < k0)
+		{
+#pragma unroll
+			for (int k = 0; k < 6; k++) acc = fma(-Ls[(k0 + k) * SN_XS + tid], sX[k0 + k], acc);
+		}
+	}
+}
+
 template <class FT>
 __global__ void __launch_bounds__(SN_THREADS) k_sn_bwd(const int* __restrict__ grp_c0, const int* __restrict__ grp_s, const int* __restrict__ grp_nr,
                                                         const int* __restrict__ colptr, const int* __restrict__ rowidx, const FT* __restrict__ L,
@@ -1075,49 +1123,131 @@
 	if (tid < n6) sZ[tid] = w[(size_t)c0 * 6 + tid];
 	sn_load_diag(s, c0, colptr, L, Ls, sSrc, sDst, sCol);
 	const int rows0 = colptr[c0 + s - 1] + 1;
-	const int sub = tid & 3;
-	for (int i = tid >> 2; i < nr; i += SN_THREADS / 4)
-	{
-		const double* xr = v + (size_t)rowidx[rows0 + i] * 6;
-		double x6[6];
-		ld<6>(x6, xr);
-		for (int t = sub; t < s; t += 4)
-		{
-			const FT* blk = L + ((size_t)sCol[t] + (s - t) + i) * 36;
-			double b[36];
-			ld<36>(b, blk);
-#pragma unroll
-			for (int c = 0; c < 6; c++)
-			{
-				double o = 0.0;
-#pragma unroll
-				for (int r = 0; r < 6; r++) o = fma(b[r * 6 + c], x6[r], o);
-				lds_add_f64(&sZ[6 * t + c], -o);
-			}
-		}
-	}
+	sn_bwd_rows(s, nr, [&](int i) { return v + (size_t)rowidx[rows0 + i] * 6; },
+	            [&](int i, int t) { return L + ((size_t)sCol[t] + (s - t) + i) * 36; }, sZ);
 	__syncthreads();
-	double acc = tid < n6 ? sZ[tid] : 0.0;
-	for (int t = s - 1; t >= 0; t--)
-	{
-		const int k0 = 6 * t;
-		if (tid >= k0 && tid < k0 + 6) sA[tid - k0] = acc;
-		__syncthreads();
-		if (tid >= k0 && tid < k0 + 6)
-		{
-			const int c = tid - k0;
-			double x = 0.0;
-			for (int k = c; k < 6; k++) x = fma(sDi[t * 36 + k * 6 + c], sA[k], x);
-			sX[tid] = x;
-		}
-		__syncthreads();
-		if (tid < k0)
-		{
-#pragma unroll
-			for (int k = 0; k < 6; k++) acc = fma(-Ls[(k0 + k) * SN_XS + tid], sX[k0 + k], acc);
-		}
-	}
+	sn_bwd_columns(s, Ls, sDi, sZ, sA, sX);
 	if (tid < n6) v[(size_t)c0 * 6 + tid] = sX[tid];
+}
+
+static_assert(CHOL_TAIL_NR == SN_RB, "the tail takes the levels of one pair set of the fused panel kernel");
+#define SNT_BUF (6 * CHOL_GS * SN_XS + CHOL_GS * 36 + CHOL_TAIL_NR * CHOL_GS * 36 + 6 * CHOL_GS)
+#define SNT_LOADERS (SN_THREADS - 64)
+#define SNT_BLOCKS (CHOL_GS * (CHOL_GS + 1) / 2 + CHOL_TAIL_NR * CHOL_GS + CHOL_GS)
+static_assert(SNT_BLOCKS <= SNT_LOADERS, "one loader lane per block of a member's table");
+#define SNT_NPF ((SNT_BLOCKS * 18 + SNT_LOADERS - 1) / SNT_LOADERS)
+static size_t sn_tail_lds(int chain_cols) { return ((size_t)2 * SNT_BUF + (size_t)6 * chain_cols) * sizeof(double); }
+template <class FT>
+__global__ void __launch_bounds__(SN_THREADS) k_sn_tail_bwd(const int* __restrict__ chain_ptr, const int* __restrict__ recs, const FT* __restrict__ L,
+                                                             const FT* __restrict__ Dinv, double* __restrict__ v, const double* __restrict__ w)
+{
+	extern __shared__ double Ms[];
+	__shared__ double sA[6], sZ[6 * CHOL_GS], sX[6 * CHOL_GS];
+	__shared__ int sRec[4][CHOL_TAIL_REC], sTab[2][2 * SNT_BLOCKS], sTabN[2][4];
+	typedef typename SnPair<FT>::T Pair;
+	const int tid = threadIdx.x, lt = tid - 64;
+	const int m0 = chain_ptr[blockIdx.x], len = chain_ptr[blockIdx.x + 1] - m0;
+	double* const sXc = Ms + 2 * SNT_BUF;
+	auto buf_Ls = [&](int b) { return Ms + b * SNT_BUF; };
+	auto buf_Di = [&](int b) { return Ms + b * SNT_BUF + 6 * CHOL_GS * SN_XS; };
+	auto buf_Xp = [&](int b) { return Ms + b * SNT_BUF + 6 * CHOL_GS * SN_XS + CHOL_GS * 36; };
+	auto buf_W = [&](int b) { return Ms + b * SNT_BUF + 6 * CHOL_GS * SN_XS + CHOL_GS * 36 + CHOL_TAIL_NR * CHOL_GS * 36; };
+	Pair val[SNT_NPF];
+	int dst[SNT_NPF];
+	double2 wval = make_double2(0.0, 0.0);
+	int wdst = -1;
+	auto table = [&](const int* rc, int* tb, int* tn) {
+		const int c0 = rc[0], s = rc[1], nr = rc[2], nb = s * (s + 1) / 2, npb = nr * s, e = lt;
+		if (e < nb)
+		{
+			int t = 0;
+			while (sn_idx(s, s - 1, t) < e) t++;
+			const int u = t + (e - sn_idx(s, t, t));
+			tb[e] = (rc[4 + t] + (u - t)) * 36;
+			tb[SNT_BLOCKS + e] = 6 * u * SN_XS + 6 * t;
+		}
+		else if (e < nb + npb)
+		{
+			const int ee = e - nb, i = ee / s, t = ee - i * s;
+			tb[e] = (rc[4 + t] + (s - t) + i) * 36;
+			tb[SNT_BLOCKS + e] = 6 * CHOL_GS * SN_XS + CHOL_GS * 36 + ee * 36;
+		}
+		else if (e < nb + npb + s)
+		{
+			const int ee = e - nb - npb;
+			tb[e] = (c0 + ee) * 36;
+			tb[SNT_BLOCKS + e] = 6 * CHOL_GS * SN_XS + ee * 36;
+		}
+		if (e == 0) { tn[0] = nb; tn[1] = nb + npb; tn[2] = nb + npb + s; tn[3] = c0; }
+	};
+	auto issue = [&](const int* tb, const int* tn) {
+		const int nb = tn[0], nl = tn[1], nt = tn[2], c0 = tn[3];
+#pragma unroll
+		for (int j = 0; j < SNT_NPF; j++)
+		{
+			const int q = j * SNT_LOADERS + lt, e = q / 18, w2 = 2 * (q - e * 18);
+			dst[j] = -1;
+			if (e < nt)
+			{
+				const FT* src = (e < nl ? L : Dinv) + (size_t)tb[e] + w2;
+				val[j] = *reinterpret_cast<const Pair*>(src);
+				dst[j] = tb[SNT_BLOCKS + e] + (e < nb ? (w2 / 6) * SN_XS + w2 % 6 : w2);
+			}
+		}
+		wdst = -1;
+		if (lt < 3 * (nt - nl)) { wval = *reinterpret_cast<const double2*>(w + (size_t)c0 * 6 + 2 * lt); wdst = 2 * lt; }
+	};
+	auto put = [&](int b) {
+		double* const base = Ms + b * SNT_BUF;
+#pragma unroll
+		for (int j = 0; j < SNT_NPF; j++)
+			if (dst[j] >= 0) { base[dst[j]] = (double)val[j].x; base[dst[j] + 1] = (double)val[j].y; }
+		if (wdst >= 0) { double* const W = buf_W(b); W[wdst] = wval.x; W[wdst + 1] = wval.y; }
+	};
+	{
+		const int wv = tid >> 6, l = tid & 63;
+		if (wv < 3 && wv < len && l < CHOL_TAIL_REC) sRec[(len - 1 - wv) & 3][l] = recs[(size_t)(m0 + len - 1 - wv) * CHOL_TAIL_REC + l];
+	}
+	__syncthreads();
+	if (tid >= 64)
+	{
+		table(sRec[(len - 1) & 3], sTab[(len - 1) & 1], sTabN[(len - 1) & 1]);
+		if (len >= 2) table(sRec[(len - 2) & 3], sTab[(len - 2) & 1], sTabN[(len - 2) & 1]);
+	}
+	__syncthreads();
+	if (tid >= 64) { issue(sTab[(len - 1) & 1], sTabN[(len - 1) & 1]); put(0); }
+	__syncthreads();
+	int rnext;
+	for (int k = len - 1; k >= 0; k--)
+	{
+		const int cur = (len - 1 - k) & 1;
+		const int* rc = sRec[k & 3];
+		if (tid >= 64)
+		{
+			if (k >= 1) issue(sTab[(k - 1) & 1], sTabN[(k - 1) & 1]);
+			if (k >= 3 && lt < CHOL_TAIL_REC) rnext = recs[(size_t)(m0 + k - 3) * CHOL_TAIL_REC + lt];
+		}
+		const int c0 = rc[0], s = rc[1], nr = rc[2], n6 = 6 * s;
+		if (tid < n6) sZ[tid] = buf_W(cur)[tid];
+		__syncthreads();
+		const double* const Xp = buf_Xp(cur);
+		sn_bwd_rows(s, nr, [&](int i) { return sXc + 6 * rc[4 + CHOL_GS + i]; }, [&](int i, int t) { return Xp + (i * s + t) * 36; }, sZ);
+		__syncthreads();
+		sn_bwd_columns(s, buf_Ls(cur), buf_Di(cur), sZ, sA, sX);
+		if (tid < n6)
+		{
+			const double x = sX[tid];
+			v[(size_t)c0 * 6 + tid] = x;
+			sXc[6 * rc[3] + tid] = x;
+		}
+		if (tid >= 64)
+		{
+			if (k >= 1) put(cur ^ 1);
+			if (k >= 2) table(sRec[(k - 2) & 3], sTab[k & 1], sTabN[k & 1]);
+			if (k >= 3 && lt < CHOL_TAIL_REC) sRec[(k - 3) & 3][lt] = rnext;
+		}
+		__syncthreads();
+	}
 }
 
 __global__ void k_to_float(size_t n, const double* __restrict__ a, float* __restrict__ b)
@@ -1212,12 +1342,22 @@
 			                                 " fit, " + std::to_string(ch.task0_maxsize) + " columns at most)");
 	}
 	ch.ngroups = sym.ngroups; ch.glevel_ptr = sym.glevel_ptr; ch.glevel_maxnr = sym.glevel_maxnr; ch.glevel_maxs = sym.glevel_maxs;
+	ch.gtail_level = sym.gtail.level; ch.gtail_chains = (int)sym.gtail.chain_ptr.size() - 1; ch.gtail_groups = (int)sym.gtail.chain_grp.size();
+	ch.gtail_singles = (int)sym.gtail.single.size(); ch.gtail_longest = ch.gtail_cols = 0;
+	for (int c = 0; c < ch.gtail_chains; c++)
+	{
+		int cols = 0;
+		for (int k = sym.gtail.chain_ptr[c]; k < sym.gtail.chain_ptr[c + 1]; k++) cols += sym.grp_s[sym.gtail.chain_grp[k]];
+		ch.gtail_cols = std::max(ch.gtail_cols, cols);
+		ch.gtail_longest = std::max(ch.gtail_longest, sym.gtail.chain_ptr[c + 1] - sym.gtail.chain_ptr[c]);
+	}
 	ch.work_total = sym.work_total; ch.work_shared = sym.work_shared;
 	ch.first_shared = sym.first_shared; ch.shared_blk0 = sym.colptr[sym.first_shared]; ch.glevel_owned = sym.glevel_owned; ch.glevel_shared = sym.glevel_shared;
 	const struct { int** dst; const std::vector<int>* v; } parts[] = {
 		{ &ch.grp_c0, &sym.grp_c0 }, { &ch.grp_s, &sym.grp_s }, { &ch.grp_nr, &sym.grp_nr }, { &ch.col_nin, &sym.col_nin }, { &ch.col_task, &sym.col_task },
 		{ &ch.col_lpos, &sym.col_lpos }, { &ch.task_cols, &sym.task_cols }, { &ch.task_ptr, &sym.task_ptr }, { &ch.colptr, &sym.colptr },
-		{ &ch.rowidx, &sym.rowidx }, { &ch.perm, &sym.perm }, { &ch.pinv, &sym.pinv }, { &ch.order, &sym.order }, { &ch.col_owner, &sym.col_owner } };
+		{ &ch.rowidx, &sym.rowidx }, { &ch.perm, &sym.perm }, { &ch.pinv, &sym.pinv }, { &ch.order, &sym.order }, { &ch.col_owner, &sym.col_owner },
+		{ &ch.gtail_ptr, &sym.gtail.chain_ptr }, { &ch.gtail_rec, &sym.gtail_rec }, { &ch.gtail_single, &sym.gtail_single } };
 	size_t total = 0;
 	for (const auto& pt : parts) total += pt.v->size();
 	static thread_local std::vector<int> blob;
@@ -1258,6 +1398,11 @@
 bool chol_distributed(const lsfm_context* ctx, const CholDev& ch)
 {
 	return ctx->comm && ctx->comm->world > 1 && ch.col_owner && ch.first_shared < ch.M;
+}
+bool chol_tail_on(const lsfm_context* ctx, const CholDev& ch)
+{
+	static const bool on = !(getenv("LSFM_SN_TAIL") && atoi(getenv("LSFM_SN_TAIL")) == 0);
+	return on && !ctx->comm && ch.gtail_chains > 0;
 }
 static void comm_sum(lsfm_context* ctx, void* p, size_t count, int dtype)
 {
@@ -1386,6 +1531,13 @@
 	const int ngl = (int)ch.glevel_ptr.size() - 1;
 	const bool dist = chol_distributed(ctx, ch);
 	const OwnFilter mine{ dist ? ch.col_owner : nullptr, dist ? ctx->comm->rank : 0 }, shared{ dist ? ch.col_owner : nullptr, -1 };
+	const bool tail = chol_tail_on(ctx, ch);
+	static const bool tail_lds_set = []() {
+		(void)hipFuncSetAttribute(reinterpret_cast<const void*>(&k_sn_tail_bwd<double>), hipFuncAttributeMaxDynamicSharedMemorySize, (int)sn_tail_lds(CHOL_TAIL_COLS));
+		(void)hipFuncSetAttribute(reinterpret_cast<const void*>(&k_sn_tail_bwd<float>), hipFuncAttributeMaxDynamicSharedMemorySize, (int)sn_tail_lds(CHOL_TAIL_COLS));
+		return true;
+	}();
+	(void)tail_lds_set;
 	auto sweep = [&](auto tag, const auto* Lx, const auto* Gx, const auto* Dx) {
 		typedef decltype(tag) FT;
 		if (!fwd_done)
@@ -1402,8 +1554,15 @@
 				}
 			}
 		}
+		if (tail)
+		{
+			hipLaunchKernelGGL(k_sn_tail_bwd<FT>, dim3(ch.gtail_chains), dim3(SN_THREADS), sn_tail_lds(ch.gtail_cols), s, ch.gtail_ptr, ch.gtail_rec, Gx, Dx, v, ch.wv);
+			if (ch.gtail_singles)
+				hipLaunchKernelGGL(k_sn_bwd<FT>, dim3(ch.gtail_singles), dim3(SN_THREADS), 0, s, ch.gtail_single, ch.gtail_single + ch.gtail_singles,
+				                   ch.gtail_single + 2 * ch.gtail_singles, ch.colptr, ch.rowidx, Gx, Dx, v, ch.wv, mine);
+		}
 		for (int phase = (dist ? 1 : 0); phase >= 0; phase--)
-			for (int l = ngl - 1; l >= 0; l--)
+			for (int l = (tail ? ch.gtail_level : ngl) - 1; l >= 0; l--)
 			{
 				const int g0 = ch.glevel_ptr[l], ng = ch.glevel_ptr[l + 1] - g0;
 				if (!ng || (dist && !(phase == 0 ? ch.glevel_owned[l] : ch.glevel_shared[l]))) continue;
@@ -1490,6 +1649,11 @@
 	info[6] = ch.sn_fused_levels; info[7] = ch.sn_split_levels;
 	info[8] = ch.glevel_maxnr.empty() ? 0 : *std::max_element(ch.glevel_maxnr.begin(), ch.glevel_maxnr.end());
 	info[9] = chol_err; info[10] = rs.floored;
+	{
+		const bool tail = chol_tail_on(ctx, ch);
+		const int ti[8] = { ch.gtail_level, tail ? ch.gtail_chains : 0, tail ? ch.gtail_groups : 0, tail ? ch.gtail_longest : 0, tail ? ch.gtail_singles : 0, tail ? nrhs : 0, 0, 0 };
+		std::copy(ti, ti + 8, ctx->chol_tail_info);
+	}
 	d2h(ctx, z, dz, ns * nrhs * sizeof(double));
 	d2h(ctx, dot, ddot, (size_t)nseg * nrhs * sizeof(double));
 	if (perm) d2h(ctx, perm, ch.perm, (size_t)m * sizeof(int));
diff --git a/linearsfm_amd/csrc/lsfm_chol.hpp b/linearsfm_amd/csrc/lsfm_chol.hpp
--- a/linearsfm_amd/csrc/lsfm_chol.hpp
+++ b/linearsfm_amd/csrc/lsfm_chol.hpp
@@ -28,6 +28,8 @@
 	std::vector<int> glevel_ptr;
 	std::vector<int> glevel_maxnr;
 	std::vector<int> glevel_maxs;
+	int gtail_level = 0, gtail_chains = 0, gtail_groups = 0, gtail_longest = 0, gtail_singles = 0, gtail_cols = 0;
+	int *gtail_ptr = nullptr, *gtail_rec = nullptr, *gtail_single = nullptr;
 	int sn_fused_levels = 0, sn_split_levels = 0;
 	int* col_owner = nullptr;
 	int first_shared = 0, shared_blk0 = 0;
@@ -75,6 +77,7 @@
 void chol_round_to_float(lsfm_context* ctx, CholDev& ch);
 void chol_perm_in(lsfm_context* ctx, const CholDev& ch, const double* r, const unsigned char* fixed, double* v);
 void chol_apply(lsfm_context* ctx, const CholDev& ch, const double* r, double* v, double* z, const unsigned char* fixed, const int* pose_seg, double* dot, int dot_stride, bool fwd_done = false);
+bool chol_tail_on(const lsfm_context* ctx, const CholDev& ch);
 bool chol_distributed(const lsfm_context* ctx, const CholDev& ch);
 void comm_sum_host(lsfm_context* ctx, long long* h, int n);
 
diff --git a/linearsfm_amd/csrc/lsfm_internal.hpp b/linearsfm_amd/csrc/lsfm_internal.hpp
--- a/linearsfm_amd/csrc/lsfm_internal.hpp
+++ b/linearsfm_amd/csrc/lsfm_internal.hpp
@@ -263,6 +263,7 @@
 	bool warm() const { return plan && plan->valid; }
 	lsfm::RunStatsDev* d_run = nullptr;
 	lsfm::Comm* comm = nullptr;
+	int chol_tail_info[8] = { 0 };
 	std::vector<hipEvent_t> ev_pool;
 	size_t ev_next = 0;
 	struct Timed { hipEvent_t a, b; double* sink; };
diff --git a/linearsfm_amd/csrc/lsfm_level.hip b/linearsfm_amd/csrc/lsfm_level.hip
--- a/linearsfm_amd/csrc/lsfm_level.hip
+++ b/linearsfm_amd/csrc/lsfm_level.hip
@@ -60,7 +60,7 @@
 	auto rebase = [&](int*& p) { if (p) p = (int*)((char*)p + shift); };
 	rebase(P.ch.colptr); rebase(P.ch.rowidx); rebase(P.ch.perm); rebase(P.ch.pinv); rebase(P.ch.order); rebase(P.ch.task_cols);
 	rebase(P.ch.task_ptr); rebase(P.ch.col_task); rebase(P.ch.col_lpos); rebase(P.ch.col_nin); rebase(P.ch.grp_c0); rebase(P.ch.grp_s);
-	rebase(P.ch.grp_nr); rebase(P.ch.col_owner);
+	rebase(P.ch.grp_nr); rebase(P.ch.col_owner); rebase(P.ch.gtail_ptr); rebase(P.ch.gtail_rec); rebase(P.ch.gtail_single);
 	LSFM_CHECK_HIP(hipStreamSynchronize(ctx->stream));
 	return sp;
 }
diff --git a/linearsfm_amd/csrc/lsfm_symbolic.cpp b/linearsfm_amd/csrc/lsfm_symbolic.cpp
--- a/linearsfm_amd/csrc/lsfm_symbolic.cpp
+++ b/linearsfm_amd/csrc/lsfm_symbolic.cpp
@@ -680,8 +680,97 @@
 		ch.glevel_ptr = gl_count;
 		ch.glevel_owned.assign(ngl, 0); ch.glevel_shared.assign(ngl, 0);
 		for (int g = 0; g < ng; g++) (gc0[g] >= ch.first_shared ? ch.glevel_shared : ch.glevel_owned)[glev[g]] = 1;
+		std::vector<int>& gat = glev;
+		std::fill(gfill.begin(), gfill.end(), 0);
+		for (int g = 0; g < ng; g++) { const int l = glev[g]; gat[g] = gl_count[l] + gfill[l]++; }
+		ch.grp_parent.assign(ng, -1);
+		for (int g = 0; g < ng; g++)
+		{
+			const int pj = parent[gc0[g] + gs[g] - 1];
+			if (pj >= 0) ch.grp_parent[gat[g]] = gat[grp[pj]];
+		}
+		chol_tail_chains(ch.glevel_ptr, ch.glevel_maxnr, ch.grp_parent, ch.grp_s, ch.gtail);
+		const CholTail& tl = ch.gtail;
+		ch.gtail_rec.assign(tl.chain_grp.size() * CHOL_TAIL_REC, -1);
+		std::vector<int> slot(tl.chain_grp.empty() ? 0 : M, -1);
+		bool closed = true;
+		for (size_t c = 0; c + 1 < tl.chain_ptr.size(); c++)
+		{
+			const int b = tl.chain_ptr[c], e = tl.chain_ptr[c + 1];
+			int off = 0;
+			for (int k = b; k < e; k++)
+			{
+				const int g = tl.chain_grp[k];
+				for (int t = 0; t < ch.grp_s[g]; t++) slot[ch.grp_c0[g] + t] = off++;
+			}
+			for (int k = b; k < e; k++)
+			{
+				const int g = tl.chain_grp[k], c0 = ch.grp_c0[g], s = ch.grp_s[g], nr = ch.grp_nr[g];
+				int* rec = &ch.gtail_rec[(size_t)k * CHOL_TAIL_REC];
+				rec[0] = c0; rec[1] = s; rec[2] = nr; rec[3] = slot[c0];
+				for (int t = 0; t < s; t++) rec[4 + t] = colptr[c0 + t];
+				for (int i = 0; i < nr; i++)
+				{
+					const int sl = slot[rowidx[colptr[c0 + s - 1] + 1 + i]];
+					rec[4 + CHOL_GS + i] = sl;
+					if (sl < rec[3] + s) closed = false;
+				}
+			}
+			for (int k = b; k < e; k++)
+			{
+				const int g = tl.chain_grp[k];
+				for (int t = 0; t < ch.grp_s[g]; t++) slot[ch.grp_c0[g] + t] = -1;
+			}
+		}
+		if (!closed) { ch.gtail = CholTail(); ch.gtail.level = ngl; ch.gtail.chain_ptr.assign(1, 0); ch.gtail_rec.clear(); }
+		const size_t nsg = tl.single.size();
+		ch.gtail_single.resize(3 * nsg);
+		for (size_t q = 0; q < nsg; q++)
+		{
+			const int g = tl.single[q];
+			ch.gtail_single[q] = ch.grp_c0[g]; ch.gtail_single[nsg + q] = ch.grp_s[g]; ch.gtail_single[2 * nsg + q] = ch.grp_nr[g];
+		}
 	}
 	tick("groups");
+}
+
+void chol_tail_chains(const std::vector<int>& glevel_ptr, const std::vector<int>& glevel_maxnr, const std::vector<int>& grp_parent,
+                      const std::vector<int>& grp_s, CholTail& out)
+{
+	const int ngl = (int)glevel_ptr.size() - 1, ng = ngl > 0 ? glevel_ptr[ngl] : 0;
+	out.level = std::max(ngl, 0);
+	out.chain_ptr.assign(1, 0); out.chain_grp.clear(); out.single.clear();
+	if (ng == 0) return;
+	std::vector<int> root(ng), seen(ng, -1), cols(ng, 0);
+	for (int g = ng - 1; g >= 0; g--) root[g] = grp_parent[g] < 0 ? g : root[grp_parent[g]];
+	for (int l = ngl - 1; l >= 0; l--)
+	{
+		bool ok = glevel_maxnr[l] <= CHOL_TAIL_NR;
+		for (int g = glevel_ptr[l]; ok && g < glevel_ptr[l + 1]; g++)
+		{
+			const int r = root[g];
+			if (seen[r] == l || cols[r] + grp_s[g] > CHOL_TAIL_COLS) ok = false;
+			seen[r] = l; cols[r] += grp_s[g];
+		}
+		if (!ok) break;
+		out.level = l;
+	}
+	const int g0 = glevel_ptr[out.level];
+	std::vector<int>& cnt = cols;
+	std::fill(cnt.begin(), cnt.end(), 0);
+	for (int g = g0; g < ng; g++) cnt[root[g]]++;
+	std::vector<int>& chain = seen;
+	std::fill(chain.begin(), chain.end(), -1);
+	for (int g = g0; g < ng; g++)
+	{
+		const int r = root[g];
+		if (cnt[r] < 2) { out.single.push_back(g); continue; }
+		if (chain[r] < 0) { chain[r] = (int)out.chain_ptr.size() - 1; out.chain_ptr.push_back(out.chain_ptr.back() + cnt[r]); }
+	}
+	out.chain_grp.assign(out.chain_ptr.back(), -1);
+	std::vector<int> fill(out.chain_ptr.begin(), out.chain_ptr.end() - 1);
+	for (int g = g0; g < ng; g++)
+		if (cnt[root[g]] >= 2) out.chain_grp[fill[chain[root[g]]]++] = g;
 }
 
 }
@@ -735,3 +824,24 @@
 	}
 	return LSFM_OK;
 }
+
+extern "C" int lsfm_symbolic_tail(int nlevels, const int* glevel_ptr, const int* glevel_maxnr, const int* grp_parent, const int* grp_s, int* level,
+                                  int* nchains, int* chain_ptr, int* chain_grp, int* nsingle, int* single)
+{
+	if (nlevels < 0 || !glevel_ptr || glevel_ptr[0] != 0 || !level || !nchains || !chain_ptr || !chain_grp || !nsingle || !single) return LSFM_ERR_ARG;
+	if (nlevels > 0 && (!glevel_maxnr || !grp_parent || !grp_s)) return LSFM_ERR_ARG;
+	for (int l = 0; l < nlevels; l++)
+		if (glevel_ptr[l + 1] < glevel_ptr[l] || glevel_maxnr[l] < 0) return LSFM_ERR_ARG;
+	const int ng = glevel_ptr[nlevels];
+	for (int l = 0; l < nlevels; l++)
+		for (int g = glevel_ptr[l]; g < glevel_ptr[l + 1]; g++)
+			if (grp_s[g] < 1 || grp_s[g] > CHOL_GS || grp_parent[g] >= ng || (grp_parent[g] >= 0 && grp_parent[g] < glevel_ptr[l + 1])) return LSFM_ERR_ARG;
+	lsfm::CholTail t;
+	lsfm::chol_tail_chains(std::vector<int>(glevel_ptr, glevel_ptr + nlevels + 1), std::vector<int>(glevel_maxnr, glevel_maxnr + nlevels),
+	                       std::vector<int>(grp_parent, grp_parent + ng), std::vector<int>(grp_s, grp_s + ng), t);
+	*level = t.level; *nchains = (int)t.chain_ptr.size() - 1; *nsingle = (int)t.single.size();
+	std::copy(t.chain_ptr.begin(), t.chain_ptr.end(), chain_ptr);
+	std::copy(t.chain_grp.begin(), t.chain_grp.end(), chain_grp);
+	std::copy(t.single.begin(), t.single.end(), single);
+	return LSFM_OK;
+}
diff --git a/linearsfm_amd/csrc/lsfm_symbolic.hpp b/linearsfm_amd/csrc/lsfm_symbolic.hpp
--- a/linearsfm_amd/csrc/lsfm_symbolic.hpp
+++ b/linearsfm_amd/csrc/lsfm_symbolic.hpp
@@ -10,6 +10,18 @@
 #define CHOL_FACTOR_LDS (60 * 1024)
 #define CHOL_TASK_X_MAX 164
 
+#define CHOL_TAIL_NR 16
+#define CHOL_TAIL_COLS 512
+#define CHOL_TAIL_REC (4 + CHOL_GS + CHOL_TAIL_NR)
+struct CholTail {
+	int level = 0;
+	std::vector<int> chain_ptr;
+	std::vector<int> chain_grp;
+	std::vector<int> single;
+};
+void chol_tail_chains(const std::vector<int>& glevel_ptr, const std::vector<int>& glevel_maxnr, const std::vector<int>& grp_parent,
+                      const std::vector<int>& grp_s, CholTail& out);
+
 struct CholSymbolic {
 	int M = 0, nnzL = 0, nlevels = 0, tail_begin = 0;
 	std::vector<int> colptr, rowidx, perm, pinv, order, level_ptr;
@@ -17,6 +29,9 @@
 	std::vector<int> tlevel_ptr, tlevel_maxsize, tlevel_col0, tlevel_nsmall, tlevel_small_lds, tlevel_outer;
 	int ngroups = 0;
 	std::vector<int> grp_c0, grp_s, grp_nr, glevel_ptr, glevel_maxnr, glevel_maxs;
+	std::vector<int> grp_parent;
+	CholTail gtail;
+	std::vector<int> gtail_rec, gtail_single;
 	std::vector<int> parent, ccount;
 	int task_x = 0;
 	std::vector<int> col_owner;
```

Measured after the change: 29.78. About the same (+0.5%).
